# FYTalon/pienerf

Hardware: AMD Instinct MI355X
Metric: sim+render steps/s @800x800 chair (higher is better)
Workload: dtype f32 render / f64 sim

## Files before the change

### include/pienerf_hip.h

```cpp
#ifndef PIENERF_HIP_H
#define PIENERF_HIP_H
#include <stdint.h>
#ifdef __cplusplus
extern "C" {
#endif

#define PN_OK 0
#define PN_ERR_ARG 1
#define PN_ERR_HIP 2
#define PN_ERR_CAPACITY 3

const char* pn_version(void);

int pn_stream_create_cu_mask(uint32_t total_cu, uint32_t first_cu, uint32_t n_cu, int invert, void** stream_out);
int pn_stream_destroy(void* stream);
int pn_march_set_tail_rounds(int rounds);
int pn_march_set_skip_dda(int on);
int pn_device_cu_count(void);
const char* pn_last_error(void);


int pn_sph_from_ray(const float* rays_o, const float* rays_d, float radius, uint32_t N, float* coords, void* stream);
int pn_near_far_from_aabb(const float* rays_o, const float* rays_d, const float* aabb, uint32_t N, float min_near, float* nears, float* fars,
                          void* stream);

int pn_march_rays_quadratic_bending(const int* pig_cnt, const int* pig_bgn, const int* pig_idx, int n_vtx, int n_grid, const float* p_def,
                                    const float* p_ori, const float* F_IP, const float* dF_IP, int max_iter_num, const float* bbmin,
                                    const float* bbmax, float hgs, const int* resolution, int num_seek_IP, float IP_dx, int cut,
                                    const float* cut_bounds, uint32_t n_alive, uint32_t n_step, const int* rays_alive, const float* rays_t,
                                    const float* rays_o, const float* rays_d, float bound, float dt_gamma, uint32_t max_steps, uint32_t C,
                                    uint32_t H, const uint8_t* grid, const float* nears, const float* fars, float* xyzs, float* dirs,
                                    float* deltas, const float* noises, int* err_flag, void* stream);

int pn_composite_rays(uint32_t n_alive, uint32_t n_step, float T_thresh, int* rays_alive, float* rays_t, const float* sigmas, const float* rgbs,
                      const float* deltas, float* weights_sum, float* depth, float* image, void* stream);

int pn_compact_rays(const int* rays_alive, uint32_t n, int* out, int* n_out, int* scratch, void* stream);
uint32_t pn_compact_scratch_ints(uint32_t n);

int pn_pnts_in_grids(int n_vtx, int n_grid, const float* pnts, const float* bbmin, float hgs, const int* resolution, int* pig_cnt, int* pig_bgn,
                     int* pig_idx, int* err_flag, void* stream);

int pn_get_rays(const float* pose, float fx, float fy, float cx, float cy, int H, int W, float* rays_o, float* rays_d, void* stream);


int pn_grid_encode_forward(const float* inputs, const float* embeddings, const int* offsets_host, float* outputs, uint32_t B, uint32_t D,
                           uint32_t C, uint32_t L, float S, uint32_t H, float* dy_dx, uint32_t gridtype, int align_corners,
                           uint32_t interp, int out_bl_major, void* stream);

int pn_grid_encode_forward_half(const float* inputs, const uint16_t* embeddings, const int* offsets_host, uint16_t* outputs, uint32_t B, uint32_t D,
                                uint32_t C, uint32_t L, float S, uint32_t H, uint32_t gridtype, int align_corners, uint32_t interp,
                                int out_bl_major, void* stream);


int pn_sh_encode_forward(const float* inputs, float* outputs, uint32_t B, uint32_t D, uint32_t C, float* dy_dx, void* stream);


int pn_march_rays(uint32_t n_alive, uint32_t n_step, const int* rays_alive, const float* rays_t, const float* rays_o, const float* rays_d,
                  float bound, float dt_gamma, uint32_t max_steps, uint32_t C, uint32_t H, const uint8_t* grid, const float* nears,
                  const float* fars, float* xyzs, float* dirs, float* deltas, const float* noises, void* stream);
int pn_packbits(const float* grid, uint32_t N, float density_thresh, uint8_t* bitfield, void* stream);
int pn_morton3D(const int* coords, uint32_t N, int* indices, void* stream);
int pn_morton3D_invert(const int* indices, uint32_t N, int* coords, void* stream);


int pn_march_rays_train(const float* rays_o, const float* rays_d, const uint8_t* grid, float bound, float dt_gamma, uint32_t max_steps, uint32_t N,
                        uint32_t C, uint32_t H, uint32_t M, const float* nears, const float* fars, float* xyzs, float* dirs, float* deltas, int* rays,
                        int* counter, const float* noises, void* stream);
int pn_composite_rays_train_forward(const float* sigmas, const float* rgbs, const float* deltas, const int* rays, uint32_t M, uint32_t N, float T_thresh,
                                    float* weights_sum, float* depth, float* image, void* stream);
int pn_composite_rays_train_backward(const float* grad_weights_sum, const float* grad_image, const float* sigmas, const float* rgbs,
                                     const float* deltas, const int* rays, const float* weights_sum, const float* image, uint32_t M, uint32_t N,
                                     float T_thresh, float* grad_sigmas, float* grad_rgbs, void* stream);
int pn_grid_encode_backward(const float* grad, const float* inputs, const float* embeddings, const int* offsets_host, float* grad_embeddings,
                            uint32_t B, uint32_t D, uint32_t C, uint32_t L, float S, uint32_t H, const float* dy_dx, float* grad_inputs,
                            uint32_t gridtype, int align_corners, uint32_t interp, void* stream);
int pn_grid_encode_backward_half(const uint16_t* grad, const float* inputs, const int* offsets_host, uint16_t* grad_embeddings, uint32_t B, uint32_t D,
                                 uint32_t C, uint32_t L, float S, uint32_t H, uint32_t gridtype, int align_corners, uint32_t interp, void* stream);
int pn_grad_total_variation(const float* inputs, const float* embeddings, float* grad, const int* offsets_host, float weight, uint32_t B, uint32_t D,
                            uint32_t C, uint32_t L, float S, uint32_t H, uint32_t gridtype, int align_corners, void* stream);
int pn_sh_encode_backward(const float* grad, const float* inputs, uint32_t B, uint32_t D, uint32_t C, const float* dy_dx, float* grad_inputs,
                          void* stream);


typedef struct pn_net pn_net;
int pn_net_create(pn_net** out, const float* embeddings , const int* offsets_host , uint32_t L, uint32_t C,
                  float per_level_scale_log2, uint32_t base_resolution, float bound, const float* W0_host, const float* W1_host,
                  const float* W2_host, const float* W3_host, const float* W4_host, void* stream);
void pn_net_destroy(pn_net* net);
int pn_net_update(pn_net* net, const float* embeddings, const float* W0_host, const float* W1_host, const float* W2_host, const float* W3_host,
                  const float* W4_host, void* stream);
int pn_net_form(const pn_net* net);
int pn_net_form_epoch(const pn_net* net);
int pn_net_enable_half(pn_net* net, void* stream);
int pn_nerf_forward(const pn_net* net, const float* xyzs, const float* dirs, uint32_t M, float density_scale, float* sigmas, float* rgbs,
                    void* stream);
int pn_nerf_forward_half(const pn_net* net, const float* xyzs, const float* dirs, uint32_t M, float density_scale, float* sigmas, float* rgbs,
                         void* stream);
int pn_nerf_density(const pn_net* net, const float* xyzs, uint32_t M, float* sigmas, float* geo_feat, void* stream);
int pn_nerf_density_half(const pn_net* net, const float* xyzs, uint32_t M, float* sigmas, float* geo_feat, void* stream);
int pn_nerf_sigma(const pn_net* net, const float* xyzs, uint32_t M, float density_scale, float* sigmas, int half, void* stream);
int pn_host_float_to_half(const float* in_host, uint16_t* out_host, uint32_t n);


typedef struct pn_bg_net pn_bg_net;
int pn_bg_net_create(pn_bg_net** out, const float* embeddings, const int* offsets_host , uint32_t L, uint32_t C, float per_level_scale_log2,
                     uint32_t base_resolution, const float* W0_host, const float* W1_host, void* stream);
int pn_bg_net_update(pn_bg_net* net, const float* embeddings, const float* W0_host, const float* W1_host, void* stream);
void pn_bg_net_destroy(pn_bg_net* net);
int pn_background_forward(const pn_bg_net* net, const float* rays_o, const float* rays_d, uint32_t N, float radius, float* rgb_out,
                          const float* weights_sum, float* image, float* coords_out, void* stream);
int pn_background_forward_half(const pn_bg_net* net, const float* rays_o, const float* rays_d, uint32_t N, float radius, float* rgb_out,
                               const float* weights_sum, float* image, float* coords_out, void* stream);

int pn_background_coords(const pn_bg_net* net, const float* coords, const float* dirs, uint32_t N, float* rgb_out, int half, void* stream);

int pn_nerf_color(const pn_net* net, const float* dirs, const float* geo_feat, const uint8_t* mask, uint32_t M, float* rgbs, void* stream);
int pn_nerf_color_half(const pn_net* net, const float* dirs, const float* geo_feat, const uint8_t* mask, uint32_t M, float* rgbs, void* stream);

int pn_render_hier(const pn_net* net, const float* rays_o, const float* rays_d, uint32_t N, const float* aabb_host, float min_near, int num_steps,
                   int upsample_steps, float density_scale, float bg_scalar, const float* bg_rays, float* image, float* depth, float* weights_sum, int half,
                   void* stream);
int pn_hier_max_samples(void);


typedef struct pn_frame pn_frame;
typedef struct {
    int max_iter_num;
    float hash_grid_size;
    int num_seek_IP;
    float IP_dx;
    int cut;
    float cut_bounds[6];
    float bound;
    float min_near;
    float dt_gamma;
    uint32_t max_steps;
    float T_thresh;
    uint32_t cascade;
    uint32_t grid_size;
    float density_scale;
    float bg_color;
    int fp16;
    int reuse_tables;
    int ray_batch;
    int throughput;
    int throughput_trips;
    int ray_tile_w;
    int fused_from;
    int fused_whole;
    int fused_fold;
    int fused_grid;
} pn_render_opts;
int pn_frame_create(pn_frame** out, uint32_t max_rays, uint32_t max_vtx, uint32_t max_grid_cells);
void pn_frame_destroy(pn_frame* f);
int pn_render_deformed(pn_frame* f, const pn_net* net, const pn_render_opts* opts, const float* rays_o, const float* rays_d, uint32_t N,
                       const float* p_def, const float* p_ori, const float* F_IP, const float* dF_IP, int n_vtx, const uint8_t* bitfield,
                       float* image, float* depth, float* depth_0, float* weights_sum, int64_t* stats_host, void* stream);

int pn_render_deformed_async(pn_frame* f, const pn_net* net, const pn_render_opts* opts, const float* rays_o, const float* rays_d, uint32_t N,
                             const float* p_def, const float* p_ori, const float* F_IP, const float* dF_IP, int n_vtx, const uint8_t* bitfield,
                             float* image, float* depth, float* depth_0, float* weights_sum, int n_trips, void* stream);
int pn_render_status(pn_frame* f, int64_t* stats_host, int synchronize, void* stream);
int pn_frame_reset_unfinished(pn_frame* f, void* stream);

int pn_render_continue(pn_frame* f, const pn_net* net, const pn_render_opts* opts, const float* rays_o, const float* rays_d, uint32_t N,
                       const uint8_t* bitfield, float* image, float* depth, float* depth_0, float* weights_sum, int64_t* stats_host, int n_trips,
                       int is_static, void* stream);

int pn_render_static(pn_frame* f, const pn_net* net, const pn_render_opts* opts, const float* rays_o, const float* rays_d, uint32_t N,
                     const float* aabb_host, const uint8_t* bitfield, float* image, float* depth, float* depth_0, float* weights_sum,
                     int64_t* stats_host, int n_trips, void* stream);


typedef struct pn_copier pn_copier;
int pn_copier_create(pn_copier** out);
void pn_copier_destroy(pn_copier* c);
int pn_copier_submit(pn_copier* c, void* dst_host, const void* src_dev, uint64_t bytes, void* after_event, uint64_t* ticket);
int pn_copier_wait(pn_copier* c, uint64_t ticket);


int pn_mark_untrained_grid(const float* poses, uint32_t B, float fx, float fy, float cx, float cy, uint32_t cascade, uint32_t H, float bound,
                           float* density_grid, int* n_unseen, void* stream);
int pn_density_cells_full(uint32_t cascade, uint32_t H, float bound, const float* noise, float* xyzs, void* stream);
int pn_density_cells_partial(uint32_t cas, uint32_t H, float bound, uint32_t N, const int* rand_coords, const float* rand_pick, const float* noise,
                             const float* density_grid_cas, float* tmp_grid_cas, int* scratch, int* indices, float* xyzs, void* stream);
uint64_t pn_density_partial_scratch_ints(uint32_t H);
int pn_density_scatter(uint32_t n, const int* indices, const float* sigmas, float* tmp_grid_cas, void* stream);
int pn_density_grid_update(uint32_t n, float* density_grid, const float* tmp_grid, float decay, float density_thresh, uint8_t* bitfield,
                           double* partial, float* mean_thresh, void* stream);

int pn_frame_march_counters(pn_frame* f, int enable, uint64_t* counters_host, void* stream);
int pn_frame_fused_clocks(pn_frame* f, uint64_t* clocks_host, int* first_trip_out, int reset, void* stream);
int pn_frame_trip_records(pn_frame* f, int* records_host, int* tail_counts_host, int max_trips, void* stream);
int pn_frame_trip_times(pn_frame* f, float* march_ms_host, float* network_ms_host, int max_trips, int* n_trips_out, void* stream);


int pn_sim_update_F(int n_IP, const int* topo, const double* dof, const double* Nx, const double* dNx, const double* ddNx, float* pos, float* F,
                    float* dF, void* stream);

int pn_sim_calc_elastic(int n_IP, const int* topo, const double* dNx, const double* dof, double* RF, double* VF, double* FF, int mcadams_sweeps,
                        void* stream);

int pn_sim_collect_rhs(int n_k, double dx, const int* csr_bg, const int* csr_cnt, const int* csr_buf, const double* mu, const double* lam,
                       const double* dNx, const double* RF, const double* VF, double* rhs, void* stream);

int pn_sim_matvec3(int n, const double* A, const double* X, double* Y, void* stream);

int pn_sim_stepforward(int n_k, int n_IP, int iters, double dt, double dx, const int* topo, const int* csr_bg, const int* csr_cnt,
                       const int* csr_buf, const double* mu, const double* lam, const double* dNx, const double* dNx_csr, const int* csr_pos,
                       const double* Ainv,
                       const double* Mmat, const double* dof_rest, const double* rhs_rest, const double* rhs_gravity, const double* dof_f,
                       double* dof, double* dof_vel, double* work, int prepared, int mcadams_sweeps, void* stream);
uint64_t pn_sim_work_doubles(int n_k, int n_IP);
int pn_sim_cells_chunk_ips(void);
uint64_t pn_sim_cells_work_doubles(int n_k, int n_chunks);
int pn_sim_cells_prepare(int n_k, int n_chunks, double* work, void* stream);
int pn_sim_stepforward_cells(int n_k, int n_chunks, int iters, double dt, double dx, const int* chunk_tab, const double* dNx_cell, const double* mu_cell,
                             const double* lam_cell, const int* kp_bg, const int* kp_pos, const double* Ainv, const double* Mmat, const double* dof_rest,
                             const double* rhs_rest, const double* rhs_gravity, const double* dof_f, double* dof, double* dof_vel, double* work,
                             int mcadams_sweeps, void* stream);
uint64_t pn_sim_coop_bytes(int n_k, int n_IP, int n_wg);
int pn_sim_coop_prepare(int n_k, int n_IP, int n_wg, const int* csr_bg, const int* csr_cnt, void* coop, int* plan_out, void* stream);
int pn_sim_coop_status(const void* coop, int* timed_out);
int pn_sim_coop_clocks(const void* coop, uint64_t* ticks9);
int pn_sim_stepforward_coop(int n_k, int n_IP, int iters, double dt, double dx, const int* topo, const double* mu, const double* lam, const double* dNx,
                            const double* dNx_csr, const int* csr_pos, const double* Ainv, const double* Mmat, const double* dof_rest,
                            const double* rhs_rest, const double* rhs_gravity, const double* dof_f, double* dof, double* dof_vel, double* work,
                            void* coop, int n_wg, const int* plan, void* stream);
int pn_sim_prepare(int n_k, int n_IP, const int* csr_bg, const int* csr_cnt, double* work, void* stream);

int pn_sim_update_force(int n_k, int vid, const double* f3_host, double dx, const int* topo, const double* rho, const double* Nx, double* dof_f,
                        void* stream);

typedef struct pn_drag_state {
    int vid;
    int active;
    double target[3];
    double scale;
} pn_drag_state;
uint64_t pn_sim_drag_bytes(void);
uint64_t pn_sim_drag_work_doubles(void);
int pn_sim_drag_force(int n_k, int n_IP, const void* drag, const double* dof, double dx, const int* topo, const double* rho, const double* Nx,
                      double* dof_f, void* stream);
int pn_sim_drag_set(void* drag, int n_IP, int vid, int active, double scale, const double* target3_host, void* stream);
int pn_sim_drag_unproject(const float* depth0, int W, int H, double x, double y, const double* intr4, const double* pose16, const float* ip_pos,
                          int n_IP, void* drag, double* work, void* stream);


uint64_t pn_mc_work_bytes(int nx, int ny, int nz);
int pn_mc_count(const float* field, int nx, int ny, int nz, double threshold, void* work, int64_t* totals, void* stream);
int pn_mc_emit(const float* field, int nx, int ny, int nz, double threshold, const void* work, double* vertices, int* triangles, void* stream);
int pn_mc_case_table(uint8_t* tri_count, int8_t* tri_edges);

int pn_ccl_label(const uint8_t* occ, int nx, int ny, int nz, int connectivity, int* labels, void* stream);



int pn_sample_cells(const float* weights, const float* expo, int n_cells, int N, int64_t* cells_out, int* status, void* stream);
int pn_train_batch(const float* pose, float fx, float fy, float cx, float cy, int H, int W, int N, int mode, const int64_t* a, const int64_t* b,
                   const float* u, int patch, const float* image, int C, int64_t* inds_out, float* rays_o, float* rays_d, float* pixels_out,
                   void* stream);
int pn_error_map_update(float* map_row, const int64_t* cells, const float* err, int N, void* stream);

#ifdef __cplusplus
}
#endif
#endif
```

### pienerf_amd/_lib.py

```python
import ctypes as C
import os

_HERE = os.path.dirname(os.path.abspath(__file__))
LIB_PATH = os.environ.get("PN_LIB_PATH") or os.path.join(_HERE, "lib", "libpienerf_hip.so")

P = C.c_void_p
u32, i32, f32, f64, u64 = C.c_uint32, C.c_int, C.c_float, C.c_double, C.c_uint64


class RenderOpts(C.Structure):
    _fields_ = [("max_iter_num", i32), ("hash_grid_size", f32), ("num_seek_IP", i32), ("IP_dx", f32), ("cut", i32), ("cut_bounds", f32 * 6),
                ("bound", f32), ("min_near", f32), ("dt_gamma", f32), ("max_steps", u32), ("T_thresh", f32), ("cascade", u32), ("grid_size", u32),
                ("density_scale", f32), ("bg_color", f32), ("fp16", i32), ("reuse_tables", i32), ("ray_batch", i32), ("throughput", i32), ("throughput_trips", i32), ("ray_tile_w", i32),
                ("fused_from", i32), ("fused_whole", i32), ("fused_fold", i32), ("fused_grid", i32)]


SIGNATURES = {
    "pn_version": (C.c_char_p, []),
    "pn_last_error": (C.c_char_p, []),
    "pn_stream_create_cu_mask": (i32, [u32, u32, u32, i32, C.POINTER(C.c_void_p)]),
    "pn_stream_destroy": (i32, [P]),
    "pn_device_cu_count": (i32, []),
    "pn_march_set_tail_rounds": (i32, [i32]),
    "pn_march_set_skip_dda": (i32, [i32]),
    "pn_copier_create": (i32, [C.POINTER(P)]),
    "pn_copier_destroy": (None, [P]),
    "pn_copier_submit": (i32, [P, P, P, C.c_uint64, P, C.POINTER(C.c_uint64)]),
    "pn_copier_wait": (i32, [P, C.c_uint64]),
    "pn_near_far_from_aabb": (i32, [P, P, P, u32, f32, P, P, P]),
    "pn_sph_from_ray": (i32, [P, P, f32, u32, P, P]),
    "pn_march_rays_quadratic_bending": (i32, [P, P, P, i32, i32, P, P, P, P, i32, P, P, f32, P, i32, f32, i32, P, u32, u32, P, P, P, P, f32, f32, u32,
                                              u32, u32, P, P, P, P, P, P, P, P, P]),
    "pn_composite_rays": (i32, [u32, u32, f32, P, P, P, P, P, P, P, P, P]),
    "pn_compact_rays": (i32, [P, u32, P, P, P, P]),
    "pn_compact_scratch_ints": (u32, [u32]),
    "pn_pnts_in_grids": (i32, [i32, i32, P, P, f32, P, P, P, P, P, P]),
    "pn_get_rays": (i32, [P, f32, f32, f32, f32, i32, i32, P, P, P]),
    "pn_grid_encode_forward": (i32, [P, P, P, P, u32, u32, u32, u32, f32, u32, P, u32, i32, u32, i32, P]),
    "pn_sh_encode_forward": (i32, [P, P, u32, u32, u32, P, P]),
    "pn_net_create": (i32, [C.POINTER(P), P, P, u32, u32, f32, u32, f32, P, P, P, P, P, P]),
    "pn_net_destroy": (None, [P]),
    "pn_net_update": (i32, [P, P, P, P, P, P, P, P]),
    "pn_net_enable_half": (i32, [P, P]),
    "pn_nerf_forward_half": (i32, [P, P, P, u32, f32, P, P, P]),
    "pn_nerf_density_half": (i32, [P, P, u32, P, P, P]),
    "pn_nerf_sigma": (i32, [P, P, u32, f32, P, i32, P]),
    "pn_host_float_to_half": (i32, [P, P, u32]),
    "pn_grid_encode_forward_half": (i32, [P, P, P, P, u32, u32, u32, u32, f32, u32, u32, i32, u32, i32, P]),
    "pn_march_rays_train": (i32, [P, P, P, f32, f32, u32, u32, u32, u32, u32, P, P, P, P, P, P, P, P, P]),
    "pn_composite_rays_train_forward": (i32, [P, P, P, P, u32, u32, f32, P, P, P, P]),
    "pn_composite_rays_train_backward": (i32, [P, P, P, P, P, P, P, P, u32, u32, f32, P, P, P]),
    "pn_grid_encode_backward": (i32, [P, P, P, P, P, u32, u32, u32, u32, f32, u32, P, P, u32, i32, u32, P]),
    "pn_grid_encode_backward_half": (i32, [P, P, P, P, u32, u32, u32, u32, f32, u32, u32, i32, u32, P]),
    "pn_grad_total_variation": (i32, [P, P, P, P, f32, u32, u32, u32, u32, f32, u32, u32, i32, P]),
    "pn_sh_encode_backward": (i32, [P, P, u32, u32, u32, P, P, P]),
    "pn_march_rays": (i32, [u32, u32, P, P, P, P, f32, f32, u32, u32, u32, P, P, P, P, P, P, P, P]),
    "pn_packbits": (i32, [P, u32, f32, P, P]),
    "pn_morton3D": (i32, [P, u32, P, P]),
    "pn_morton3D_invert": (i32, [P, u32, P, P]),
    "pn_nerf_forward": (i32, [P, P, P, u32, f32, P, P, P]),
    "pn_nerf_density": (i32, [P, P, u32, P, P, P]),
    "pn_bg_net_create": (i32, [C.POINTER(P), P, P, u32, u32, f32, u32, P, P, P]),
    "pn_bg_net_update": (i32, [P, P, P, P, P]),
    "pn_bg_net_destroy": (None, [P]),
    "pn_background_forward": (i32, [P, P, P, u32, f32, P, P, P, P, P]),
    "pn_background_forward_half": (i32, [P, P, P, u32, f32, P, P, P, P, P]),
    "pn_background_coords": (i32, [P, P, P, u32, P, i32, P]),
    "pn_nerf_color": (i32, [P, P, P, P, u32, P, P]),
    "pn_nerf_color_half": (i32, [P, P, P, P, u32, P, P]),
    "pn_render_hier": (i32, [P, P, P, u32, C.POINTER(f32), f32, i32, i32, f32, f32, P, P, P, P, i32, P]),
    "pn_hier_max_samples": (i32, []),
    "pn_frame_create": (i32, [C.POINTER(P), u32, u32, u32]),
    "pn_frame_destroy": (None, [P]),
    "pn_render_deformed": (i32, [P, P, C.POINTER(RenderOpts), P, P, u32, P, P, P, P, i32, P, P, P, P, P, P, P]),
    "pn_render_deformed_async": (i32, [P, P, C.POINTER(RenderOpts), P, P, u32, P, P, P, P, i32, P, P, P, P, P, i32, P]),
    "pn_render_status": (i32, [P, P, i32, P]),
    "pn_frame_reset_unfinished": (i32, [P, P]),
    "pn_render_continue": (i32, [P, P, C.POINTER(RenderOpts), P, P, u32, P, P, P, P, P, P, i32, i32, P]),
    "pn_render_static": (i32, [P, P, C.POINTER(RenderOpts), P, P, u32, P, P, P, P, P, P, P, i32, P]),
    "pn_mark_untrained_grid": (i32, [P, u32, f32, f32, f32, f32, u32, u32, f32, P, P, P]),
    "pn_density_cells_full": (i32, [u32, u32, f32, P, P, P]),
    "pn_density_cells_partial": (i32, [u32, u32, f32, u32, P, P, P, P, P, P, P, P, P]),
    "pn_density_partial_scratch_ints": (u64, [u32]),
    "pn_density_scatter": (i32, [u32, P, P, P, P]),
    "pn_density_grid_update": (i32, [u32, P, P, f32, f32, P, P, P, P]),
    "pn_frame_march_counters": (i32, [P, i32, P, P]),
    "pn_frame_trip_times": (i32, [P, P, P, i32, P, P]),
    "pn_frame_fused_clocks": (i32, [P, P, P, i32, P]),
    "pn_net_form": (i32, [P]),
    "pn_net_form_epoch": (i32, [P]),
    "pn_frame_trip_records": (i32, [P, P, P, i32, P]),
    "pn_sim_update_F": (i32, [i32, P, P, P, P, P, P, P, P, P]),
    "pn_sim_calc_elastic": (i32, [i32, P, P, P, P, P, P, i32, P]),
    "pn_sim_collect_rhs": (i32, [i32, f64, P, P, P, P, P, P, P, P, P, P]),
    "pn_sim_matvec3": (i32, [i32, P, P, P, P]),
    "pn_sim_stepforward": (i32, [i32, i32, i32, f64, f64, P, P, P, P, P, P, P, P, P, P, P, P, P, P, P, P, P, P, i32, i32, P]),
    "pn_sim_prepare": (i32, [i32, i32, P, P, P, P]),
    "pn_sim_cells_chunk_ips": (i32, []),
    "pn_sim_cells_work_doubles": (u64, [i32, i32]),
    "pn_sim_cells_prepare": (i32, [i32, i32, P, P]),
    "pn_sim_stepforward_cells": (i32, [i32, i32, i32, f64, f64, P, P, P, P, P, P, P, P, P, P, P, P, P, P, P, i32, P]),
    "pn_sim_work_doubles": (u64, [i32, i32]),
    "pn_sim_coop_bytes": (u64, [i32, i32, i32]),
    "pn_sim_coop_prepare": (i32, [i32, i32, i32, P, P, P, C.POINTER(i32), P]),
    "pn_sim_coop_status": (i32, [P, C.POINTER(i32)]),
    "pn_sim_coop_clocks": (i32, [P, C.POINTER(u64)]),
    "pn_sim_stepforward_coop": (i32, [i32, i32, i32, f64, f64, P, P, P, P, P, P, P, P, P, P, P, P, P, P, P, P, i32, C.POINTER(i32), P]),
    "pn_sim_update_force": (i32, [i32, i32, P, f64, P, P, P, P, P]),
    "pn_sim_drag_bytes": (u64, []),
    "pn_sim_drag_work_doubles": (u64, []),
    "pn_sim_drag_force": (i32, [i32, i32, P, P, f64, P, P, P, P, P]),
    "pn_sim_drag_set": (i32, [P, i32, i32, i32, f64, P, P]),
    "pn_sim_drag_unproject": (i32, [P, i32, i32, f64, f64, P, P, P, i32, P, P, P]),
    "pn_mc_work_bytes": (u64, [i32, i32, i32]),
    "pn_mc_count": (i32, [P, i32, i32, i32, f64, P, P, P]),
    "pn_mc_emit": (i32, [P, i32, i32, i32, f64, P, P, P, P]),
    "pn_mc_case_table": (i32, [P, P]),
    "pn_ccl_label": (i32, [P, i32, i32, i32, i32, P, P]),
    "pn_sample_cells": (i32, [P, P, i32, i32, P, P, P]),
    "pn_train_batch": (i32, [P, f32, f32, f32, f32, i32, i32, i32, i32, P, P, P, i32, P, i32, P, P, P, P, P]),
    "pn_error_map_update": (i32, [P, P, P, i32, P]),
}

_lib = None


def lib():
    global _lib
    if _lib is None:
        if not os.path.exists(LIB_PATH):
            raise RuntimeError(f"{LIB_PATH} is missing: build it with `python -m pienerf_amd.build` (hipcc, gfx950). There is no CPU fallback.")
        import torch
        h = C.CDLL(LIB_PATH)
        for name, (res, args) in SIGNATURES.items():
            fn = getattr(h, name)
            fn.restype = res
            fn.argtypes = args
        _lib = h
    return _lib


def check(rc, what=""):
    if rc != 0:
        msg = lib().pn_last_error().decode(errors="replace")
        raise RuntimeError(f"libpienerf_hip: {what} failed with code {rc}: {msg}")


def require_gpu(*tensors):
    for t in tensors:
        if t is not None and not t.is_cuda:
            raise RuntimeError("pienerf_amd ops run on the GPU only (HIP kernels); got a CPU tensor and there is no CPU fallback")


def ptr(t):
    if t is None:
        return None
    assert t.is_contiguous(), "tensor must be contiguous"
    return C.c_void_p(t.data_ptr())


def stream_ptr():
    import torch
    return C.c_void_p(torch.cuda.current_stream().cuda_stream)
```

### pienerf_amd/csrc/pn_frame_kernels.h

```cpp
#pragma once
#include <float.h>

#include "pn_cell_hash.h"
#include "pn_compact.h"
#include "pn_march_kernels.h"
#include "pn_near_far.h"
#include "pn_side_tables.h"

#define PN_MAX_TRIPS 1100
#define PN_MIN_RAY_BATCH 64
#define PN_TRIP_BATCH 8
#define PN_TRIP_MARGIN 2
#define PN_TIMED_TRIPS 64

#include "pn_trips_fused.h"

struct pn_frame {
    uint32_t max_rays, max_vtx, max_cells;
    float *nears, *fars, *rays_t, *xyzs, *dirs, *deltas, *sigmas, *rgbs;
    float* acc_image;
    int *alive_a, *alive_b, *list, *chunk_counts;
    TailEntry* tail;
    int* list_seg;
    int* active_seg;
    uint32_t seg_cap;
    uint32_t* cell_bits;
    uint32_t* grid_regions;
    float* fars_eff;
    int* seg_counters;
    int* tail_counts;
    int *pig_cnt, *pig_bgn, *pig_idx, *pig_cursor;
    MarchSide side;
    PnTrip* trips;
    PnGroup* groups;
    int* group_cnt;
    uint32_t max_groups;
    PnFrameDev* dev;
    float* cut_bounds;
    PnTrip* trips_pinned;
    PnFrameDev* dev_pinned;
    float cut_bounds_host[6];
    int cut_bounds_valid;
    int last_trips;
    uint32_t last_N;
    uint32_t last_group_rays;
    int tables_n_vtx;
    unsigned long long* march_counters;
    int march_counters_on;
    hipEvent_t ev[PN_TIMED_TRIPS][3];
    int timed_trips;
    unsigned long long* stamps;
    int stamped;
    int* fused_ctl;
    uint32_t fused_blocks;
    unsigned long long* fused_clocks;
    int fused_first;
    float* t_resume;
    int* blist;
    int4* strag;
    uint32_t blist_cap;
    int skip_done;
    int head_marched;
    int fused_mode;
};

__global__ void k_set_aabb(PnFrameDev* dev, float a0, float a1, float a2, float a3, float a4, float a5) {
    dev->aabb[0] = a0; dev->aabb[1] = a1; dev->aabb[2] = a2; dev->aabb[3] = a3; dev->aabb[4] = a4; dev->aabb[5] = a5;
    dev->resolution[0] = dev->resolution[1] = dev->resolution[2] = dev->resolution[3] = 0;
    dev->err = 0;
}

__global__ void k_reset_unfinished(PnFrameDev* dev) { dev->unfinished = 0; }

__global__ void __launch_bounds__(256) k_frame_finish(uint32_t N, float bg, const float* __restrict__ nears, const float* __restrict__ fars,
                                                      const float* __restrict__ weights_sum, const float* __restrict__ depth_0,
                                                      const float* __restrict__ acc, float* __restrict__ image, float* __restrict__ depth,
                                                      const PnTrip* __restrict__ trips, PnFrameDev* dev, int trips_run, int add_fused) {
    const uint32_t i = threadIdx.x + blockIdx.x * blockDim.x;
    if (i < 64) {
        const int lane = (int)i;
        const int t_final = min(trips_run + (add_fused ? dev->fused_trips : 0), PN_MAX_TRIPS);
        int n_trips = 0;
        long long n_samples = 0;
        for (int k = lane; k < t_final; k += 64) {
            const PnTrip* r = trips + k;
            if (r->n_alive > 0) n_trips++;
            n_samples += r->dense ? r->n_emitted : r->n_samples;
        }
#pragma unroll
        for (int o = 32; o > 0; o >>= 1) { n_trips += __shfl_xor(n_trips, o); n_samples += __shfl_xor(n_samples, o); }
        if (lane == 0) {
            const int left = trips[t_final].n_alive;
            dev->trips_run = t_final;
            dev->fused_trips = 0;
            dev->stat_trips = n_trips;
            dev->stat_samples = n_samples;
            dev->alive_at_exit = left;
            if (left > 0) atomicAdd(&dev->unfinished, left);
        }
    }
    if (i >= N) return;
    const float k = (1 - weights_sum[i]) * bg;
    image[i * 3] = acc[i * 3] + k;
    image[i * 3 + 1] = acc[i * 3 + 1] + k;
    image[i * 3 + 2] = acc[i * 3 + 2] + k;
    depth[i] = fmaxf(depth_0[i] - nears[i], 0.0f) / (fars[i] - nears[i]);
}

__global__ void k_stamp(unsigned long long* slot) { *slot = __builtin_amdgcn_s_memrealtime(); }

template <bool LARGE>
__global__ void __launch_bounds__(1024) k_frame_tables(const float* __restrict__ p_def, int n_vtx, int cut, float bound, float hgs, int max_cells,
                                                       PnFrameDev* dev, int* pig_cnt, int* pig_bgn, int* pig_idx, int* pig_cursor, uint32_t* cell_bits) {
    extern __shared__ unsigned cnt2[];
    for (int w = threadIdx.x; w < 2 * ((max_cells + 31) / 32); w += blockDim.x) cell_bits[w] = 0u;
    __shared__ float smin[3][16], smax[3][16];
    __shared__ float sh_min[3];
    __shared__ int sh_res[4];
    __shared__ int wsum[16];
    __shared__ int carry_s;
    float mn[3] = {FLT_MAX, FLT_MAX, FLT_MAX}, mx[3] = {-FLT_MAX, -FLT_MAX, -FLT_MAX};
    for (int i = threadIdx.x; i < n_vtx; i += blockDim.x)
#pragma unroll
        for (int c = 0; c < 3; c++) { const float v = p_def[i * 3 + c]; mn[c] = fminf(mn[c], v); mx[c] = fmaxf(mx[c], v); }
    const int lane = threadIdx.x & 63, wid = threadIdx.x >> 6;
#pragma unroll
    for (int c = 0; c < 3; c++) {
#pragma unroll
        for (int o = 32; o > 0; o >>= 1) { mn[c] = fminf(mn[c], __shfl_xor(mn[c], o)); mx[c] = fmaxf(mx[c], __shfl_xor(mx[c], o)); }
        if (lane == 0) { smin[c][wid] = mn[c]; smax[c][wid] = mx[c]; }
    }
    __syncthreads();
    if (threadIdx.x == 0) {
        int ncell = 1;
        for (int c = 0; c < 3; c++) {
            float a = smin[c][0], b = smax[c][0];
            for (int w = 1; w < 16; w++) { a = fminf(a, smin[c][w]); b = fmaxf(b, smax[c][w]); }
            if (cut) { a = -bound; b = bound; }
            const float lo = a - 1e-3f, hi = b + 1e-3f;
            dev->aabb[c] = lo;
            dev->aabb[3 + c] = hi;
            sh_min[c] = lo;
            const int r = (int)ceilf((hi - lo) / hgs);
            dev->resolution[c] = r;
            sh_res[c] = r;
            ncell *= r;

        }
        int err = 0;
        if (ncell > max_cells || ncell <= 0) { err = 4; ncell = 0; }
        dev->resolution[3] = ncell;
        dev->err = err;
        dev->nb_alloc = 0;
        sh_res[3] = ncell;
        carry_s = 0;
    }
    __syncthreads();
    const int n_grid_all = sh_res[3], r0 = sh_res[0], r1 = sh_res[1], r2 = sh_res[2];
    const float b0 = sh_min[0], b1 = sh_min[1], b2 = sh_min[2];
    if (n_grid_all == 0) return;
    __shared__ int s_lo[3], s_hi[3];
    if (threadIdx.x < 3) { s_lo[threadIdx.x] = 0x7fffffff; s_hi[threadIdx.x] = -1; }
    __syncthreads();
    for (int p = threadIdx.x; p < n_vtx; p += blockDim.x) {
        const int q0 = (int)floorf((p_def[p * 3] - b0) / hgs), q1 = (int)floorf((p_def[p * 3 + 1] - b1) / hgs), q2 = (int)floorf((p_def[p * 3 + 2] - b2) / hgs);
        const int gid = q2 * r1 * r0 + q1 * r0 + q0;
        if (gid < 0 || gid >= n_grid_all) continue;
        const int c0 = gid % r0, c1 = (gid / r0) % r1, c2 = gid / (r0 * r1);
        atomicMin(&s_lo[0], c0); atomicMax(&s_hi[0], c0);
        atomicMin(&s_lo[1], c1); atomicMax(&s_hi[1], c1);
        atomicMin(&s_lo[2], c2); atomicMax(&s_hi[2], c2);
    }
    __syncthreads();
    if (threadIdx.x < 3) {
        const bool any = s_hi[threadIdx.x] >= 0;
        dev->ip_lo[threadIdx.x] = any ? s_lo[threadIdx.x] : 0;
        dev->ip_hi[threadIdx.x] = any ? s_hi[threadIdx.x] : -1;
    }
    if (LARGE) return;
    const int n_grid = n_grid_all;
    for (int g = threadIdx.x; g < (n_grid + 1) / 2; g += blockDim.x) cnt2[g] = 0u;
    __syncthreads();
    auto cell_of = [&](int p) {
        const int g0 = (int)floorf((p_def[p * 3] - b0) / hgs);
        const int g1 = (int)floorf((p_def[p * 3 + 1] - b1) / hgs);
        const int g2 = (int)floorf((p_def[p * 3 + 2] - b2) / hgs);
        const int gid = g2 * r1 * r0 + g1 * r0 + g0;
        return (gid < 0 || gid >= n_grid) ? -1 : gid;
    };
    auto count_of = [&](int g) { return (int)((cnt2[g >> 1] >> (16 * (g & 1))) & 0xFFFFu); };
    for (int p = threadIdx.x; p < n_vtx; p += blockDim.x) {
        const int gid = cell_of(p);
        if (gid >= 0) atomicAdd(&cnt2[gid >> 1], 1u << (16 * (gid & 1)));
        else atomicOr(&dev->err, 2);
    }
    __syncthreads();
    {
        int* out_cnt = pig_cnt;
        int* out_bgn = pig_bgn;
        int* out_cur = pig_cursor;
        for (int base = 0; base < n_grid; base += 4096) {
            const int i0 = base + threadIdx.x * 4;
            int v[4];
#pragma unroll
            for (int k = 0; k < 4; k++) {
                const int c = i0 + k;
                int val = 0;
                if (c < n_grid) {
                    val = count_of(c);
                    out_cnt[c] = val;
                }
                v[k] = val;
            }
            const int tsum = v[0] + v[1] + v[2] + v[3];
            int inc = tsum;
#pragma unroll
            for (int o = 1; o < 64; o <<= 1) {
                const int u = __shfl_up(inc, o);
                if (lane >= o) inc += u;
            }
            if (lane == 63) wsum[wid] = inc;
            __syncthreads();
            int woff = 0;
            for (int w = 0; w < wid; w++) woff += wsum[w];
            int total = 0;
            for (int w = 0; w < 16; w++) total += wsum[w];
            int run = carry_s + woff + inc - tsum;
#pragma unroll
            for (int k = 0; k < 4; k++) {
                if (i0 + k < n_grid) { out_bgn[i0 + k] = run; out_cur[i0 + k] = run; }
                run += v[k];
            }
            __syncthreads();
            if (threadIdx.x == 0) carry_s += total;
            __syncthreads();
        }
        if (threadIdx.x == 0) carry_s = 0;
        __syncthreads();
    }
    int* lidx = reinterpret_cast<int*>(cnt2 + (max_cells + 1) / 2);
    for (int p = threadIdx.x; p < n_vtx; p += blockDim.x) {
        const int gid = cell_of(p);
        if (gid >= 0) lidx[atomicAdd(pig_cursor + gid, 1)] = p;
    }
    __syncthreads();
    for (int g = threadIdx.x; g < n_grid; g += blockDim.x) {
        const int c = count_of(g);
        if (c < 2) continue;
        int* a = lidx + __hip_atomic_load(pig_bgn + g, __ATOMIC_RELAXED, __HIP_MEMORY_SCOPE_AGENT);
        for (int i = 1; i < c; i++) {
            const int v = a[i];
            int j = i - 1;
            while (j >= 0 && a[j] > v) { a[j + 1] = a[j]; j--; }
            a[j + 1] = v;
        }
    }
    __syncthreads();
    for (int p = threadIdx.x; p < n_vtx; p += blockDim.x) pig_idx[p] = lidx[p];
}

struct FramePrologue {
    int n_grid_max; const int* n_grid_dev; const int* res; const int* pig_cnt; const int* pig_bgn; const int* pig_idx; const float* p_def; int swap;
    int2* nb_rng; float4* nb; int nb_capacity; int list_blocks; uint32_t* cell_bits; int lds_words;
    int pack_blocks; int n_vtx; const float* p_ori; const float* F_IP; const float* dF_IP; float* rec;
    const float* rays_o; const float* rays_d; PnFrameDev* dev; uint32_t N; float min_near; float* nears; float* fars; float* rays_t; PnTrip* trips;
    int* tail_counts; int* seg_counters; int n_trip_records; int* alive; float* weights_sum; float* depth_0; float* image; PnGroup* groups;
    int* group_cnt; uint32_t group_rays; uint32_t n_groups; int* chunk_words;
    uint32_t tile_w, tile_lw;
    int early_finish; float bg; float* image_out; float* depth_out;
    const uint8_t* grid; uint32_t* grid_regions; int gr_blocks; int gr_R; int gr_C; uint32_t gr_H; float gr_bound; const float* cut_bounds;
};
#define PN_GRID_REGION_WORDS 1024

__device__ __forceinline__ void frame_lists_block(const FramePrologue& a) {
    extern __shared__ uint32_t lds_bits[];
    __shared__ int wtot[4];
    __shared__ int blk_base;
    const int n_grid = min(*a.n_grid_dev, a.n_grid_max);
    const int r0 = a.res[0], r1 = a.res[1], r2 = a.res[2];
    const int lane = threadIdx.x & 63, wid = threadIdx.x >> 6, sub = threadIdx.x & 7;
    const int words = (a.n_grid_max + 31) / 32;
    const int per_round = a.list_blocks * 32;
    const int ilo0 = a.dev->ip_lo[0], ilo1 = a.dev->ip_lo[1], ilo2 = a.dev->ip_lo[2], ihi0 = a.dev->ip_hi[0], ihi1 = a.dev->ip_hi[1], ihi2 = a.dev->ip_hi[2];
    const bool in_lds = a.lds_words > 0;
    if (in_lds) {
        for (int w = threadIdx.x; w < 2 * a.lds_words; w += blockDim.x) lds_bits[w] = 0u;
        __syncthreads();
    }
    for (int c0 = 0; c0 < n_grid; c0 += per_round) {
        const int c = c0 + (int)blockIdx.x * 32 + ((int)threadIdx.x >> 3);
        const bool valid = c < n_grid;
        int g0 = 0, g1 = 0, g2 = 0;
        if (valid) nb_cell_coords(c, r0, r1, g0, g1, g2);
        const bool near_ips = valid && g0 >= ilo0 - 1 && g0 <= ihi0 + 1 && g1 >= ilo1 - 1 && g1 <= ihi1 + 1 && g2 >= ilo2 - 1 && g2 <= ihi2 + 1;
        int cell[4], cnt[4], before[4];
        int total = 0;
#pragma unroll
        for (int k = 0; k < 4; k++) {
            const int q = sub + 8 * k;
            cell[k] = (near_ips && q < 27) ? ((q == 0) ? c : nb_neighbour(q - 1, a.swap, g0, g1, g2, r0, r1, r2)) : -1;
            cnt[k] = cell[k] >= 0 ? a.pig_cnt[cell[k]] : 0;
            int inc = cnt[k];
#pragma unroll
            for (int o = 1; o < 8; o <<= 1) {
                const int u = __shfl_up(inc, o, 8);
                if (sub >= o) inc += u;
            }
            before[k] = total + inc - cnt[k];
            total += __shfl(inc, 7, 8);
        }
        const int mine = (sub == 0) ? total : 0;
        int inc = mine;
#pragma unroll
        for (int o = 1; o < 64; o <<= 1) {
            const int u = __shfl_up(inc, o);
            if (lane >= o) inc += u;
        }
        if (lane == 63) wtot[wid] = inc;
        const int in_wave = __shfl(inc - mine, lane & ~7);
        __syncthreads();
        if (threadIdx.x == 0) {
            const int sum = wtot[0] + wtot[1] + wtot[2] + wtot[3];
            blk_base = sum ? atomicAdd(&a.dev->nb_alloc, sum) : 0;
        }
        __syncthreads();
        int w0 = blk_base + in_wave;
        for (int w = 0; w < wid; w++) w0 += wtot[w];
        __syncthreads();
        if (!valid) continue;
        const bool fits = w0 + total <= a.nb_capacity;
        if (sub == 0) {
            a.nb_rng[c] = (total > 0 && fits) ? make_int2(w0, w0 + total) : make_int2(0, 0);
            if (total > 0 && !fits) atomicOr(&a.dev->err, 8);
        }
        if (total == 0 || !fits) continue;
        if (sub == 0) atomicOr((in_lds ? lds_bits : a.cell_bits) + (c >> 5), 1u << (c & 31));
#pragma unroll
        for (int k = 0; k < 4; k++) {
            if (cell[k] < 0) continue;
            atomicOr((in_lds ? lds_bits + a.lds_words : a.cell_bits + words) + (cell[k] >> 5), 1u << (cell[k] & 31));
            const int n = cnt[k], b = a.pig_bgn[cell[k]];
            for (int i = 0; i < n; i++) {
                const int ip = a.pig_idx[b + i];
                a.nb[w0 + before[k] + i] = make_float4(a.p_def[ip * 3], a.p_def[ip * 3 + 1], a.p_def[ip * 3 + 2], __int_as_float(ip));
            }
        }
    }
    if (in_lds) {
        __syncthreads();
        for (int w = threadIdx.x; w < 2 * a.lds_words; w += blockDim.x) {
            const uint32_t v = lds_bits[w];
            if (v) atomicOr(a.cell_bits + (w < a.lds_words ? w : words + (w - a.lds_words)), v);
        }
    }
}

__device__ __forceinline__ void frame_rays_block(const FramePrologue& a, uint32_t block) {
    const uint32_t n = threadIdx.x + block * blockDim.x;
    if (block == 0 && a.groups) {
        for (uint32_t b = threadIdx.x; b < a.n_groups; b += blockDim.x) {
            a.groups[b] = PnGroup{(int)(b * a.group_rays), 1, (int)(b * a.group_rays), 0};
            a.group_cnt[b] = 0;
        }
    }
    {
        const int t = (int)block * 4 + (int)(threadIdx.x >> 6), w = threadIdx.x & 63;
        if (t < a.n_trip_records) {
            int v = 0;
            if (t == 0 && w == 0) v = (a.dev->err & 7) ? 0 : (int)a.N;
            if (t == 0 && w == 1) v = 1;
            reinterpret_cast<int*>(a.trips + t)[w] = v;
            if (w == 0) a.tail_counts[t] = 0;
        }
        if (block + 1 == gridDim.x - (uint32_t)(a.list_blocks + a.pack_blocks)) {
            for (int t2 = ((int)block + 1) * 4 + (int)(threadIdx.x >> 6); t2 < a.n_trip_records; t2 += 4) {
                reinterpret_cast<int*>(a.trips + t2)[w] = 0;
                if (w == 0) a.tail_counts[t2] = 0;
            }
        }
    }
    if (block == 0)
        for (int t = threadIdx.x; t < 6 * PN_SEGS; t += blockDim.x) a.seg_counters[t * PN_SEG_STRIDE] = 0;
    if (block == 0 && threadIdx.x == 0) {
        a.dev->fused_trips = 0;
        if (a.early_finish) {
            a.dev->trips_run = 0; a.dev->stat_trips = 0; a.dev->stat_samples = 0; a.dev->alive_at_exit = (int)a.N;
        }
    }
    if (threadIdx.x == 0) a.chunk_words[block] = 0;
    if (threadIdx.x < 2 && block + 1 == gridDim.x - (uint32_t)(a.list_blocks + a.pack_blocks)) a.chunk_words[block + 1 + threadIdx.x] = 0;
    if (n >= a.N) return;
    const float* aabb = a.dev->aabb;
    const float ox = a.rays_o[n * 3], oy = a.rays_o[n * 3 + 1], oz = a.rays_o[n * 3 + 2];
    const float dx = a.rays_d[n * 3], dy = a.rays_d[n * 3 + 1], dz = a.rays_d[n * 3 + 2];
    float near, far;
    pn_near_far(aabb, ox, oy, oz, dx, dy, dz, a.min_near, near, far);
    a.nears[n] = near;
    a.fars[n] = far;
    a.rays_t[n] = near;
    uint32_t ray = n;
    if (a.tile_w) {
        const uint32_t lw = a.tile_lw, tile = n >> 6, in = n & 63u, tiles_x = a.tile_w >> lw;
        ray = ((tile / tiles_x) * (64u >> lw) + (in >> lw)) * a.tile_w + ((tile % tiles_x) << lw) + (in & ((1u << lw) - 1u));
    }
    a.alive[n] = (int)ray;
    a.weights_sum[n] = 0.f;
    a.depth_0[n] = 0.f;
    a.image[n * 3] = 0.f; a.image[n * 3 + 1] = 0.f; a.image[n * 3 + 2] = 0.f;
    if (a.early_finish) {
        const float k = (1 - 0.f) * a.bg;
        a.image_out[n * 3] = 0.f + k; a.image_out[n * 3 + 1] = 0.f + k; a.image_out[n * 3 + 2] = 0.f + k;
        a.depth_out[n] = fmaxf(0.f - near, 0.0f) / (far - near);
    }
}

__global__ void __launch_bounds__(256) k_frame_prologue(FramePrologue a) {
    const int b = (int)blockIdx.x;
    if (b < a.list_blocks) { frame_lists_block(a); return; }
    if (b < a.list_blocks + a.pack_blocks) {
        const int t = threadIdx.x + (b - a.list_blocks) * 256;
        const int ip = t / PN_REC_FLOATS, j = t % PN_REC_FLOATS;
        if (ip < a.n_vtx) a.rec[t] = pnm2::pack_ip_float(j, ip, a.p_ori, a.p_def, a.F_IP, a.dF_IP);
        return;
    }
    if (b < a.list_blocks + a.pack_blocks + a.gr_blocks) {
        const int R = a.gr_R, n_reg = R * R * R;
        const int r = threadIdx.x + (b - a.list_blocks - a.pack_blocks) * 256;
        if (r < n_reg) {
            bool any = false;
            const int b0 = r % R, b1 = (r / R) % R, b2 = r / (R * R);
            const uint32_t vox_side = a.gr_H / (uint32_t)R, words_per_region = (vox_side * vox_side * vox_side) >> 6;
            const uint32_t words_per_level = (a.gr_H * a.gr_H * a.gr_H) >> 6;
            const uint2* g2 = reinterpret_cast<const uint2*>(a.grid);
            uint32_t acc_l[3] = {0u, 0u, 0u};
            for (int l = 0; l < a.gr_C; l++) {
                const int j = a.gr_C - 1 - l, side = 1 << j;
                const int c0 = R / 2 + (b0 - R / 2) * side, c1 = R / 2 + (b1 - R / 2) * side, c2 = R / 2 + (b2 - R / 2) * side;
                if (c0 < 0 || c1 < 0 || c2 < 0 || c0 + side > R || c1 + side > R || c2 + side > R) continue;
                const uint32_t first = (uint32_t)l * words_per_level + pnm2::morton3D((uint32_t)c0, (uint32_t)c1, (uint32_t)c2) * words_per_region;
                const uint32_t n_words = words_per_region << (3 * j);
                for (uint32_t q = 0; q < n_words; q++) {
                    const uint2 v = g2[(size_t)first + q];
                    acc_l[l] |= v.x | v.y;
                }
            }
            for (int L = a.gr_C - 2; L >= 0; L--) acc_l[L] |= acc_l[L + 1];
            const float w = 2.0f * a.gr_bound / (float)R, eps = 0.01f * w;
            const float x0 = -a.gr_bound + (float)b0 * w, y0 = -a.gr_bound + (float)b1 * w, z0 = -a.gr_bound + (float)b2 * w;
            const float* cb = a.cut_bounds;
            if (x0 + w > cb[0] - eps && x0 < cb[1] + eps && y0 + w > cb[2] - eps && z0 + w > cb[4] - eps && z0 < cb[5] + eps) any = true;
            for (int L = 0; L < a.gr_C; L++) {
                const unsigned long long m = __ballot(any || acc_l[L] != 0u);
                if ((threadIdx.x & 63) == 0) {
                    a.grid_regions[(size_t)L * (n_reg >> 5) + (r >> 5)] = (uint32_t)m;
                    a.grid_regions[(size_t)L * (n_reg >> 5) + (r >> 5) + 1] = (uint32_t)(m >> 32);
                }
            }
        }
        return;
    }
    frame_rays_block(a, (uint32_t)(b - a.list_blocks - a.pack_blocks - a.gr_blocks));
}
```

### pienerf_amd/csrc/pn_render_ops.hip

```cpp
#include <float.h>

#include "pn_render_records.h"
#include "pn_cell_hash.h"
#include "pn_side_tables.h"
#include "pn_march_kernels.h"
#include "pn_composite.h"
#include "pn_compact.h"
#include "pn_frame_kernels.h"

thread_local char pn_err_buf[512] = {0};

extern "C" int pn_pnts_in_grids(int n_vtx, int n_grid, const float* pnts, const float* bbmin, float hgs, const int* resolution, int* pig_cnt,
                                int* pig_bgn, int* pig_idx, int* err_flag, void* stream) {
    PN_REQUIRE(n_vtx > 0 && n_grid > 0 && pnts && bbmin && resolution && pig_cnt && pig_bgn && pig_idx);
    int* cursor = nullptr;
    hipStream_t st = (hipStream_t)stream;
    PN_HIP_CHECK(hipMallocAsync((void**)&cursor, sizeof(int) * (size_t)n_grid, st));
    int rc = pig_build(n_vtx, n_grid, nullptr, pnts, bbmin, hgs, resolution, pig_cnt, pig_bgn, pig_idx, cursor, err_flag, st);
    PN_HIP_CHECK(hipFreeAsync(cursor, st));
    return rc;
}

extern "C" int pn_march_set_skip_dda(int on) {
    PN_REQUIRE(on >= -1 && on <= 1);
    g_skip_dda_override = on;
    return PN_OK;
}
extern "C" int pn_march_set_tail_rounds(int rounds) {
    PN_REQUIRE(rounds >= 0);
    g_tail_rounds_override = rounds;
    return PN_OK;
}

extern "C" int pn_march_rays_quadratic_bending(const int* pig_cnt, const int* pig_bgn, const int* pig_idx, int n_vtx, int n_grid,
                                               const float* p_def, const float* p_ori, const float* F_IP, const float* dF_IP, int max_iter_num,
                                               const float* bbmin, const float* bbmax, float hgs, const int* resolution, int num_seek_IP,
                                               float IP_dx, int cut, const float* cut_bounds, uint32_t n_alive, uint32_t n_step,
                                               const int* rays_alive, const float* rays_t, const float* rays_o, const float* rays_d, float bound,
                                               float dt_gamma, uint32_t max_steps, uint32_t C, uint32_t H, const uint8_t* grid, const float* nears,
                                               const float* fars, float* xyzs, float* dirs, float* deltas, const float* noises, int* err_flag,
                                               void* stream) {
    (void)nears;
    PN_REQUIRE(pig_cnt && pig_bgn && pig_idx && p_def && p_ori && F_IP && dF_IP && bbmin && bbmax && resolution);
    PN_REQUIRE(rays_alive && rays_t && rays_o && rays_d && grid && fars && xyzs && dirs && deltas);
    PN_REQUIRE(num_seek_IP >= 1 && num_seek_IP <= 3);
    PN_REQUIRE(!cut || cut_bounds);
    PN_REQUIRE(C >= 1 && C <= 8 && H > 0 && n_step >= 1 && n_vtx > 0 && n_grid > 0);
    if (n_alive == 0) return PN_OK;
    hipStream_t st = (hipStream_t)stream;
    MarchSide s;
    s.nb_capacity = 27 * n_vtx;
    char* pool = nullptr;
    const size_t ints = ((size_t)n_grid + 1) * 5 * sizeof(int), nbb = (size_t)s.nb_capacity * sizeof(float4), recb = (size_t)n_vtx * PN_REC_FLOATS * sizeof(float);
    const size_t off_nb = (ints + 255) & ~(size_t)255, off_rec = (off_nb + nbb + 255) & ~(size_t)255;
    const size_t off_res = (off_rec + recb + 255) & ~(size_t)255;
    const uint32_t tail_cap = seg_cap_for(n_alive);
    const size_t tail_ctr = (size_t)3 * PN_SEGS * PN_SEG_STRIDE * sizeof(int);
    const size_t off_tail = (off_res + (size_t)n_alive * sizeof(float) + 255) & ~(size_t)255;
    PN_HIP_CHECK(hipMallocAsync((void**)&pool, off_tail + tail_ctr + (size_t)PN_SEGS * tail_cap * sizeof(TailEntry), st));
    PN_HIP_CHECK(hipMemsetAsync(pool + off_tail, 0, tail_ctr, st));
    s.nb_cnt = (int*)pool; s.nb_bgn = s.nb_cnt + n_grid + 1; s.nb_cursor = s.nb_bgn + n_grid + 1; s.nb_rng = (int2*)(s.nb_cursor + n_grid + 1);
    s.nb = (float4*)(pool + off_nb); s.rec = (float*)(pool + off_rec);
    int rc = march_side_build(s, n_vtx, n_grid, nullptr, resolution, pig_cnt, pig_bgn, pig_idx, p_def, p_ori, F_IP, dF_IP, num_seek_IP, err_flag, st);
    if (rc == PN_OK) {
        pnm::MarchParams a = make_march_params(pig_cnt, pig_bgn, pig_idx, n_vtx, n_grid, p_def, p_ori, F_IP, dF_IP, max_iter_num, bbmin, bbmax, hgs,
                                               resolution, num_seek_IP, IP_dx, cut, cut_bounds, rays_t, rays_o, rays_d, bound, dt_gamma, max_steps,
                                               C, H, grid, fars, err_flag);
        pnm2::March2Tables tb{s.nb_rng, s.nb, (const float4*)s.rec};
        int* const tail_ctrs = (int*)(pool + off_tail);
        MarchIO io{};
        io.n_alive = n_alive; io.n_step = n_step; io.rays_alive = rays_alive;
        io.xyzs = xyzs; io.dirs = dirs; io.deltas = deltas; io.noises = noises;
        io.t_resume = (float*)(pool + off_res);
        io.tail = (TailEntry*)(pool + off_tail + tail_ctr);
        io.tail_counts = tail_ctrs; io.tail_back = tail_ctrs + PN_SEGS * PN_SEG_STRIDE; io.tail_cursors = tail_ctrs + 2 * PN_SEGS * PN_SEG_STRIDE;
        io.tail_seg_cap = (int)tail_cap;
        io.max_rounds = (int)march_tail_rounds();
        if (io.t_resume) k_march_skip<<<pn_div_up(n_alive, 256), 256, 0, st>>>(a, tb, io);
        launch_march(num_seek_IP, pn_div_up(n_alive, 32), std::max(std::min(pn_div_up(n_alive, 4), 2048u), (uint32_t)PN_SEGS / 4), st, a, tb, io);
    }
    PN_HIP_CHECK(hipFreeAsync(pool, st));
    if (rc) return rc;
    PN_LAUNCH_CHECK();
    return PN_OK;
}

extern "C" int pn_composite_rays(uint32_t n_alive, uint32_t n_step, float T_thresh, int* rays_alive, float* rays_t, const float* sigmas,
                                 const float* rgbs, const float* deltas, float* weights_sum, float* depth, float* image, void* stream) {
    if (n_alive == 0) return PN_OK;
    PN_REQUIRE(rays_alive && rays_t && sigmas && rgbs && deltas && weights_sum && depth && image && n_step >= 1);
    k_composite<<<pn_div_up(n_alive, 256), 256, 0, (hipStream_t)stream>>>(n_alive, n_step, T_thresh, rays_alive, rays_t, sigmas, rgbs, deltas,
                                                                         weights_sum, depth, image, nullptr, nullptr, nullptr, 0, nullptr);
    PN_LAUNCH_CHECK();
    return PN_OK;
}

extern "C" uint32_t pn_compact_scratch_ints(uint32_t n) { return pn_div_up(n, 256) + 1; }

extern "C" int pn_compact_rays(const int* rays_alive, uint32_t n, int* out, int* n_out, int* scratch, void* stream) {
    PN_REQUIRE(n_out);
    hipStream_t st = (hipStream_t)stream;
    if (n == 0) { PN_HIP_CHECK(hipMemsetAsync(n_out, 0, sizeof(int), st)); return PN_OK; }
    PN_REQUIRE(rays_alive && out && scratch);
    const uint32_t chunks = pn_div_up(n, 256);
    k_chunk_count<<<chunks, 256, 0, st>>>(rays_alive, n, scratch);
    k_compact<<<chunks, 256, 0, st>>>(rays_alive, n, scratch, out, n_out, nullptr, nullptr, 0, 0, 0, nullptr, nullptr, nullptr, nullptr, nullptr, 0, 0);
    PN_LAUNCH_CHECK();
    return PN_OK;
}


extern "C" int pn_frame_create(pn_frame** out, uint32_t max_rays, uint32_t max_vtx, uint32_t max_grid_cells) {
    PN_REQUIRE(out && max_rays > 0 && max_vtx > 0 && max_grid_cells > 0);
    pn_frame* f = new pn_frame();
    memset(f, 0, sizeof(*f));
    f->max_rays = max_rays; f->max_vtx = max_vtx; f->max_cells = max_grid_cells;
    const size_t N = max_rays;
#define PN_ALLOC(ptr, bytes) PN_HIP_CHECK(hipMalloc((void**)&(ptr), (bytes)))
    PN_ALLOC(f->nears, N * 4); PN_ALLOC(f->fars, N * 4); PN_ALLOC(f->rays_t, N * 4);
    {
        int dev_id = 0, cus = 0;
        PN_HIP_CHECK(hipGetDevice(&dev_id));
        PN_HIP_CHECK(hipDeviceGetAttribute(&cus, hipDeviceAttributeMultiprocessorCount, dev_id));
        f->fused_blocks = (uint32_t)std::min(std::max(cus, 1), 1024);
    }
    f->blist_cap = (uint32_t)(N / 8 + 64 + (size_t)(f->fused_blocks + 1) * 64);
    const size_t NS = N + (size_t)f->fused_blocks * PN_FUSED_WAVES * 64 + f->blist_cap;
    PN_ALLOC(f->xyzs, NS * 12); PN_ALLOC(f->dirs, NS * 12); PN_ALLOC(f->deltas, NS * 8); PN_ALLOC(f->sigmas, NS * 4); PN_ALLOC(f->rgbs, NS * 12);
    PN_ALLOC(f->fused_ctl, (size_t)PN_FUSED_CTL_INTS * 4);
    PN_HIP_CHECK(hipMemset(f->fused_ctl, 0, (size_t)PN_FUSED_CTL_INTS * 4));
    PN_ALLOC(f->fused_clocks, 16 * sizeof(unsigned long long));
    PN_HIP_CHECK(hipMemset(f->fused_clocks, 0, 16 * sizeof(unsigned long long)));
    f->fused_first = -1;
    PN_ALLOC(f->t_resume, N * 4);
    PN_ALLOC(f->blist, (size_t)f->blist_cap * 8);
    PN_ALLOC(f->strag, (size_t)f->blist_cap * 16);
    PN_ALLOC(f->acc_image, N * 12);
    PN_ALLOC(f->alive_a, N * 4); PN_ALLOC(f->alive_b, N * 4); PN_ALLOC(f->list, N * 4); PN_ALLOC(f->chunk_counts, (N / 256 + 4) * 4);
    PN_ALLOC(f->pig_cnt, (size_t)max_grid_cells * 4); PN_ALLOC(f->pig_bgn, (size_t)max_grid_cells * 4);
    PN_ALLOC(f->pig_cursor, (size_t)max_grid_cells * 4); PN_ALLOC(f->pig_idx, (size_t)max_vtx * 4);
    PN_ALLOC(f->side.nb_rng, ((size_t)max_grid_cells + 1) * sizeof(int2));
    f->side.nb_capacity = 27 * (int)max_vtx;
    PN_ALLOC(f->side.nb, (size_t)f->side.nb_capacity * sizeof(float4)); PN_ALLOC(f->side.rec, (size_t)max_vtx * PN_REC_FLOATS * 4);
    f->seg_cap = seg_cap_for(max_rays);
    PN_ALLOC(f->tail, (size_t)PN_SEGS * f->seg_cap * sizeof(TailEntry)); PN_ALLOC(f->tail_counts, sizeof(int) * (PN_MAX_TRIPS + 2));
    PN_ALLOC(f->list_seg, (size_t)PN_SEGS * f->seg_cap * 4); PN_ALLOC(f->active_seg, (size_t)PN_SEGS * f->seg_cap * 4);
    PN_ALLOC(f->seg_counters, (size_t)6 * PN_SEGS * PN_SEG_STRIDE * 4);
    PN_ALLOC(f->cell_bits, 2 * (((size_t)max_grid_cells + 31) / 32) * 4);
    PN_ALLOC(f->fars_eff, N * 4);
    PN_ALLOC(f->grid_regions, (size_t)PN_GRID_REGION_WORDS * 4);
    PN_ALLOC(f->trips, sizeof(PnTrip) * (PN_MAX_TRIPS + 2)); PN_ALLOC(f->dev, sizeof(PnFrameDev)); PN_ALLOC(f->cut_bounds, 6 * 4);
    f->max_groups = pn_div_up(max_rays, PN_MIN_RAY_BATCH) + 1;
    PN_ALLOC(f->groups, sizeof(PnGroup) * 2 * f->max_groups); PN_ALLOC(f->group_cnt, sizeof(int) * f->max_groups);
#undef PN_ALLOC
    PN_HIP_CHECK(hipMalloc((void**)&f->march_counters, 16 * sizeof(unsigned long long)));
    PN_HIP_CHECK(hipMalloc((void**)&f->stamps, sizeof(unsigned long long) * PN_TIMED_TRIPS * 3));
    PN_HIP_CHECK(hipHostMalloc((void**)&f->trips_pinned, sizeof(PnTrip) * (PN_MAX_TRIPS + 2)));
    PN_HIP_CHECK(hipHostMalloc((void**)&f->dev_pinned, sizeof(PnFrameDev)));
    PN_HIP_CHECK(hipMemset(f->dev, 0, sizeof(PnFrameDev)));
    memset(f->dev_pinned, 0, sizeof(PnFrameDev));
    *out = f;
    return PN_OK;
}

extern "C" void pn_frame_destroy(pn_frame* f) {
    if (!f) return;
    void* ptrs[] = {f->acc_image, f->nears, f->fars, f->rays_t, f->xyzs, f->dirs, f->deltas, f->sigmas, f->rgbs, f->alive_a, f->alive_b, f->list,
                    f->chunk_counts, f->pig_cnt, f->pig_bgn, f->pig_cursor, f->pig_idx, f->trips, f->dev, f->cut_bounds,
                    f->side.nb_rng, f->side.nb, f->side.rec, f->march_counters, f->tail, f->tail_counts, f->stamps,
                    f->list_seg, f->active_seg, f->seg_counters, f->cell_bits, f->fars_eff, f->grid_regions, f->groups, f->group_cnt, f->fused_ctl, f->fused_clocks, f->t_resume, f->blist, f->strag};
    for (void* p : ptrs) if (p) (void)hipFree(p);
    for (int t = 0; t < PN_TIMED_TRIPS; t++)
        for (int e = 0; e < 3; e++) if (f->ev[t][e]) (void)hipEventDestroy(f->ev[t][e]);
    if (f->trips_pinned) (void)hipHostFree(f->trips_pinned);
    if (f->dev_pinned) (void)hipHostFree(f->dev_pinned);
    delete f;
}

static void frame_stats(pn_frame* f, int64_t* stats_host) {
    stats_host[0] = f->dev_pinned->stat_trips;
    stats_host[1] = f->dev_pinned->stat_samples;
    stats_host[2] = f->dev_pinned->err;
    stats_host[3] = f->dev_pinned->alive_at_exit;
    stats_host[4] = f->dev_pinned->unfinished;
}


struct FramePlan {
    bool is_static;
    uint32_t nblk;
    uint32_t march_grid, march_grid_first, march_grid_later, trip_grid, tail_grid;
    int dda_start;
    uint32_t skip_hop_budget;
    size_t bit_words;
    bool short_rays;
    int skip_bits_words;
    uint32_t reg_R;
    int grid_region_words_1, grid_region_words;
    size_t skip_lds;
    uint32_t lpr_rounds, lpr_trips;
    uint32_t group_rays, n_groups;
    bool fused_ok, want_whole, want_fold, early_finish;
    int fuse_from;
};

static FramePlan make_frame_plan(const pn_frame* f, const pn_render_opts* o, uint32_t N, bool is_static, bool resume, int async_trips, const uint8_t* bitfield) {
    FramePlan p{};
    p.is_static = is_static;
    p.nblk = pn_div_up(N, 256);
    p.march_grid = 8192;
    p.trip_grid = std::min(p.nblk, 1024u);
    p.march_grid_first = std::max(std::min(pn_div_up(N, 32), p.march_grid), (uint32_t)PN_SEGS);
    p.march_grid_later = std::max(std::min(pn_div_up(N, 256), p.march_grid), (uint32_t)PN_SEGS);
    p.tail_grid = std::max(std::min(pn_div_up(N, 4), 1024u), (uint32_t)PN_SEGS / 4);
    p.dda_start = g_skip_dda_override >= 0 ? g_skip_dda_override : 1;
    p.skip_hop_budget = 8;
    p.lpr_rounds = o->throughput > 0 ? (uint32_t)o->throughput : 0u;
    p.lpr_trips = (uint32_t)std::max(o->throughput_trips, 1);
    p.bit_words = (f->max_cells + 31) / 32;
    p.short_rays = !is_static && !o->cut && p.bit_words * 8 <= 48 * 1024;
    p.skip_bits_words = (p.short_rays || p.bit_words * 4 <= 48 * 1024) ? (int)p.bit_words : 0;
    p.reg_R = o->grid_size / 8;
    const bool reg_ok = !is_static && o->cut && p.dda_start && bitfield && o->grid_size % 32 == 0 && o->cascade >= 1 && o->cascade <= 3 &&
                        o->bound == (float)(1u << (o->cascade - 1)) && (p.reg_R / 2) % (1u << (o->cascade - 1)) == 0 &&
                        (uint64_t)p.reg_R * p.reg_R * p.reg_R / 32 * o->cascade <= PN_GRID_REGION_WORDS && ((uintptr_t)bitfield & 15) == 0;
    p.grid_region_words_1 = reg_ok ? (int)((uint64_t)p.reg_R * p.reg_R * p.reg_R / 32) : 0;
    p.grid_region_words = p.grid_region_words_1 * (int)o->cascade;
    p.skip_lds = (size_t)p.skip_bits_words * 4 * (p.short_rays ? 2 : 1) + (size_t)p.grid_region_words * 4;
    p.group_rays = o->ray_batch > 0 ? (uint32_t)o->ray_batch : 0u;
    p.n_groups = p.group_rays ? pn_div_up(N, p.group_rays) : 0u;
    p.fused_ok = !is_static && !p.group_rays && o->fused_from >= 0 && o->max_steps <= 8u * PN_FUSED_MAX_TRIPS;
    p.fuse_from = p.fused_ok ? std::max(o->fused_from, 1) : PN_MAX_TRIPS + 1;
    p.want_whole = p.fused_ok && o->fused_whole != 0 && o->fused_from == 0 && !resume;
    p.want_fold = p.fused_ok && !p.want_whole && o->fused_fold != 0 && o->fused_from <= 1 && !resume;
    p.early_finish = p.want_whole;
    return p;
}

struct RenderCall {
    pn_frame* f;
    const pn_net* net;
    const pn_render_opts* o;
    const float *rays_o, *rays_d;
    uint32_t N;
    const float *p_def, *p_ori, *F_IP, *dF_IP;
    int n_vtx;
    const uint8_t* bitfield;
    float *image, *depth, *depth_0, *weights_sum;
    const float* aabb_static;
    hipStream_t st;
    pnm::MarchParams mp, mq;
    pnm2::March2Tables tb;
};

static int* alive_list(const pn_frame* f, int t) { return (t & 1) ? f->alive_b : f->alive_a; }
static PnGroup* group_records(const pn_frame* f, const FramePlan& pl, int t) { return pl.group_rays ? f->groups + (size_t)(t & 1) * f->max_groups : nullptr; }
enum { SEG_TAIL, SEG_SAMP, SEG_EMIT, SEG_CURS, SEG_BACK, SEG_ACTIVE };
static int* seg_counter(const pn_frame* f, int which) { return f->seg_counters + which * PN_SEGS * PN_SEG_STRIDE; }

static MarchIO make_march_io(const RenderCall& c, const FramePlan& pl, int tt) {
    const pn_frame* f = c.f;
    const bool lpr = (uint32_t)tt < pl.lpr_trips && pl.lpr_rounds > 0;
    MarchIO io{};
    io.rays_alive = alive_list(f, tt);
    io.xyzs = f->xyzs; io.dirs = f->dirs; io.deltas = f->deltas;
    io.trip = f->trips + tt;
    io.list = f->list;
    io.t_resume = (tt == 0) ? f->t_resume : nullptr;
    io.tail = f->tail;
    io.tail_counts = seg_counter(f, SEG_TAIL); io.tail_back = seg_counter(f, SEG_BACK); io.tail_cursors = seg_counter(f, SEG_CURS);
    io.tail_seg_cap = (int)f->seg_cap;
    io.max_rounds = lpr ? (int)pl.lpr_rounds : (int)march_tail_rounds(tt);
    io.active = (tt == 0) ? f->active_seg : nullptr;
    io.active_counts = (tt == 0) ? seg_counter(f, SEG_ACTIVE) : nullptr;
    io.active_seg_cap = (int)f->seg_cap;
    io.list_seg = f->list_seg; io.samp_counts = seg_counter(f, SEG_SAMP); io.list_seg_cap = (int)f->seg_cap;
    io.emit_parts = seg_counter(f, SEG_EMIT);
    io.cell_bits = f->cell_bits; io.cell_bits_words = pl.skip_bits_words;
    io.cell_bits2 = pl.short_rays ? f->cell_bits + pl.bit_words : nullptr;
    io.fars_eff = pl.short_rays ? f->fars_eff : nullptr;
    io.groups = group_records(f, pl, tt); io.group_rays = pl.group_rays;
    io.lane_per_ray = lpr ? 1 : 0;
    io.dda_start = pl.dda_start; io.hop_budget = (int)pl.skip_hop_budget;
    io.grid_regions = pl.grid_region_words > 0 ? f->grid_regions : nullptr;
    io.grid_regions_words = pl.grid_region_words; io.grid_regions_R = (int)pl.reg_R;
    return io;
}

static int time_mark(pn_frame* f, hipStream_t st, int trip, int e, bool fused_group) {
    if (!(f->march_counters_on & 2) || trip >= PN_TIMED_TRIPS) return PN_OK;
    hipStreamCaptureStatus cs = hipStreamCaptureStatusNone;
    PN_HIP_CHECK(hipStreamIsCapturing(st, &cs));
    const bool stamp = cs != hipStreamCaptureStatusNone;
    f->stamped = stamp ? 1 : 0;
    if (stamp) {
        k_stamp<<<1, 1, 0, st>>>(f->stamps + trip * 3 + e);
    } else {
        if (!f->ev[trip][e]) PN_HIP_CHECK(hipEventCreate(&f->ev[trip][e]));
        PN_HIP_CHECK(hipEventRecord(f->ev[trip][e], st));
    }
    if (e == 2) f->timed_trips = fused_group ? std::max(f->timed_trips, trip + 1) : trip + 1;
    return PN_OK;
}

static int enqueue_tables(const RenderCall& c, bool is_static, bool keep_tables) {
    pn_frame* f = c.f;
    const pn_render_opts* o = c.o;
    const size_t tables_lds = ((size_t)f->max_cells + 1) / 2 * sizeof(unsigned) + (size_t)f->max_vtx * sizeof(int);
    const bool large = tables_lds > 150 * 1024;
    if (is_static) {
        const float* b = c.aabb_static;
        k_set_aabb<<<1, 1, 0, c.st>>>(f->dev, b[0], b[1], b[2], b[3], b[4], b[5]);
    } else if (keep_tables) {
    } else if (!large) {
        static size_t tables_lds_set[PN_MAX_DEVICES] = {0};
        int dev_id = 0;
        PN_HIP_CHECK(hipGetDevice(&dev_id));
        if (dev_id < 0 || dev_id >= PN_MAX_DEVICES || tables_lds > tables_lds_set[dev_id]) {
            PN_HIP_CHECK(hipFuncSetAttribute((const void*)k_frame_tables<false>, hipFuncAttributeMaxDynamicSharedMemorySize, (int)tables_lds));
            if (dev_id >= 0 && dev_id < PN_MAX_DEVICES) tables_lds_set[dev_id] = tables_lds;
        }
        k_frame_tables<false><<<1, 1024, tables_lds, c.st>>>(c.p_def, c.n_vtx, o->cut, o->bound, o->hash_grid_size, (int)f->max_cells, f->dev, f->pig_cnt,
                                                         f->pig_bgn, f->pig_idx, f->pig_cursor, f->cell_bits);
    } else {
        k_frame_tables<true><<<1, 1024, 0, c.st>>>(c.p_def, c.n_vtx, o->cut, o->bound, o->hash_grid_size, (int)f->max_cells, f->dev, f->pig_cnt, f->pig_bgn,
                                                   f->pig_idx, f->pig_cursor, f->cell_bits);
        return pig_build(c.n_vtx, (int)f->max_cells, f->dev->resolution + 3, c.p_def, f->dev->aabb, o->hash_grid_size, f->dev->resolution, f->pig_cnt, f->pig_bgn,
                         f->pig_idx, f->pig_cursor, &f->dev->err, c.st);
    }
    return PN_OK;
}

static int enqueue_prologue(const RenderCall& c, const FramePlan& pl) {
    pn_frame* f = c.f;
    const pn_render_opts* o = c.o;
    const bool keep_tables = !pl.is_static && o->reuse_tables && f->tables_n_vtx == c.n_vtx;
    int rc = enqueue_tables(c, pl.is_static, keep_tables);
    if (rc) return rc;
    FramePrologue fp;
    memset(&fp, 0, sizeof(fp));
    if (!pl.is_static && !keep_tables) {
        f->tables_n_vtx = c.n_vtx;
        fp.n_grid_max = (int)f->max_cells; fp.n_grid_dev = f->dev->resolution + 3; fp.res = f->dev->resolution; fp.pig_cnt = f->pig_cnt; fp.pig_bgn = f->pig_bgn;
        fp.pig_idx = f->pig_idx; fp.p_def = c.p_def; fp.swap = (o->num_seek_IP == 1) ? 1 : 0; fp.nb_rng = f->side.nb_rng; fp.nb = f->side.nb;
        fp.nb_capacity = f->side.nb_capacity; fp.cell_bits = f->cell_bits;
        fp.list_blocks = (int)std::min(pn_div_up((uint64_t)f->max_cells, 32), 2048u);
        fp.pack_blocks = (int)pn_div_up((uint64_t)c.n_vtx * PN_REC_FLOATS, 256);
        fp.n_vtx = c.n_vtx; fp.p_ori = c.p_ori; fp.F_IP = c.F_IP; fp.dF_IP = c.dF_IP; fp.rec = f->side.rec;
    }
    fp.rays_o = c.rays_o; fp.rays_d = c.rays_d; fp.dev = f->dev; fp.N = c.N; fp.min_near = o->min_near; fp.nears = f->nears; fp.fars = f->fars; fp.rays_t = f->rays_t;
    fp.trips = f->trips; fp.tail_counts = f->tail_counts; fp.seg_counters = f->seg_counters; fp.n_trip_records = PN_MAX_TRIPS + 2; fp.alive = f->alive_a;
    fp.weights_sum = c.weights_sum; fp.depth_0 = c.depth_0; fp.image = f->acc_image; fp.groups = pl.group_rays ? f->groups : nullptr; fp.group_cnt = f->group_cnt;
    fp.group_rays = pl.group_rays; fp.n_groups = pl.n_groups; fp.chunk_words = f->chunk_counts;
    fp.early_finish = pl.early_finish ? 1 : 0; fp.bg = o->bg_color; fp.image_out = c.image; fp.depth_out = c.depth;
    {
        const uint32_t lw = 4;
        const uint32_t tw = o->ray_tile_w > 0 ? (uint32_t)o->ray_tile_w : 0u;
        fp.tile_lw = lw;
        fp.tile_w = (!pl.is_static && !pl.group_rays && tw && tw % (1u << lw) == 0 && c.N % ((64u >> lw) * tw) == 0) ? tw : 0u;
    }
    fp.lds_words = (fp.list_blocks > 0 && pl.bit_words * 8 <= 64 * 1024) ? (int)pl.bit_words : 0;
    if (pl.grid_region_words > 0) {
        fp.grid = c.bitfield; fp.grid_regions = f->grid_regions; fp.gr_R = (int)pl.reg_R; fp.gr_C = (int)o->cascade; fp.gr_H = o->grid_size;
        fp.gr_bound = o->bound; fp.cut_bounds = f->cut_bounds; fp.gr_blocks = (int)pn_div_up((uint64_t)pl.grid_region_words_1 * 32, 256);
    }
    k_frame_prologue<<<(uint32_t)(fp.list_blocks + fp.pack_blocks + fp.gr_blocks) + pl.nblk, 256, (size_t)fp.lds_words * 8, c.st>>>(fp);
    PN_LAUNCH_CHECK();
    return PN_OK;
}

static void enqueue_skip(const RenderCall& c, const FramePlan& pl, const MarchIO& io0) {
    if (c.f->skip_done) return;
    k_march_skip<<<pl.nblk, 256, pl.skip_lds, c.st>>>(c.mp, c.tb, io0);
    c.f->skip_done = 1;
}
static void enqueue_march(const RenderCall& c, const FramePlan& pl, int t, bool margin) {
    const MarchIO io = make_march_io(c, pl, t);
    if (io.t_resume) enqueue_skip(c, pl, io);
    launch_march(c.o->num_seek_IP, t == 0 ? pl.march_grid_first : (margin ? 2u * PN_SEGS : pl.march_grid_later), margin ? (uint32_t)PN_SEGS : pl.tail_grid, c.st,
                 c.mq, c.tb, io);
}

static void enqueue_composite(const RenderCall& c, const FramePlan& pl, int t, bool margin) {
    pn_frame* f = c.f;
    const pn_render_opts* o = c.o;
    int *cur = alive_list(f, t), *nxt = alive_list(f, t + 1);
    PnGroup *g_cur = group_records(f, pl, t), *g_nxt = group_records(f, pl, t + 1);
    static const bool cc_trip0 = pn_env_u32("PN_CC_TRIP0", 0) != 0;
    if (!pl.is_static && !margin && (t > 0 || cc_trip0)) {
        static const uint32_t cc_grid = pn_env_u32("PN_CC_GRID", 512);
        const uint32_t cc_poll_cap = 1u << 20;
        k_composite_compact<<<std::min(cc_grid, pn_div_up(c.N, 256)), 256, 0, c.st>>>(o->T_thresh, cur, nxt, f->rays_t, f->sigmas, f->rgbs, f->deltas, c.weights_sum,
                                                                                   c.depth_0, f->acc_image, f->trips + t, f->trips + t + 1, (unsigned*)f->chunk_counts,
                                                                                   (uint32_t)t + 1, c.N, o->max_steps, 1, f->seg_counters, f->tail_counts + t, g_cur,
                                                                                   g_nxt, f->group_cnt, pl.group_rays, pl.n_groups, &f->dev->err, cc_poll_cap);
        return;
    }
    const uint32_t pair_grid = margin ? std::min(pl.trip_grid, 64u) : pl.trip_grid;
    k_composite<<<pair_grid, 256, 0, c.st>>>(0, 0, o->T_thresh, cur, f->rays_t, f->sigmas, f->rgbs, f->deltas, c.weights_sum, c.depth_0, f->acc_image, f->trips + t,
                                             f->chunk_counts, g_cur, pl.group_rays, pl.n_groups > 1 ? f->group_cnt : nullptr);
    k_compact<<<pair_grid, 256, 0, c.st>>>(cur, 0, f->chunk_counts, nxt, nullptr, f->trips + t, f->trips + t + 1, c.N, o->max_steps, pl.is_static ? 0 : 1,
                                           pl.is_static ? nullptr : f->seg_counters, f->tail_counts + t, g_cur, g_nxt, f->group_cnt, pl.group_rays, pl.n_groups);
}

static int enqueue_trip(const RenderCall& c, const FramePlan& pl, int t, bool margin) {
    pn_frame* f = c.f;
    const pn_render_opts* o = c.o;
    int rc;
    if ((rc = time_mark(f, c.st, t, 0, false))) return rc;
    if (pl.is_static) {
        k_march_static_trip<<<pl.trip_grid, 256, 0, c.st>>>(f->trips + t, alive_list(f, t), f->rays_t, c.rays_o, c.rays_d, o->bound, o->dt_gamma, o->max_steps,
                                                            o->cascade, o->grid_size, c.bitfield, f->fars, f->xyzs, f->dirs, f->deltas, f->list);
    } else {
        if (!(t == 0 && f->head_marched)) enqueue_march(c, pl, t, margin);
        if (t == 0) k_list_pack<<<PN_SEGS, 256, 0, c.st>>>(f->trips + t, seg_counter(f, SEG_SAMP), f->list_seg, (int)f->seg_cap, f->list);
    }
    if ((rc = time_mark(f, c.st, t, 1, false))) return rc;
    rc = pn_nerf_forward_launch(c.net, f->xyzs, f->dirs, f->list, &f->trips[t].n_samples, c.N, o->density_scale, f->sigmas, f->rgbs, o->fp16, c.st, margin ? 64u : 0u);
    if (rc) return rc;
    if ((rc = time_mark(f, c.st, t, 2, false))) return rc;
    enqueue_composite(c, pl, t, margin);
    return PN_OK;
}

static int enqueue_fused(const RenderCall& c, const FramePlan& pl, int t, int form, bool finalize) {
    pn_frame* f = c.f;
    const pn_net* net = c.net;
    const pn_render_opts* o = c.o;
    const bool whole = form == 1, fold = form == 2;
    int rc;
    if (fold) {
        if ((rc = time_mark(f, c.st, 0, 0, true))) return rc;
        enqueue_march(c, pl, 0, false);
        f->head_marched = 1;
        if ((rc = time_mark(f, c.st, 0, 1, true)) || (rc = time_mark(f, c.st, 0, 2, true))) return rc;
    }
    FusedArgs fa;
    memset(&fa, 0, sizeof(fa));
    fa.lv = (const PnFusedLevel*)(o->fp16 ? net->fused_levels : net->byte_levels); fa.emb = net->embeddings; fa.emb_h = (const uint32_t*)net->emb_half; fa.emb_bytes = net->n_entries * 4u;
    fa.wimg_g = (const uint4*)(o->fp16 ? net->whalf : (net->x_ok ? net->wx : net->wsplit)); fa.net_bound = net->bound; fa.net_inv2b = 1.0f / (2 * net->bound); fa.density_scale = o->density_scale;
    fa.x_scales = net->x_scales;
    fa.trips = f->trips + t; fa.N_rays = c.N; fa.max_steps = o->max_steps; fa.T_thresh = o->T_thresh;
    fa.alive = alive_list(f, t);
    fa.rays_t = f->rays_t; fa.weights_sum = c.weights_sum; fa.depth = c.depth_0; fa.image = f->acc_image;
    fa.xyzs = f->xyzs; fa.dirs = f->dirs; fa.deltas = f->deltas; fa.sigmas = f->sigmas; fa.rgbs = f->rgbs;
    fa.ctl = f->fused_ctl; fa.dev = f->dev; fa.tail_diag = f->tail_counts + t;
    fa.clocks = (f->march_counters_on & 4) ? f->fused_clocks : nullptr;
    if (whole) {
        fa.active = f->active_seg; fa.active_counts = seg_counter(f, SEG_ACTIVE); fa.active_seg_cap = (int)f->seg_cap; fa.t_resume = f->t_resume;
        fa.blist = f->blist; fa.strag = f->strag; fa.blist_cap = f->blist_cap;
        fa.a_rounds = 24;
    }
    if (fold) {
        fa.list_seg = f->list_seg; fa.samp_counts = seg_counter(f, SEG_SAMP); fa.list_seg_cap = (int)f->seg_cap;
        fa.seg_tail = seg_counter(f, SEG_TAIL); fa.seg_back = seg_counter(f, SEG_BACK);
        fa.blist = f->blist; fa.strag = f->strag; fa.blist_cap = f->blist_cap;
    }
    if (finalize) {
        fa.finalize = 1; fa.bg = o->bg_color; fa.nears = f->nears; fa.fars_full = f->fars; fa.image_out = c.image; fa.depth_out = c.depth;
    }
    const int tb_idx = fold ? 1 : t;
    if ((rc = time_mark(f, c.st, tb_idx, 0, true))) return rc;
    if (whole) enqueue_skip(c, pl, make_march_io(c, pl, 0));
    const uint32_t blocks = o->fused_grid > 0 ? std::min((uint32_t)o->fused_grid, f->fused_blocks) : f->fused_blocks;
    rc = launch_trips_fused(o->num_seek_IP, o->max_iter_num > 1, o->fp16 ? 1 : (net->x_ok ? 2 : 0), form, blocks, c.st, c.mq, c.tb, fa);
    if (rc) return rc;
    if ((rc = time_mark(f, c.st, tb_idx, 1, true)) || (rc = time_mark(f, c.st, tb_idx, 2, true))) return rc;
    f->fused_first = tb_idx;
    f->fused_mode = form;
    return PN_OK;
}

static int check_render_call(const RenderCall& c, bool is_static, bool resume, int async_trips) {
    const pn_frame* f = c.f;
    const pn_render_opts* o = c.o;
    PN_REQUIRE(f && c.net && o && c.rays_o && c.rays_d && c.bitfield && c.image && c.depth && c.depth_0 && c.weights_sum);
    PN_REQUIRE(is_static || resume || (c.p_def && c.p_ori && c.F_IP && c.dF_IP && c.n_vtx > 0 && (uint32_t)c.n_vtx <= f->max_vtx));
    PN_REQUIRE(!resume || c.N == f->last_N);
    PN_REQUIRE(c.N > 0 && c.N <= f->max_rays);
    PN_REQUIRE(o->num_seek_IP >= 1 && o->num_seek_IP <= 3 && o->cascade >= 1 && o->cascade <= 8 && o->max_steps <= PN_MAX_TRIPS - PN_TRIP_BATCH);
    PN_REQUIRE(async_trips >= 0 && async_trips <= PN_MAX_TRIPS);
    PN_REQUIRE(!o->fp16 || c.net->emb_half);
    PN_REQUIRE(o->ray_batch == 0 || (o->ray_batch >= PN_MIN_RAY_BATCH && !is_static));
    PN_REQUIRE((o->ray_batch > 0 ? pn_div_up(c.N, (uint32_t)o->ray_batch) : 0u) <= f->max_groups);
    PN_REQUIRE(!resume || (o->ray_batch > 0 ? (uint32_t)o->ray_batch : 0u) == f->last_group_rays);
    return PN_OK;
}

static int enqueue_trips(const RenderCall& c, const FramePlan& pl, int async_trips, bool resume, int& t, int& add_fused, bool& finished_in_launch) {
    pn_frame* f = c.f;
    int rc;
    bool done = false;
    bool whole_try = pl.want_whole && t == 0, fold_try = pl.want_fold && t == 0;
    while (!done && t < PN_MAX_TRIPS) {
        const bool whole = whole_try;
        whole_try = false;
        const bool fold = !whole && fold_try && t == 0 && !f->head_marched;
        if (fold) fold_try = false;
        if (whole || fold || t >= pl.fuse_from) {
            const bool finalize = (whole || fold) && pl.early_finish;
            if ((rc = enqueue_fused(c, pl, t, whole ? 1 : (fold ? 2 : 0), finalize))) return rc;
            if (async_trips > 0) {
                add_fused = 1;
                finished_in_launch = finalize;
                break;
            }
            PN_HIP_CHECK(hipMemcpyAsync(f->dev_pinned, f->dev, sizeof(PnFrameDev), hipMemcpyDeviceToHost, c.st));
            PN_HIP_CHECK(hipMemcpyAsync(f->trips_pinned + t, f->trips + t, sizeof(PnTrip), hipMemcpyDeviceToHost, c.st));
            PN_HIP_CHECK(hipStreamSynchronize(c.st));
            if (f->dev_pinned->fused_trips > 0) {
                t += f->dev_pinned->fused_trips;
                finished_in_launch = finalize;
                break;
            }
            if (f->trips_pinned[t].n_alive <= 0) break;
            f->fused_first = -1;
            f->fused_mode = 0;
        }
        const int batch = async_trips > 0 ? (pl.fused_ok ? pl.fuse_from - t : async_trips) : (pl.fused_ok ? std::max(pl.fuse_from - t, 1) : PN_TRIP_BATCH);
        for (int k = 0; k < batch; k++, t++) {
            const bool margin = !pl.fused_ok && async_trips > PN_TRIP_MARGIN && k >= async_trips - PN_TRIP_MARGIN && !resume;
            if ((rc = enqueue_trip(c, pl, t, margin))) return rc;
        }
        PN_LAUNCH_CHECK();
        if (async_trips > 0) {
            if (pl.fused_ok) continue;
            break;
        }
        if (pl.fused_ok && t >= pl.fuse_from) continue;
        PN_HIP_CHECK(hipMemcpyAsync(f->trips_pinned + t, f->trips + t, sizeof(PnTrip), hipMemcpyDeviceToHost, c.st));
        PN_HIP_CHECK(hipStreamSynchronize(c.st));
        done = f->trips_pinned[t].n_alive <= 0;
    }
    return PN_OK;
}

static int render_impl(pn_frame* f, const pn_net* net, const pn_render_opts* o, const float* rays_o, const float* rays_d, uint32_t N,
                       const float* p_def, const float* p_ori, const float* F_IP, const float* dF_IP, int n_vtx, const uint8_t* bitfield, float* image,
                       float* depth, float* depth_0, float* weights_sum, int64_t* stats_host, int async_trips, void* stream,
                       const float* aabb_static = nullptr, int mode = 0 ) {
    const bool is_static = aabb_static != nullptr || mode == 2;
    const bool resume = mode != 0;
    RenderCall c{};
    c.f = f; c.net = net; c.o = o; c.rays_o = rays_o; c.rays_d = rays_d; c.N = N;
    c.p_def = p_def; c.p_ori = p_ori; c.F_IP = F_IP; c.dF_IP = dF_IP; c.n_vtx = n_vtx; c.bitfield = bitfield;
    c.image = image; c.depth = depth; c.depth_0 = depth_0; c.weights_sum = weights_sum; c.aabb_static = aabb_static; c.st = (hipStream_t)stream;
    int rc = check_render_call(c, is_static, resume, async_trips);
    if (rc) return rc;
    const FramePlan pl = make_frame_plan(f, o, N, is_static, resume, async_trips, bitfield);
    c.mp = make_march_params(f->pig_cnt, f->pig_bgn, f->pig_idx, n_vtx, 0, p_def, p_ori, F_IP, dF_IP, o->max_iter_num, f->dev->aabb, f->dev->aabb + 3,
                             o->hash_grid_size, f->dev->resolution, o->num_seek_IP, o->IP_dx, o->cut, f->cut_bounds, f->rays_t, rays_o, rays_d, o->bound,
                             o->dt_gamma, o->max_steps, o->cascade, o->grid_size, bitfield, f->fars, &f->dev->err);
    c.mp.stats = (f->march_counters_on & 1) ? f->march_counters : nullptr;
    c.mq = c.mp;
    if (pl.short_rays) c.mq.fars = f->fars_eff;
    c.tb = pnm2::March2Tables{f->side.nb_rng, f->side.nb, (const float4*)f->side.rec};

    if (!f->cut_bounds_valid || memcmp(f->cut_bounds_host, o->cut_bounds, sizeof(f->cut_bounds_host)) != 0) {
        memcpy(f->cut_bounds_host, o->cut_bounds, sizeof(f->cut_bounds_host));
        PN_HIP_CHECK(hipMemcpyAsync(f->cut_bounds, f->cut_bounds_host, 6 * sizeof(float), hipMemcpyHostToDevice, c.st));
        f->cut_bounds_valid = 1;
    }
    if (!resume) {
        if ((rc = enqueue_prologue(c, pl))) return rc;
        f->skip_done = 0;
        f->head_marched = 0;
    }
    int t = resume ? f->dev_pinned->trips_run : 0;
    PN_REQUIRE(t >= 0 && t <= PN_MAX_TRIPS);
    f->fused_first = -1;
    int add_fused = 0;
    bool finished_in_launch = false;
    if ((rc = enqueue_trips(c, pl, async_trips, resume, t, add_fused, finished_in_launch))) return rc;
    if (!finished_in_launch)
        k_frame_finish<<<pl.nblk, 256, 0, c.st>>>(N, o->bg_color, f->nears, f->fars, weights_sum, depth_0, f->acc_image, image, depth, f->trips, f->dev, t, add_fused);
    PN_LAUNCH_CHECK();
    f->last_trips = t;
    f->last_N = N;
    f->last_group_rays = pl.group_rays;
    PN_HIP_CHECK(hipMemcpyAsync(f->dev_pinned, f->dev, sizeof(PnFrameDev), hipMemcpyDeviceToHost, c.st));
    if (async_trips == 0 && stats_host) {
        PN_HIP_CHECK(hipStreamSynchronize(c.st));
        frame_stats(f, stats_host);
    }
    return PN_OK;
}

extern "C" int pn_render_deformed(pn_frame* f, const pn_net* net, const pn_render_opts* o, const float* rays_o, const float* rays_d, uint32_t N,
                                  const float* p_def, const float* p_ori, const float* F_IP, const float* dF_IP, int n_vtx,
                                  const uint8_t* bitfield, float* image, float* depth, float* depth_0, float* weights_sum, int64_t* stats_host,
                                  void* stream) {
    return render_impl(f, net, o, rays_o, rays_d, N, p_def, p_ori, F_IP, dF_IP, n_vtx, bitfield, image, depth, depth_0, weights_sum, stats_host, 0, stream);
}

extern "C" int pn_render_deformed_async(pn_frame* f, const pn_net* net, const pn_render_opts* o, const float* rays_o, const float* rays_d,
                                        uint32_t N, const float* p_def, const float* p_ori, const float* F_IP, const float* dF_IP, int n_vtx,
                                        const uint8_t* bitfield, float* image, float* depth, float* depth_0, float* weights_sum, int n_trips,
                                        void* stream) {
    PN_REQUIRE(n_trips > 0);
    return render_impl(f, net, o, rays_o, rays_d, N, p_def, p_ori, F_IP, dF_IP, n_vtx, bitfield, image, depth, depth_0, weights_sum, nullptr, n_trips,
                       stream);
}

extern "C" int pn_render_static(pn_frame* f, const pn_net* net, const pn_render_opts* o, const float* rays_o, const float* rays_d, uint32_t N,
                                const float* aabb_host, const uint8_t* bitfield, float* image, float* depth, float* depth_0, float* weights_sum,
                                int64_t* stats_host, int n_trips, void* stream) {
    PN_REQUIRE(aabb_host && n_trips >= 0);
    return render_impl(f, net, o, rays_o, rays_d, N, nullptr, nullptr, nullptr, nullptr, 0, bitfield, image, depth, depth_0, weights_sum, stats_host, n_trips,
                       stream, aabb_host);
}

extern "C" int pn_render_continue(pn_frame* f, const pn_net* net, const pn_render_opts* o, const float* rays_o, const float* rays_d, uint32_t N,
                                  const uint8_t* bitfield, float* image, float* depth, float* depth_0, float* weights_sum, int64_t* stats_host, int n_trips,
                                  int is_static, void* stream) {
    PN_REQUIRE(n_trips >= 0);
    return render_impl(f, net, o, rays_o, rays_d, N, nullptr, nullptr, nullptr, nullptr, 0, bitfield, image, depth, depth_0, weights_sum, stats_host, n_trips,
                       stream, nullptr, is_static ? 2 : 1);
}

extern "C" int pn_frame_march_counters(pn_frame* f, int enable, uint64_t* counters_host, void* stream) {
    PN_REQUIRE(f);
    hipStream_t st = (hipStream_t)stream;
    if (counters_host) {
        PN_HIP_CHECK(hipMemcpyAsync(counters_host, f->march_counters, 4 * sizeof(unsigned long long), hipMemcpyDeviceToHost, st));
#if PN_DBG_PHASES || PN_DBG_STATS
        {
            unsigned long long ph[16];
            PN_HIP_CHECK(hipMemcpy(ph, f->march_counters, sizeof(ph), hipMemcpyDeviceToHost));
            fprintf(stderr, "phases:");
            for (int i = 4; i < 16; i++) fprintf(stderr, " %llu", ph[i]);
            fprintf(stderr, "\n");
        }
#endif
        PN_HIP_CHECK(hipStreamSynchronize(st));
    }
    if ((enable & 1) && !(f->march_counters_on & 1)) PN_HIP_CHECK(hipMemsetAsync(f->march_counters, 0, 16 * sizeof(unsigned long long), st));
    f->march_counters_on = enable & 7;
    return PN_OK;
}

extern "C" int pn_frame_fused_clocks(pn_frame* f, uint64_t* clocks_host, int* first_trip_out, int reset, void* stream) {
    PN_REQUIRE(f);
    hipStream_t st = (hipStream_t)stream;
    if (clocks_host) {
        PN_HIP_CHECK(hipMemcpyAsync(clocks_host, f->fused_clocks, 16 * sizeof(unsigned long long), hipMemcpyDeviceToHost, st));
        PN_HIP_CHECK(hipStreamSynchronize(st));
        clocks_host[15] = f->fused_first >= 0 ? (uint64_t)f->fused_mode : 0u;
    }
    if (first_trip_out) *first_trip_out = f->fused_first;
    if (reset) PN_HIP_CHECK(hipMemsetAsync(f->fused_clocks, 0, 16 * sizeof(unsigned long long), st));
    return PN_OK;
}

extern "C" int pn_frame_trip_times(pn_frame* f, float* march_ms_host, float* network_ms_host, int max_trips, int* n_trips_out, void* stream) {
    PN_REQUIRE(f && march_ms_host && network_ms_host && n_trips_out && max_trips >= 0);
    PN_HIP_CHECK(hipStreamSynchronize((hipStream_t)stream));
    const int n = f->timed_trips < max_trips ? f->timed_trips : max_trips;
    if (f->stamped) {
        static unsigned long long host[PN_TIMED_TRIPS * 3];
        PN_HIP_CHECK(hipMemcpy(host, f->stamps, sizeof(unsigned long long) * (size_t)n * 3, hipMemcpyDeviceToHost));
        for (int t = 0; t < n; t++) {
            march_ms_host[t] = (float)((double)(host[t * 3 + 1] - host[t * 3]) * 1e-5);
            network_ms_host[t] = (float)((double)(host[t * 3 + 2] - host[t * 3 + 1]) * 1e-5);
        }
    } else {
        for (int t = 0; t < n; t++) {
            PN_HIP_CHECK(hipEventElapsedTime(march_ms_host + t, f->ev[t][0], f->ev[t][1]));
            PN_HIP_CHECK(hipEventElapsedTime(network_ms_host + t, f->ev[t][1], f->ev[t][2]));
        }
    }
    *n_trips_out = n;
    return PN_OK;
}

extern "C" int pn_frame_trip_records(pn_frame* f, int* records_host, int* tail_counts_host, int max_trips, void* stream) {
    PN_REQUIRE(f && records_host && tail_counts_host && max_trips >= 0);
    PN_HIP_CHECK(hipStreamSynchronize((hipStream_t)stream));
    const int n = max_trips < PN_MAX_TRIPS ? max_trips : PN_MAX_TRIPS;
    std::vector<PnTrip> rec((size_t)n);
    PN_HIP_CHECK(hipMemcpy(rec.data(), f->trips, sizeof(PnTrip) * (size_t)n, hipMemcpyDeviceToHost));
    for (int i = 0; i < n; i++) {
        int* r = records_host + 5 * i;
        r[0] = rec[i].n_alive; r[1] = rec[i].n_step; r[2] = rec[i].step_base; r[3] = rec[i].n_samples; r[4] = rec[i].dense ? rec[i].n_emitted : -1;
    }
    PN_HIP_CHECK(hipMemcpy(tail_counts_host, f->tail_counts, sizeof(int) * (size_t)n, hipMemcpyDeviceToHost));
    return PN_OK;
}


extern "C" int pn_frame_reset_unfinished(pn_frame* f, void* stream) {
    PN_REQUIRE(f);
    k_reset_unfinished<<<1, 1, 0, (hipStream_t)stream>>>(f->dev);
    PN_LAUNCH_CHECK();
    return PN_OK;
}

extern "C" int pn_render_status(pn_frame* f, int64_t* stats_host, int synchronize, void* stream) {
    PN_REQUIRE(f && stats_host);
    if (synchronize) PN_HIP_CHECK(hipStreamSynchronize((hipStream_t)stream));
    frame_stats(f, stats_host);
    return PN_OK;
}
```

### pienerf_amd/frames.py

```python
import random

import torch
import torch.distributed as dist


def agree_on_launch_form(kw, src=0, group=None, device=None):
    import torch
    import torch.distributed as dist
    on_gpu = dist.get_backend(group) == "nccl"
    pick = torch.tensor([int(kw["fused_from"]), int(bool(kw["fused_whole"])), int(bool(kw["fused_fold"]))], dtype=torch.int64,
                        device=device if on_gpu else "cpu")
    dist.broadcast(pick, src=src, group=group)
    kw["fused_from"], kw["fused_whole"], kw["fused_fold"] = int(pick[0]), bool(pick[1]), bool(pick[2])
    return kw


def dedicated_sim_default(world_size):
    return world_size >= 3


def frame_owner(frame, world_size, sim_owner=0, dedicated_sim=False):
    if not dedicated_sim or world_size == 1:
        return frame % world_size
    k = frame % (world_size - 1)
    return k if k < sim_owner else k + 1


def broadcast_tensors(tensors, src=0, group=None):
    if not dist.is_initialized() or dist.get_world_size(group) == 1:
        return
    for t in tensors:
        dist.broadcast(t, src=src, group=group)


def checkpoint_tensors(model):
    ts = [model.encoder.embeddings.data, model.density_bitfield] + [l.weight.data for l in list(model.sigma_net) + list(model.color_net)]
    if getattr(model, "bg_net", None) is not None:
        ts += [model.encoder_bg.embeddings.data] + [l.weight.data for l in model.bg_net]
    return ts


def broadcast_checkpoint(model, src=0, group=None):
    broadcast_tensors(checkpoint_tensors(model), src=src, group=group)
    for stamp in ("_net_sig", "_bg_sig"):
        if hasattr(model, stamp):
            setattr(model, stamp, None)


def tile_partition(W, H, world, tile=8):
    ys, xs = torch.meshgrid(torch.arange(H), torch.arange(W), indexing="ij")
    block = (ys // tile) * ((W + tile - 1) // tile) + (xs // tile)
    owner = (block % world).reshape(-1)
    parts = [torch.nonzero(owner == r).reshape(-1) for r in range(world)]
    n = max(p.numel() for p in parts)
    return [torch.cat([p, torch.full((n - p.numel(),), -1, dtype=torch.int64)]) for p in parts]


class TileParallel:

    def __init__(self, W, H, render_subset, get_dof, set_dof, sim_step, sim_owner=0, group=None, tile=8, device="cpu", force_collectives=False):
        on = dist.is_available() and dist.is_initialized()
        self.collectives = on and (dist.get_world_size(group) > 1 or bool(force_collectives))
        self.world = dist.get_world_size(group) if on else 1
        self.rank = dist.get_rank(group) if on else 0
        self.W, self.H, self.group, self.owner = W, H, group, sim_owner
        self.src = dist.get_global_rank(group, sim_owner) if (on and group is not None) else sim_owner
        self.parts = [p.to(device) for p in tile_partition(W, H, self.world, tile)]
        self.render_subset, self.get_dof, self.set_dof, self.sim_step = render_subset, get_dof, set_dof, sim_step
        self._recv = None
        self._gather = None

    def step(self):
        if self.collectives:
            buf = self.get_dof() if self.rank == self.owner else (self._recv if self._recv is not None else torch.empty_like(self.get_dof()))
            self._recv = None if self.rank == self.owner else buf
            dist.broadcast(buf, src=self.src, group=self.group)
            if self.rank != self.owner:
                self.set_dof(buf)
        mine = self.render_subset(self.parts[self.rank]).contiguous()
        if self.collectives:
            if self._gather is None or self._gather.shape[1:] != mine.shape or self._gather.dtype != mine.dtype:
                self._gather = torch.empty((self.world,) + tuple(mine.shape), dtype=mine.dtype, device=mine.device)
            dist.all_gather_into_tensor(self._gather.view(-1, mine.shape[1]), mine, group=self.group)
            gathered = list(self._gather.unbind(0))
        else:
            gathered = [mine]
        full = torch.empty(self.W * self.H, mine.shape[1], dtype=mine.dtype, device=mine.device)
        for part, data in zip(self.parts, gathered):
            ok = part >= 0
            full[part[ok]] = data[ok]
        if self.rank == self.owner:
            self.sim_step()
        return full


class FramePipeline:

    def __init__(self, backend, world=1, rank=0, lanes=2, depth=2, ahead=None, sim_owner=0, dedicated_sim=None, copy_out=True, on_retire=None, force_collectives=False,
                 sim_on_lanes=False):
        self.b, self.world, self.rank, self.lanes, self.depth, self.owner = backend, int(world), int(rank), int(lanes), int(depth), int(sim_owner)
        self.dedicated = dedicated_sim_default(self.world) if dedicated_sim is None else bool(dedicated_sim and self.world > 1)
        self.ahead = self.world * self.lanes * self.depth if ahead is None else int(ahead)
        self.slots = self.ahead + self.world * self.lanes * self.depth + 1
        self.copy_out = copy_out
        self.collectives = self.world > 1 or bool(force_collectives)
        self.on_retire = on_retire
        b = backend
        self.s_sim, self.s_comm, self.s_copy = b.stream("sim"), b.stream("comm"), b.stream("copy")
        self.s_lane = [b.stream(f"lane{i}") for i in range(self.lanes)]
        S = self.slots
        self.snap_ready = [b.event() for _ in range(S)]
        self.bc_done = [b.event() for _ in range(S)]
        self.ip_done = [b.event() for _ in range(S)]
        self.bc_used, self.ip_used = [False] * S, [False] * S
        n_ws = self.lanes * self.depth
        self.render_done = [b.event() for _ in range(n_ws)]
        self.out_ready = [b.event() for _ in range(n_ws)]
        self.pending = [None] * n_ws
        self.frame = 0
        self.my_frames = 0
        self.sim_next = 0
        self.bc_next = 0
        self.retired = []
        self.last_ws, self.last_frame = None, None
        self.sim_on_lanes = bool(sim_on_lanes) and self.world == 1
        self.sub_done = [b.event() for _ in range(self.lanes + 2)] if self.sim_on_lanes else []
        self.force_done, self.force_pending = (b.event() if self.sim_on_lanes else None), False

    def before_force(self):
        if self.sim_on_lanes and self.sim_next > 0:
            self.s_sim.wait(self.sub_done[(self.sim_next - 1) % len(self.sub_done)])

    def after_force(self):
        if self.sim_on_lanes:
            self.force_done.record(self.s_sim)
            self.force_pending = True

    def _ws(self, k):
        lane = k % self.lanes
        return lane, lane * self.depth + (k // self.lanes) % self.depth

    def _advance_simulator(self, upto):
        b, S = self.b, self.slots
        while self.sim_next <= upto:
            g = self.sim_next
            slot = g % S
            s = self.s_lane[g % self.lanes] if self.sim_on_lanes else self.s_sim
            if self.sim_on_lanes:
                if g > 0:
                    s.wait(self.sub_done[(g - 1) % len(self.sub_done)])
                if self.force_pending:
                    s.wait(self.force_done)
                    self.force_pending = False
            if self.bc_used[slot]:
                s.wait(self.bc_done[slot])
            if self.ip_used[slot]:
                s.wait(self.ip_done[slot])
            b.snapshot(s, slot)
            self.snap_ready[slot].record(s)
            b.substep(s)
            if self.sim_on_lanes:
                self.sub_done[g % len(self.sub_done)].record(s)
            self.sim_next += 1

    def _broadcasts(self, upto):
        b, S = self.b, self.slots
        while self.bc_next <= upto:
            slot = self.bc_next % S
            if self.rank == self.owner:
                self.s_comm.wait(self.snap_ready[slot])
            elif self.ip_used[slot]:
                self.s_comm.wait(self.ip_done[slot])
            b.broadcast(self.s_comm, slot, self.owner)
            self.bc_done[slot].record(self.s_comm)
            self.bc_used[slot] = True
            self.bc_next += 1

    def retire(self, ws):
        f = self.pending[ws]
        if f is None:
            return None
        b = self.b
        (self.out_ready if self.copy_out else self.render_done)[ws].host_wait()
        if not b.complete(ws):
            b.finish(ws)
        self.pending[ws] = None
        res = b.result(ws)
        if self.on_retire is not None:
            self.on_retire(f, res)
            fence = getattr(b, "consumer_fence", None)
            if fence is not None:
                fence(ws)
        return f, res

    def step(self, pose=None):
        b, f, S = self.b, self.frame, self.slots
        self.retired = []
        if self.rank == self.owner:
            self._advance_simulator(f + self.ahead)
        if self.collectives:
            self._broadcasts(f + self.ahead)
        mine = frame_owner(f, self.world, self.owner, self.dedicated) == self.rank
        if mine:
            lane, ws = self._ws(self.my_frames)
            done = self.retire(ws)
            if done is not None:
                self.retired.append(done)
            slot = f % S
            s = self.s_lane[lane]
            s.wait(self.bc_done[slot] if self.collectives else self.snap_ready[slot])
            b.render(s, f, ws, slot, pose)
            self.ip_done[slot].record(s)
            self.ip_used[slot] = True
            self.render_done[ws].record(s)
            if self.copy_out:
                where = getattr(b, "copy_on", "copy")
                sc = s if where == "lane" else (self.s_sim if where == "sim" else self.s_copy)
                if sc is not s:
                    sc.wait(self.render_done[ws])
                b.copy_out(sc, ws)
                self.out_ready[ws].record(sc)
            self.pending[ws] = f
            self.last_ws, self.last_frame = ws, f
            self.my_frames += 1
        elif self.dedicated and self.rank == self.owner and self.world > 1:
            self.bc_done[f % S].host_wait()
        self.frame += 1
        return self.retired

    def drain(self):
        out = [self.retire(ws) for ws in range(self.lanes * self.depth)]
        out = sorted(r for r in out if r is not None)
        self.retired = out
        return out

    @property
    def substeps_enqueued(self):
        return self.sim_next


class _SimEvent:
    def __init__(self, be):
        self.be, self.stream, self.pos = be, None, -1

    def record(self, stream):
        self.stream, self.pos = stream, len(stream.ops) + stream.base
        stream.ops.append(("record", self, None))

    def host_wait(self):
        self.be.run_until(self)


class _SimStream:
    def __init__(self, name):
        self.name, self.ops, self.base, self.executed = name, [], 0, 0

    def wait(self, event):
        self.ops.append(("wait", (event.stream, event.pos), None))


class SimulatedBackend:

    def __init__(self, world, rank, n_dof=64, owner=0, seed=0, needs_more_trips=lambda frame: False, group=None):
        self.world, self.rank, self.owner, self.group = world, rank, owner, group
        self.rng = random.Random(seed * 1000 + rank)
        self.streams = {}
        self.dof = torch.arange(n_dof, dtype=torch.float64) * (1.0 if rank == owner else -7.0)
        self.steps = 0
        self.snap, self.snap_tag = {}, {}
        self.readers_left = {}
        self.ws_out, self.ws_host, self.ws_trips_short = {}, {}, {}
        self.needs_more_trips = needs_more_trips
        self.log = []

    def stream(self, name):
        return self.streams.setdefault(name, _SimStream(name))

    def event(self):
        return _SimEvent(self)

    def _enqueue(self, s, what, fn):
        s.ops.append(("op", what, fn))

    def _ready(self, s):
        if not s.ops:
            return False
        kind, a, _ = s.ops[0]
        return kind != "wait" or a[0] is None or a[0].executed > a[1]

    def _run_one(self, s):
        kind, a, fn = s.ops.pop(0)
        s.base += 1
        if kind == "op":
            fn()
        s.executed += 1

    def run_until(self, event):
        guard = 0
        while not (event.stream is None or event.stream.executed > event.pos):
            ready = [s for s in self.streams.values() if self._ready(s)]
            assert ready, f"deadlock: nothing can run while waiting for a point of stream {event.stream.name}"
            pick = event.stream if (event.stream in ready and self.rng.random() < 0.5) else self.rng.choice(ready)
            self._run_one(pick)
            guard += 1
            assert guard < 10_000_000

    def flush(self):
        while True:
            ready = [s for s in self.streams.values() if self._ready(s)]
            if not ready:
                break
            self._run_one(self.rng.choice(ready))
        assert all(not s.ops for s in self.streams.values()), "operations left that can never run"

    def snapshot(self, s, slot):
        g = self._sim_enq = getattr(self, "_sim_enq", 0)
        self._sim_enq += 1

        def run():
            prev = self.snap_tag.get(slot)
            assert self.steps == g, f"snapshot of frame {g} taken after {self.steps} substeps"
            assert self.readers_left.get((slot, prev), 0) == 0, f"snapshot slot {slot} overwritten with frame {g} while frame {prev} still has readers"
            self.snap[slot] = self.dof.clone()
            self.snap_tag[slot] = g
        self._enqueue(s, f"snapshot {g}", run)

    def substep(self, s):
        def run():
            self.dof = self.dof * 1.01 + 0.5
            self.steps += 1
        self._enqueue(s, "substep", run)

    def broadcast(self, s, slot, src):
        g = self._bc_enq = getattr(self, "_bc_enq", 0)
        self._bc_enq += 1

        def run():
            if self.rank == src:
                assert self.snap_tag.get(slot) == g, f"broadcast of frame {g} finds frame {self.snap_tag.get(slot)} in slot {slot}"
                buf = self.snap[slot]
            else:
                prev = self.snap_tag.get(slot)
                assert self.readers_left.get((slot, prev), 0) == 0, f"slot {slot} received frame {g} while frame {prev} still has readers"
                buf = self.snap.setdefault(slot, torch.empty_like(self.dof))
            dist.broadcast(buf, src=src, group=self.group)
            self.snap_tag[slot] = g
        self._enqueue(s, f"broadcast {g}", run)

    def render(self, s, frame, ws, slot, pose):
        key = (slot, frame)
        self.readers_left[key] = self.readers_left.get(key, 0) + 1

        def run():
            assert self.snap_tag.get(slot) == frame, f"frame {frame} rendered from slot {slot} holding frame {self.snap_tag.get(slot)}"
            self.readers_left[key] -= 1
            short = bool(self.needs_more_trips(frame))
            self.ws_out[ws] = (frame, float(self.snap[slot].sum()), None if pose is None else float(pose), "partial" if short else "full")
            self.ws_trips_short[ws] = short
            self.log.append(frame)
        self._enqueue(s, f"render {frame}", run)

    def copy_out(self, s, ws):
        def run():
            self.ws_host[ws] = self.ws_out[ws]
        self._enqueue(s, f"copy_out {ws}", run)

    def complete(self, ws):
        return not self.ws_trips_short[ws]

    def finish(self, ws):
        f, v, p, _ = self.ws_out[ws]
        self.ws_out[ws] = self.ws_host[ws] = (f, v, p, "full")
        self.ws_trips_short[ws] = False

    def result(self, ws):
        return self.ws_host.get(ws, self.ws_out.get(ws))
```

### pienerf_amd/harness.py

```python
import contextlib
import gc
import os

import numpy as np
import torch

from . import scene
from .nerf.network import NeRFNetwork
from .nerf.utils import get_rays
from .simulator.solver import Simulator


@contextlib.contextmanager
def _capture(graph, **kw):
    gc.collect()
    was = gc.isenabled()
    gc.disable()
    try:
        with torch.cuda.graph(graph, capture_error_mode="thread_local", **kw):
            yield
    finally:
        if was:
            gc.enable()


THROUGHPUT_FORM_MIN_RAYS = 131072

class SimRenderHarness:
    def __init__(self, opt=None, cloud=None, ckpt=None, device="cuda", overlap_sim=True):
        self.opt = dict(opt or scene.default_opt())
        o = self.opt
        self.device = torch.device(device)
        self.cloud = cloud if cloud is not None else scene.make_chair_points(hgs=o["hash_grid_size"], bound=o["bound"])
        self.ckpt = ckpt if ckpt is not None else scene.make_checkpoint(bound=o["bound"], bg_radius=o["bg_radius"])
        self.model = NeRFNetwork(encoding="hashgrid", bound=o["bound"], cuda_ray=True, density_scale=1, min_near=o["min_near"],
                                 density_thresh=o["density_thresh"], bg_radius=o["bg_radius"]).to(self.device)
        self.model.load_checkpoint_dict(self.ckpt)
        self.model.eval()
        self.sim = Simulator(dt=o["sim_dt"], iters=o["sim_iters"], bbox=torch.tensor([2.0 * o["bound"]] * 3), dx=o["sim_dx"], stiff=o["sim_stiff"],
                             base=torch.tensor([-o["bound"]] * 3), device=self.device)
        c = self.cloud
        self.sim.InitializeFromArrays(c["pos"], c["mass"], c["mu"], c["lam"], c["pin"])
        IP_pos, IP_F, IP_dF = self.sim.get_IP_info()
        m = self.model
        m.p_ori, m.p_def, m.IP_F, m.IP_dF = IP_pos, IP_pos, IP_F, IP_dF
        m.IP_dx = self.sim.dx * 1.05
        self.frame = 0
        self.pose = scene.orbit_pose(o["radius"])
        self.intrinsics = scene.orbit_intrinsics(o["W"], o["H"], o["fovy"])
        self._pose_dev = None
        self.overlap_sim = overlap_sim
        if overlap_sim:
            self._sim_stream = torch.cuda.Stream(self.device)
            self._ip_ready = torch.cuda.Event()
            self._sim_done = torch.cuda.Event()
            self._sim_done.record(torch.cuda.current_stream(self.device))
            self.sim.force_stream = self._sim_stream

    def synchronize(self):
        torch.cuda.synchronize(self.device)
        self._check_persistent_substep()

    def _amp(self):
        return torch.autocast("cuda", dtype=torch.float16, enabled=bool(self.opt.get("fp16", False)))

    def render_kwargs(self):
        return dict(self.opt)

    @torch.no_grad()
    def step(self, pose=None, intrinsics=None, W=None, H=None, simulate=True, collect_stats=False, fused=True, render_kw=None):
        o = self.opt
        W, H = W or o["W"], H or o["H"]
        pose = self.pose if pose is None else pose
        intrinsics = self.intrinsics if intrinsics is None else intrinsics
        key = np.asarray(pose, np.float32).tobytes()
        if self._pose_dev is None or self._pose_dev[0] != key:
            self._pose_dev = (key, torch.from_numpy(np.asarray(pose, np.float32)).unsqueeze(0).to(self.device))
        rays = get_rays(self._pose_dev[1], intrinsics, H, W, -1)
        m = self.model
        if simulate:
            main = torch.cuda.current_stream(self.device)
            if self.overlap_sim:
                main.wait_event(self._sim_done)
            IP_pos, IP_F, IP_dF = self.sim.get_IP_info()
            m.p_def, m.IP_F, m.IP_dF = IP_pos, IP_F, IP_dF
            if self.overlap_sim:
                self._ip_ready.record(main)
                self._sim_stream.wait_event(self._ip_ready)
                with torch.cuda.stream(self._sim_stream):
                    self.sim.stepforward()
                    self._sim_done.record(self._sim_stream)
            else:
                self.sim.stepforward()
            self.frame += 1
        kw = self.render_kwargs()
        kw.update(render_kw or {})
        kw["collect_stats"] = collect_stats
        with self._amp():
            if fused:
                out = m.render_deformed(rays["rays_o"], rays["rays_d"], staged=True, bg_color=None, perturb=False, **kw)
            else:
                out = m.rund_cuda_ops(rays["rays_o"], rays["rays_d"], bg_color=None, perturb=False, **kw)
        if self.sim.drag_enabled:
            self._drag_frame = ("eager", out["depth_0"].reshape(H, W), m.p_def, pose, intrinsics)
        return {"image": out["image"].reshape(-1, H, W, 3), "depth": out["depth"].reshape(-1, H, W), "depth_0": out["depth_0"].reshape(-1, H, W),
                "rays_o": rays["rays_o"], "rays_d": rays["rays_d"]}

    def _step_body(self, n_trips, W, H):
        m = self.model
        main = torch.cuda.current_stream(self.device)
        rays = get_rays(self._graph_pose, self.intrinsics, H, W, -1)
        IP_pos, IP_F, IP_dF = self.sim.get_IP_info()
        m.p_def, m.IP_F, m.IP_dF = IP_pos, IP_F, IP_dF
        self._sim_stream.wait_stream(main)
        with torch.cuda.stream(self._sim_stream):
            self.sim.stepforward()
        kw = self.render_kwargs()
        kw["async_trips"] = n_trips
        with self._amp():
            out = m.render_deformed(rays["rays_o"], rays["rays_d"], staged=True, bg_color=None, perturb=False, **kw)
        main.wait_stream(self._sim_stream)
        return {"image": out["image"].reshape(-1, H, W, 3), "depth": out["depth"].reshape(-1, H, W), "depth_0": out["depth_0"].reshape(-1, H, W),
                "weights_sum": out["weights_sum"], "rays_o": rays["rays_o"], "rays_d": rays["rays_d"], "_ip": (IP_pos, IP_F, IP_dF)}

    @torch.no_grad()
    def capture(self, n_trips=8, W=None, H=None):
        o = self.opt
        W, H = W or o["W"], H or o["H"]
        if not hasattr(self, "_sim_stream"):
            self._sim_stream = torch.cuda.Stream(self.device)
        self._graph_pose = torch.from_numpy(np.asarray(self.pose, np.float32)).unsqueeze(0).to(self.device)
        self._graph_pose_host = self.pose
        keep = (self.sim.dof.clone(), self.sim.dof_vel.clone())
        warm = torch.cuda.Stream(self.device)
        warm.wait_stream(torch.cuda.current_stream(self.device))
        with torch.cuda.stream(warm):
            for _ in range(2):
                self._step_body(n_trips, W, H)
        torch.cuda.current_stream(self.device).wait_stream(warm)
        torch.cuda.synchronize(self.device)
        self._graph = torch.cuda.CUDAGraph()
        with _capture(self._graph):
            self._graph_out = self._step_body(n_trips, W, H)
        self.sim.dof.copy_(keep[0])
        self.sim.dof_vel.copy_(keep[1])
        self.sim.reset_warm_start()
        self._graph_trips = n_trips
        self._graph_done = None
        self._graph_drag = self.sim.drag_enabled
        self._graph_form_epoch = self._net_form_epoch()
        return self

    def _net_form_epoch(self):
        from ._lib import lib
        net = getattr(self.model, "_net", None)
        return int(lib().pn_net_form_epoch(net)) if net is not None else 0

    def _check_net_form(self, captured, what):
        if self._net_form_epoch() != captured:
            raise RuntimeError(f"the network's weights were refreshed into another arithmetic form (pn_net_form) since {what} was captured: its graphs "
                               f"hold the old form's kernels — capture again")

    @torch.no_grad()
    def step_graph(self, pose=None):
        if getattr(self, "_graph", None) is None:
            self.capture()
        self._check_net_form(self._graph_form_epoch, "the step")
        self._check_previous_graph_frame()
        if pose is not None:
            self._graph_pose.copy_(torch.from_numpy(np.asarray(pose, np.float32)).unsqueeze(0))
        self._graph.replay()
        self._graph_done = torch.cuda.Event()
        self._graph_done.record(torch.cuda.current_stream(self.device))
        self.frame += 1
        if pose is not None:
            self._graph_pose_host = pose
        if self._graph_drag:
            g = self._graph_out
            self._drag_frame = ("graph", g["depth_0"][0], g["_ip"][0], self._graph_pose_host, self.intrinsics)
        else:
            self._drag_frame = ("graph",)
        return self._graph_out

    def finish_graph_frame(self):
        self._check_previous_graph_frame()
        return self._graph_out

    def _check_previous_graph_frame(self):
        if getattr(self, "_graph_done", None) is not None:
            self._graph_done.synchronize()
            st = self.model.render_status(synchronize=False)
            self._graph_done = None
            if st["alive_at_exit"] > 0:
                g = self._graph_out
                with self._amp():
                    self.model.render_continue(0, g["rays_o"], g["rays_d"], g, bg_color=None, **self.render_kwargs())
                self.graph_continued = getattr(self, "graph_continued", 0) + 1

    def _cu_masked_stream(self, first_cu, n_cu, invert):
        import ctypes

        from ._lib import check, lib
        total = lib().pn_device_cu_count()
        h = ctypes.c_void_p()
        with torch.cuda.device(self.device):
            check(lib().pn_stream_create_cu_mask(total, first_cu, n_cu, int(invert), ctypes.byref(h)), "stream_create_cu_mask")
        self._raw_streams = getattr(self, "_raw_streams", []) + [h.value]
        return torch.cuda.ExternalStream(h.value, device=self.device)

    @torch.no_grad()
    def capture_pipelined(self, lanes=2, n_trips=8, W=None, H=None, sim_ahead=None, depth=2, sim_priority=0, sim_cus=0, copy_out=True, group=None,
                          frame_parallel=False, sim_owner=0, dedicated_sim=None, on_retire=None, copy_on="host", _probe_no_substep=False, _time_trips=False,
                          render_kw=None, _force_collectives=False, sim_on_lanes=False):
        import torch.distributed as dist

        from .frames import FramePipeline
        o = self.opt
        W, H = W or o["W"], H or o["H"]
        on = bool(frame_parallel) and dist.is_available() and dist.is_initialized()
        world = dist.get_world_size(group) if on else 1
        rank = dist.get_rank(group) if on else 0
        if n_trips is None:
            self.step(simulate=False, collect_stats=True, W=W, H=H)
            n_trips = int(self.model.last_stats["trips"]) + 2
        from .frames import dedicated_sim_default
        if (world > 1 and (dedicated_sim_default(world) if dedicated_sim is None else bool(dedicated_sim)) and rank == sim_owner
                and dist.get_backend(group) == "nccl" and os.environ.get("PN_SIM_COOP", "") == "1"):
            self.sim.enable_persistent()
        be = _HipBackend(self, lanes, depth, int(n_trips), W, H, sim_priority, sim_cus, copy_out, group if on else None,
                         (dist.get_global_rank(group, sim_owner) if (on and group is not None) else sim_owner), _probe_no_substep, _time_trips, copy_on,
                         render_kw=render_kw, distributed=on)
        self._pipe = FramePipeline(be, world=world, rank=rank, lanes=lanes, depth=depth, ahead=(lanes if sim_ahead is None and world == 1 else sim_ahead),
                                   sim_owner=sim_owner, dedicated_sim=dedicated_sim, copy_out=copy_out, on_retire=on_retire,
                                   force_collectives=bool(_force_collectives) and on, sim_on_lanes=sim_on_lanes)
        self.sim.force_hooks = (self._pipe.before_force, self._pipe.after_force) if self._pipe.sim_on_lanes else None
        self._pipe_drag = self.sim.drag_enabled
        self._drag_frame = ("pipelined",)
        self._pipe_backend = be
        self._pipe_form_epoch = self._net_form_epoch()
        self.model._in_flight = lambda pipe=self._pipe: sum(f is not None for f in pipe.pending)
        return self

    def capture_frame_parallel(self, lanes=2, n_trips=8, group=None, sim_owner=0, dedicated_sim=None, **kw):
        return self.capture_pipelined(lanes=lanes, n_trips=n_trips, group=group, frame_parallel=True, sim_owner=sim_owner, dedicated_sim=dedicated_sim, **kw)

    @torch.no_grad()
    def step_pipelined(self, pose=None):
        self._check_net_form(self._pipe_form_epoch, "the pipeline")
        out = self._pipe.step(pose)
        self.frame = self._pipe.frame
        return out

    step_frame_parallel = step_pipelined

    @property
    def substeps_enqueued(self):
        return self._pipe.substeps_enqueued

    @torch.no_grad()
    def drain_pipeline(self):
        out = self._pipe.drain()
        torch.cuda.synchronize(self.device)
        self._check_persistent_substep()
        return out

    def wait_frame_copies(self):
        torch.cuda.synchronize(self.device)
        be = getattr(self, "_pipe_backend", None)
        if be is not None and hasattr(be, "wait_copies"):
            be.wait_copies()

    @torch.no_grad()
    def verify_last_frame(self):
        pipe, be, m = self._pipe, self._pipe_backend, self.model
        ws = pipe.last_ws
        if ws is None:
            return {"ok": False, "frame": None, "why": "no frame was enqueued"}
        torch.cuda.synchronize(self.device)
        res = be.result(ws)
        keep = (m.p_def, m.IP_F, m.IP_dF)
        try:
            m.p_def, m.IP_F, m.IP_dF = be.ip[ws]
            rays = get_rays(be.pose_dev[ws], self.intrinsics, be.H, be.W, -1)
            kw = dict(self.render_kwargs())
            kw.pop("ray_batch", None)
            if be.kw.get("ray_batch"):
                kw["ray_batch"] = be.kw["ray_batch"]
            with self._amp():
                out = m.render_deformed(rays["rays_o"], rays["rays_d"], staged=True, bg_color=None, perturb=False, **kw)
            torch.cuda.synchronize(self.device)
            worst, ok = 0.0, True
            for k in ("image", "depth_0"):
                want = out[k].reshape(-1).cpu().numpy()
                got = (res[k] if k in res else res["device"][k].cpu().numpy()).reshape(-1)
                ok = ok and bool(np.array_equal(want, got))
                worst = max(worst, float(np.abs(want - got).max()))
        finally:
            m.p_def, m.IP_F, m.IP_dF = keep
        return {"ok": ok, "frame": int(pipe.last_frame), "max_abs_diff": worst}

    def _check_persistent_substep(self):
        if self.sim.persistent and self.sim.persistent_timed_out():
            raise RuntimeError("the persistent substep (pn_sim_stepforward_coop) timed out at a device-wide barrier: the simulator state is invalid "
                               "(another kernel held CUs for seconds, or two persistent substeps ran at once); use Simulator(persistent=False)")

    @torch.no_grad()
    def capture_tile_parallel(self, group=None, sim_owner=0, tile=8, W=None, H=None, _force_collectives=False):
        from .frames import TileParallel
        o, m, dev = self.opt, self.model, self.device
        W, H = W or o["W"], H or o["H"]
        ip = tuple(torch.empty((self.sim.n_IP, c), dtype=torch.float32, device=dev) for c in (3, 9, 27))
        self._tile_pose = torch.from_numpy(np.asarray(self.pose, np.float32)).unsqueeze(0).to(dev)

        def render_subset(idx):
            rays = get_rays(self._tile_pose, self.intrinsics, H, W, -1)
            sel = idx.clamp(min=0)
            self.sim.get_IP_info(out=ip)
            m.p_def, m.IP_F, m.IP_dF = ip
            with self._amp():
                out = m.render_deformed(rays["rays_o"][:, sel].contiguous(), rays["rays_d"][:, sel].contiguous(), bg_color=None, perturb=False, frame_slot=800,
                                        **self.render_kwargs())
            return torch.cat([out["image"].view(-1, 3), out["depth"].view(-1, 1), out["depth_0"].view(-1, 1)], dim=1)

        def set_dof(t):
            self.sim.dof.copy_(t)
        self._tile = TileParallel(W, H, render_subset, lambda: self.sim.dof, set_dof, self.sim.stepforward, sim_owner=sim_owner, group=group, tile=tile, device=dev,
                                  force_collectives=_force_collectives)
        self._tile_WH = (W, H)
        return self

    @torch.no_grad()
    def step_tile_parallel(self, pose=None):
        if pose is not None:
            self._tile_pose.copy_(torch.from_numpy(np.asarray(pose, np.float32)).view(1, 4, 4).to(self.device))
        full = self._tile.step()
        W, H = self._tile_WH
        self.frame += 1
        return {"image": full[:, :3].reshape(1, H, W, 3), "depth": full[:, 3].reshape(1, H, W), "depth_0": full[:, 4].reshape(1, H, W)}

    def capture_staged(self, batch=None, **kw):
        rk = dict(kw.pop("render_kw", None) or {}, ray_batch=int(batch or self.opt.get("max_ray_batch", 4096)))
        return self.capture_pipelined(render_kw=rk, **kw)

    def step_staged(self, pose=None):
        return self.step_pipelined(pose)

    def finish_staged(self):
        return self.drain_pipeline()

    def enable_drag(self, scale=None):
        self.sim.enable_drag(scale)
        return self

    def _drag_check(self):
        if not self.sim.drag_enabled:
            raise RuntimeError("drag: call enable_drag() first (before capture() / capture_pipelined())")
        mode = getattr(self, "_drag_frame", None)
        if mode is None:
            raise RuntimeError("drag: no frame has been rendered yet (the cursor is unprojected against the last frame's depth_0)")
        if mode[0] == "graph" and not getattr(self, "_graph_drag", False):
            raise RuntimeError("drag: the step graph was captured before enable_drag(), its substep ignores the drag state: capture() again")
        if mode[0] == "pipelined" and not getattr(self, "_pipe_drag", False):
            raise RuntimeError("drag: the pipeline was captured before enable_drag(), its substep ignores the drag state: capture_pipelined() again")
        return mode

    def _drag_inputs(self, depth0, ip_pos, pick):
        mode = self._drag_check()
        if mode[0] == "pipelined":
            if depth0 is None:
                raise ValueError("drag in the pipelined form: pass depth0, the depth_0 of the last frame step_pipelined() returned")
            depth0 = torch.as_tensor(depth0).to(self.device, torch.float32).contiguous()
            if pick and ip_pos is None:
                with self.sim._on_force_stream():
                    ip_pos = self.sim.get_IP_info()[0]
            return depth0, ip_pos, self.pose, self.intrinsics
        if mode[0] == "graph":
            self._check_previous_graph_frame()
        return (mode[1] if depth0 is None else depth0), (mode[2] if ip_pos is None else ip_pos), mode[3], mode[4]

    def drag(self, x, y, depth0=None, ip_pos=None):
        d, ip, pose, intr = self._drag_inputs(depth0, ip_pos, True)
        return self.sim.drag_pick(d, x, y, pose, intr, ip)

    def move(self, x, y, depth0=None):
        d, _, pose, intr = self._drag_inputs(depth0, None, False)
        self.sim.drag_to(d, x, y, pose, intr)

    def release(self):
        self._drag_check()
        self.sim.release()

    def to_host(self, out):
        return {k: out[k][0].detach().cpu().numpy() for k in ("image", "depth", "depth_0")}


class _HipStream:
    def __init__(self, s):
        self.s = s

    def wait(self, ev):
        self.s.wait_event(ev.e)


class _HostCopyStream:

    def __init__(self, backend):
        self.backend, self.after, self.ticket = backend, None, None

    def wait(self, ev):
        self.after = ev


class _HipEvent:
    def __init__(self):
        self.e = torch.cuda.Event()
        self.copy = None

    def record(self, stream):
        if isinstance(stream, _HostCopyStream):
            self.copy = (stream.backend.copier, stream.ticket)
        else:
            self.copy = None
            self.e.record(stream.s)

    def host_wait(self):
        if self.copy is not None:
            from ._lib import check, lib
            check(lib().pn_copier_wait(self.copy[0], self.copy[1]), "copier_wait")
        else:
            self.e.synchronize()


class _HipBackend:

    def __init__(self, h, lanes, depth, n_trips, W, H, sim_priority, sim_cus, copy_out, group, src, probe_no_substep, time_trips=False, copy_on="host",
                 render_kw=None, distributed=False):
        self.copy_on = copy_on
        self.copier = None
        if copy_on == "host" and copy_out:
            import ctypes

            from ._lib import check, lib
            hc = ctypes.c_void_p()
            check(lib().pn_copier_create(ctypes.byref(hc)), "copier_create")
            self.copier = hc
        self.h, self.lanes, self.depth, self.trips, self.W, self.H, self.group, self.src = h, lanes, depth, n_trips, W, H, group, src
        dev, m, sim = h.device, h.model, h.sim
        self.continued = 0
        if sim_cus > 0:
            self._streams = {"sim": h._cu_masked_stream(0, sim_cus, invert=False)}
            lane_streams = [h._cu_masked_stream(0, sim_cus, invert=True) for _ in range(lanes)]
        elif sim_cus < 0:
            self._streams = {"sim": torch.cuda.Stream(dev, priority=sim_priority)}
            lane_streams = [h._cu_masked_stream(0, -sim_cus, invert=True) for _ in range(lanes)]
        else:
            self._streams = {"sim": torch.cuda.Stream(dev, priority=sim_priority)}
            lane_streams = [torch.cuda.Stream(dev) for _ in range(lanes)]
        for i, s in enumerate(lane_streams):
            self._streams[f"lane{i}"] = s
        self._streams["comm"], self._streams["copy"] = torch.cuda.Stream(dev), torch.cuda.Stream(dev)
        sim.force_stream = self._streams["sim"]
        self.snap = {}
        n_ws, n_IP = lanes * depth, sim.n_IP
        self.consumer_done = [None] * n_ws
        kw = dict(h.render_kwargs(), async_trips=n_trips)
        kw.update(render_kw or {})
        kw.setdefault("march_throughput", 64 if lanes > 1 else 0)
        if lanes > 1:
            cus = torch.cuda.get_device_properties(dev).multi_processor_count
            kw.setdefault("fused_grid", max(cus * 5 // 8 if lanes == 2 else cus // 2, 1))
        self.kw = kw
        if "fused_from" not in kw:
            h.step(simulate=False, collect_stats=True, W=W, H=H)
            recs = m.trip_records(slot=0, max_trips=64)
            kw["fused_from"] = next((i for i, r in enumerate(recs) if i >= 1 and r[1] == 8), -1) if not kw.get("ray_batch") else -1
        if "fused_whole" not in kw:
            whole = lanes == 2 and kw["fused_from"] == 1
            if whole:
                h.step(simulate=False, collect_stats=True, W=W, H=H, render_kw=dict(kw, fused_whole=True, fused_from=0, async_trips=0))
                whole = m.fused_clocks(slot=0)["first_trip"] == 0
            kw["fused_whole"] = bool(whole)
            if whole:
                kw["fused_from"] = 0
        if "fused_fold" not in kw:
            fold = lanes >= 3 and (not kw.get("fused_whole")) and kw["fused_from"] == 1
            if fold:
                h.step(simulate=False, collect_stats=True, W=W, H=H, render_kw=dict(kw, fused_fold=True, async_trips=0))
                fold = m.fused_clocks(slot=0)["mode"] == 2
            kw["fused_fold"] = bool(fold)
        if distributed:
            from .frames import agree_on_launch_form
            agree_on_launch_form(kw, src=src, group=group, device=dev)
        pose0 = torch.from_numpy(np.asarray(h.pose, np.float32)).unsqueeze(0)
        self.pose_dev = [pose0.to(dev) for _ in range(n_ws)]
        self.pose_pin = [pose0.clone().pin_memory() for _ in range(n_ws)]
        self.pose_key = [pose0.numpy().tobytes()] * n_ws
        self.ip = [tuple(torch.empty((n_IP, c), dtype=torch.float32, device=dev) for c in (3, 9, 27)) for _ in range(n_ws)]
        keep = (sim.dof.clone(), sim.dof_vel.clone())
        main = torch.cuda.current_stream(dev)
        for ws in range(n_ws):
            s = self._streams[f"lane{ws // depth}"]
            s.wait_stream(main)
            with torch.cuda.stream(s):
                for _ in range(2):
                    sim.get_IP_info(out=self.ip[ws])
                    sim.stepforward()
                    m.p_def, m.IP_F, m.IP_dF = self.ip[ws]
                    rays = get_rays(self.pose_dev[ws], h.intrinsics, H, W, -1)
                    with h._amp():
                        m.render_deformed(rays["rays_o"], rays["rays_d"], staged=True, bg_color=None, perturb=False, **dict(kw, frame_slot=ws))
            torch.cuda.synchronize(dev)
            if ws == 0 and kw.get("march_throughput") and "march_throughput_trips" not in kw:
                n_lpr = 1
                for rec in m.trip_records(slot=0)[1:]:
                    if rec[0] < THROUGHPUT_FORM_MIN_RAYS:
                        break
                    n_lpr += 1
                kw["march_throughput_trips"] = n_lpr
        self.sim_graph = torch.cuda.CUDAGraph()
        with _capture(self.sim_graph, stream=self._streams["sim"]):
            if not probe_no_substep:
                sim.stepforward()
            else:
                sim.dof_vel.mul_(1.0)
        self.graph, self.rays, self.out, self.host, self.packed = [], [], [], [], []
        N = W * H
        for ws in range(n_ws):
            s = self._streams[f"lane{ws // depth}"]
            m.p_def, m.IP_F, m.IP_dF = self.ip[ws]
            if time_trips:
                m.march_counters(2, slot=ws)
            pk = torch.empty(N * 5, dtype=torch.float32, device=dev)
            ob = {"image": pk[:3 * N].view(N, 3), "depth": pk[3 * N:4 * N], "depth_0": pk[4 * N:], "weights_sum": torch.empty(N, dtype=torch.float32, device=dev)}
            g = torch.cuda.CUDAGraph()
            with _capture(g, stream=s):
                rays = get_rays(self.pose_dev[ws], h.intrinsics, H, W, -1)
                with h._amp():
                    out = m.render_deformed(rays["rays_o"], rays["rays_d"], staged=True, bg_color=None, perturb=False, out_buffers=ob, **dict(kw, frame_slot=ws))
            self.graph.append(g)
            self.rays.append(rays)
            self.out.append(out)
            self.packed.append(pk)
            self.host.append([torch.empty(N * 5, dtype=torch.float32).pin_memory() for _ in range(2)] if copy_out else None)
        self.host_gen = [0] * n_ws
        torch.cuda.synchronize(dev)
        if self.copier is not None:
            import ctypes

            from ._lib import check, lib
            for ws in range(n_ws):
                for hb in self.host[ws]:
                    t = ctypes.c_uint64()
                    check(lib().pn_copier_submit(self.copier, ctypes.c_void_p(hb.data_ptr()), ctypes.c_void_p(self.packed[ws].data_ptr()),
                                                 hb.numel() * hb.element_size(), None, ctypes.byref(t)), "copier_submit")
                    check(lib().pn_copier_wait(self.copier, t.value), "copier_wait")
        sim.dof.copy_(keep[0])
        sim.dof_vel.copy_(keep[1])
        sim.reset_warm_start()
        torch.cuda.synchronize(dev)

    def stream(self, name):
        if name == "copy" and self.copier is not None:
            return _HostCopyStream(self)
        return _HipStream(self._streams[name])

    def __del__(self):
        if getattr(self, "copier", None) is not None:
            try:
                from ._lib import lib
                lib().pn_copier_destroy(self.copier)
            except Exception:
                pass
            self.copier = None

    def event(self):
        return _HipEvent()

    def _snap(self, slot):
        if slot not in self.snap:
            self.snap[slot] = torch.empty_like(self.h.sim.dof)
        return self.snap[slot]

    def snapshot(self, s, slot):
        with torch.cuda.stream(s.s):
            self._snap(slot).copy_(self.h.sim.dof)

    def substep(self, s):
        with torch.cuda.stream(s.s):
            self.sim_graph.replay()

    def broadcast(self, s, slot, src):
        import torch.distributed as dist
        with torch.cuda.stream(s.s):
            dist.broadcast(self._snap(slot), src=self.src, group=self.group)

    def consumer_fence(self, ws):
        ev = torch.cuda.Event()
        ev.record(torch.cuda.current_stream(self.h.device))
        self.consumer_done[ws] = ev

    def render(self, s, frame, ws, slot, pose):
        with torch.cuda.stream(s.s):
            if self.consumer_done[ws] is not None:
                s.s.wait_event(self.consumer_done[ws])
                self.consumer_done[ws] = None
            p = np.ascontiguousarray(self.h.pose if pose is None else pose, dtype=np.float32).reshape(1, 4, 4)
            key = p.tobytes()
            if self.pose_key[ws] != key:
                self.pose_key[ws] = key
                self.pose_pin[ws].copy_(torch.from_numpy(p))
                self.pose_dev[ws].copy_(self.pose_pin[ws], non_blocking=True)
            self.h.sim.get_IP_info(dof=self._snap(slot), out=self.ip[ws])
            self.graph[ws].replay()

    def copy_out(self, s, ws, same_buffer=False):
        if not same_buffer:
            self.host_gen[ws] ^= 1
        dst, src = self.host[ws][self.host_gen[ws]], self.packed[ws]
        if isinstance(s, _HostCopyStream):
            import ctypes

            from ._lib import check, lib
            t = ctypes.c_uint64()
            after = ctypes.c_void_p(s.after.e.cuda_event) if s.after is not None else None
            check(lib().pn_copier_submit(self.copier, ctypes.c_void_p(dst.data_ptr()), ctypes.c_void_p(src.data_ptr()), src.numel() * src.element_size(), after,
                                         ctypes.byref(t)), "copier_submit")
            s.ticket = t.value
            self.last_ticket = t.value
            return
        with torch.cuda.stream(s.s):
            dst.copy_(src, non_blocking=True)

    def wait_copies(self):
        if self.copier is not None and getattr(self, "last_ticket", None) is not None:
            from ._lib import check, lib
            check(lib().pn_copier_wait(self.copier, self.last_ticket), "copier_wait")

    def complete(self, ws):
        return self.h.model.render_status(synchronize=False, slot=ws)["alive_at_exit"] == 0

    def finish(self, ws):
        h, m = self.h, self.h.model
        s = self._streams[f"lane{ws // self.depth}"]
        with torch.cuda.stream(s):
            with h._amp():
                m.render_continue(ws, self.rays[ws]["rays_o"], self.rays[ws]["rays_d"], self.out[ws], bg_color=None, **self.kw)
            if self.host[ws] is not None:
                self.copy_out(_HipStream(s), ws, same_buffer=True)
        s.synchronize()
        self.continued += 1
        if self.continued == 8:
            import warnings
            warnings.warn("8 frames of this pipeline had rays alive behind their captured trips and were finished by blocking renders: the launch form picked "
                          "at capture no longer fits the scene / pose — capture_pipelined() again from the current state", RuntimeWarning, stacklevel=2)

    def result(self, ws):
        o = self.out[ws]
        H, W, N = self.H, self.W, self.H * self.W
        dev = {"image": o["image"].view(-1, H, W, 3), "depth": o["depth"].view(-1, H, W), "depth_0": o["depth_0"].view(-1, H, W)}
        if self.host[ws] is None:
            return {"device": dev}
        hb = self.host[ws][self.host_gen[ws]].numpy()
        return {"image": hb[:3 * N].reshape(H, W, 3), "depth": hb[3 * N:4 * N].reshape(H, W), "depth_0": hb[4 * N:].reshape(H, W), "device": dev}
```

### pienerf_amd/nerf/renderer.py

```python
import ctypes as C
import math

import torch
import torch.nn as nn

from .. import raymarching
from .._lib import RenderOpts, check, lib, ptr, require_gpu, stream_ptr
from .utils import get_pnts_in_grids


def _flat_rays(rays_o, rays_d):
    return rays_o.to(torch.float32).contiguous().view(-1, 3), rays_d.to(torch.float32).contiguous().view(-1, 3)


def sample_pdf(bins, weights, n_samples, det=False):
    if weights.shape[-1] < 1:
        raise RuntimeError("sample_pdf: no bin weights (the hierarchical sampler needs num_steps >= 3: weights[:, 1:-1] is empty)")
    weights = weights + 1e-5
    pdf = weights / torch.sum(weights, -1, keepdim=True)
    cdf = torch.cumsum(pdf, -1)
    cdf = torch.cat([torch.zeros_like(cdf[..., :1]), cdf], -1)
    if det:
        u = torch.linspace(0. + 0.5 / n_samples, 1. - 0.5 / n_samples, steps=n_samples).to(weights.device)
        u = u.expand(list(cdf.shape[:-1]) + [n_samples])
    else:
        u = torch.rand(list(cdf.shape[:-1]) + [n_samples]).to(weights.device)
    u = u.contiguous()
    inds = torch.searchsorted(cdf, u, right=True)
    below = torch.clamp(inds - 1, min=0)
    above = torch.clamp(inds, max=cdf.shape[-1] - 1)
    cdf_lo, cdf_hi = torch.gather(cdf, -1, below), torch.gather(cdf, -1, above)
    bins_lo, bins_hi = torch.gather(bins, -1, below), torch.gather(bins, -1, above)
    denom = cdf_hi - cdf_lo
    denom = torch.where(denom < 1e-5, torch.ones_like(denom), denom)
    t = (u - cdf_lo) / denom
    return bins_lo + t * (bins_hi - bins_lo)


class NeRFRenderer(nn.Module):
    def __init__(self, bound=1, cuda_ray=False, density_scale=1, min_near=0.2, density_thresh=0.01, bg_radius=-1):
        super().__init__()
        self.bound = bound
        self.cascade = 1 + math.ceil(math.log2(bound))
        self.grid_size = 128
        self.density_scale = density_scale
        self.min_near = min_near
        self.density_thresh = density_thresh
        self.bg_radius = bg_radius
        aabb = torch.FloatTensor([-bound, -bound, -bound, bound, bound, bound])
        self.register_buffer("aabb_train", aabb)
        self.register_buffer("aabb_infer", aabb.clone())
        self.cuda_ray = cuda_ray
        if cuda_ray:
            self.register_buffer("density_grid", torch.zeros([self.cascade, self.grid_size ** 3]))
            self.register_buffer("density_bitfield", torch.zeros(self.cascade * self.grid_size ** 3 // 8, dtype=torch.uint8))
            self.register_buffer("step_counter", torch.zeros(16, 2, dtype=torch.int32))
            self.mean_density = 0
            self.iter_density = 0
            self.mean_count = 0
            self.local_step = 0
        self._frame = None
        self._frames = {}
        self.last_stats = None

    def forward(self, x, d):
        raise NotImplementedError()

    def density(self, x):
        raise NotImplementedError()

    def color(self, x, d, mask=None, **kwargs):
        raise NotImplementedError()

    def _net_handle(self, half=False):
        raise NotImplementedError()

    def background(self, x, d):
        raise NotImplementedError()

    def blend_background(self, rays_o, rays_d, weights_sum, image):
        raise NotImplementedError()

    @staticmethod
    def _autocast_half():
        return False

    def render_deformed(self, rays_o, rays_d, staged=False, max_ray_batch=4096, **kwargs):
        if not self.cuda_ray:
            raise RuntimeError("render_deformed: only the cuda_ray path (main_gui.py / main_render.py with -O) is implemented")
        return self.rund_cuda(rays_o, rays_d, **kwargs)

    def _ip_state(self, device):
        return [t.to(device=device, dtype=torch.float32).contiguous() for t in (self.p_def, self.p_ori, self.IP_F, self.IP_dF)]

    def _frame_handle(self, N, n_vtx, hgs, slot=0, cells=None):
        side = int(math.ceil(2.2 * float(self.bound) / hgs)) + 2
        cells = side ** 3 if cells is None else int(cells)
        key = (N, n_vtx, cells)
        cur = self._frames.get(slot)
        if cur is None or cur[1] != key:
            if cur is not None:
                lib().pn_frame_destroy(cur[0])
            h = C.c_void_p()
            check(lib().pn_frame_create(C.byref(h), N, n_vtx, cells), "frame_create")
            self._frames[slot] = (h, key)
        if slot == 0:
            self._frame = self._frames[0][0]
        return self._frames[slot][0]

    def _deformed_opts(self, dt_gamma, bg_scalar, max_steps, T_thresh, kwargs, n_rays=0):
        o = RenderOpts()
        o.max_iter_num = int(kwargs.get("max_iter_num"))
        o.hash_grid_size = float(kwargs.get("hash_grid_size"))
        o.num_seek_IP = int(kwargs.get("num_seek_IP"))
        o.IP_dx = float(self.IP_dx)
        o.cut = int(bool(kwargs.get("cut")))
        cb = kwargs.get("cut_bounds") or [0.0] * 6
        for i in range(6):
            o.cut_bounds[i] = float(cb[i])
        o.bound = float(kwargs.get("bound", self.bound))
        o.min_near = float(self.min_near)
        o.dt_gamma = float(dt_gamma)
        o.max_steps = int(max_steps)
        o.T_thresh = float(T_thresh)
        o.cascade = int(self.cascade)
        o.grid_size = int(self.grid_size)
        o.density_scale = float(self.density_scale)
        o.bg_color = float(bg_scalar)
        o.fp16 = int(self._autocast_half())
        o.reuse_tables = int(bool(kwargs.get("reuse_tables")))
        o.ray_batch = int(kwargs.get("ray_batch") or 0)
        o.throughput = int(kwargs.get("march_throughput") or 0)
        o.throughput_trips = int(kwargs.get("march_throughput_trips") or 0)
        tw = kwargs.get("ray_tile_w")
        if tw is None and n_rays and kwargs.get("W") and kwargs.get("H") and int(kwargs["W"]) * int(kwargs["H"]) == n_rays:
            tw = kwargs["W"]
        o.ray_tile_w = int(tw or 0)
        o.fused_from = int(kwargs.get("fused_from") or 0)
        o.fused_grid = int(kwargs.get("fused_grid") or 0)
        o.fused_fold = int(bool(kwargs.get("fused_fold")))
        o.fused_whole = int(bool(kwargs.get("fused_whole")))
        return o

    def _static_opts(self, dt_gamma, bg_scalar, max_steps, T_thresh):
        o = RenderOpts()
        o.max_iter_num, o.hash_grid_size, o.num_seek_IP, o.IP_dx, o.cut = 1, 1.0, 1, 0.0, 0
        o.bound, o.min_near, o.dt_gamma, o.max_steps, o.T_thresh = float(self.bound), float(self.min_near), float(dt_gamma), int(max_steps), float(T_thresh)
        o.cascade, o.grid_size, o.density_scale, o.bg_color = int(self.cascade), int(self.grid_size), float(self.density_scale), float(bg_scalar)
        o.fp16 = int(self._autocast_half())
        return o

    def rund_cuda(self, rays_o, rays_d, dt_gamma=0, bg_color=None, perturb=False, max_steps=1024, T_thresh=1e-2, **kwargs):
        if perturb:
            return self.rund_cuda_ops(rays_o, rays_d, dt_gamma, bg_color, perturb, max_steps, T_thresh, **kwargs)
        prefix = rays_o.shape[:-1]
        rays_o, rays_d = _flat_rays(rays_o, rays_d)
        require_gpu(rays_o, rays_d)
        N, device = rays_o.shape[0], rays_o.device
        if self.bg_radius > 0:
            bg_color = 0
        if bg_color is None:
            bg_color = 1
        bg_tensor = bg_color.to(device=device, dtype=torch.float32) if torch.is_tensor(bg_color) else None
        p_def, p_ori, F_IP, dF_IP = self._ip_state(device)
        assert p_def.shape == p_ori.shape and p_ori.shape[0] > 0
        n_vtx = p_ori.shape[0]
        o = self._deformed_opts(dt_gamma, 0.0 if bg_tensor is not None else bg_color, max_steps, T_thresh, kwargs, n_rays=N)
        ob = kwargs.get("out_buffers")
        if ob is not None:
            image, depth, depth_0, weights_sum = ob["image"], ob["depth"], ob["depth_0"], ob["weights_sum"]
            assert image.shape == (N, 3) and depth.shape == (N,) and all(t.is_contiguous() and t.dtype == torch.float32 for t in (image, depth, depth_0, weights_sum))
        else:
            image = torch.empty(N, 3, dtype=torch.float32, device=device)
            depth = torch.empty(N, dtype=torch.float32, device=device)
            depth_0 = torch.empty(N, dtype=torch.float32, device=device)
            weights_sum = torch.empty(N, dtype=torch.float32, device=device)
        async_trips = int(kwargs.get("async_trips") or 0)
        frame, net = self._frame_handle(N, n_vtx, o.hash_grid_size, int(kwargs.get("frame_slot") or 0)), self._net_handle(half=bool(o.fp16))
        if async_trips > 0:
            check(lib().pn_render_deformed_async(frame, net, C.byref(o), ptr(rays_o), ptr(rays_d), N, ptr(p_def), ptr(p_ori), ptr(F_IP), ptr(dF_IP),
                                                 n_vtx, ptr(self.density_bitfield), ptr(image), ptr(depth), ptr(depth_0), ptr(weights_sum),
                                                 async_trips, stream_ptr()), "render_deformed_async")
        else:
            stats = (C.c_int64 * 5)() if kwargs.get("collect_stats") else None
            check(lib().pn_render_deformed(frame, net, C.byref(o), ptr(rays_o), ptr(rays_d), N, ptr(p_def), ptr(p_ori), ptr(F_IP), ptr(dF_IP), n_vtx,
                                           ptr(self.density_bitfield), ptr(image), ptr(depth), ptr(depth_0), ptr(weights_sum), stats, stream_ptr()),
                  "render_deformed")
            if stats is not None:
                self._set_stats(stats)
        if self.bg_radius > 0:
            self.blend_background(rays_o, rays_d, weights_sum, image)
        elif bg_tensor is not None:
            image = image + (1 - weights_sum).unsqueeze(-1) * bg_tensor
        return {"depth": depth.view(*prefix), "image": image.view(*prefix, 3), "depth_0": depth_0.view(*prefix), "weights_sum": weights_sum}

    def render_continue(self, slot, rays_o, rays_d, out, n_trips=0, dt_gamma=0, bg_color=None, max_steps=1024, T_thresh=1e-2, static=False, **kwargs):
        rays_o, rays_d = _flat_rays(rays_o, rays_d)
        N = rays_o.shape[0]
        if self.bg_radius > 0:
            bg_color = 0
        if static:
            o = self._static_opts(dt_gamma, 1 if bg_color is None else bg_color, max_steps, T_thresh)
        else:
            o = self._deformed_opts(dt_gamma, 1 if bg_color is None else bg_color, max_steps, T_thresh, kwargs, n_rays=N)
        image, depth, ws = out["image"].view(-1, 3), out["depth"].view(-1), out["weights_sum"].view(-1)
        depth_0 = out["depth_0"].view(-1) if "depth_0" in out else torch.empty_like(depth)
        assert image.is_contiguous() and image.shape[0] == N
        stats = (C.c_int64 * 5)() if int(n_trips) == 0 else None
        check(lib().pn_render_continue(self._frames[slot][0], self._net_handle(half=bool(o.fp16)), C.byref(o), ptr(rays_o), ptr(rays_d), N,
                                       ptr(self.density_bitfield), ptr(image), ptr(depth), ptr(depth_0), ptr(ws), stats, int(n_trips), int(bool(static)),
                                       stream_ptr()), "render_continue")
        if self.bg_radius > 0:
            self.blend_background(rays_o, rays_d, ws, image)
        if stats is not None:
            self._set_stats(stats)
        return out

    def _set_stats(self, stats):
        self.last_stats = dict(trips=int(stats[0]), samples=int(stats[1]), err=int(stats[2]), alive_at_exit=int(stats[3]), unfinished=int(stats[4]))
        if stats[2]:
            raise RuntimeError(f"render_deformed: device error flags {int(stats[2])} (1: sample cell outside the spatial hash, "
                               "2: IP outside it, 4: spatial-hash capacity exceeded, 8: candidate-list capacity exceeded, "
                               "16: the fused composite/compaction gave up waiting for an earlier chunk, 32: the fused launch found its kernarg segment laid "
                               "out otherwise than csrc/pn_trips_fused.h: fused_karg_fresh assumes)")

    def march_counters(self, enable, read=False, slot=0):
        out = (C.c_uint64 * 4)() if read else None
        check(lib().pn_frame_march_counters(self._frames[slot][0], int(enable), out, stream_ptr()), "march_counters")
        return None if out is None else dict(iterations=int(out[0]), candidates=int(out[1]), warps=int(out[2]), samples=int(out[3]))

    def fused_clocks(self, slot=0, reset=False):
        out, first = (C.c_uint64 * 16)(), C.c_int(-1)
        check(lib().pn_frame_fused_clocks(self._frames[slot][0], out, C.byref(first), int(bool(reset)), stream_ptr()), "fused_clocks")
        return dict(refill=int(out[0]), march=int(out[1]), windows=int(out[2]), network=int(out[3]), composite=int(out[4]), wave_rounds=int(out[5]),
                    waves=int(out[6]), lifetime_ticks=int(out[7]), max_rounds=int(out[8]), max_lifetime_ticks=int(out[9]), first_trip=int(first.value),
                    a_march=int(out[10]), a_windows=int(out[11]), a_network=int(out[12]), a_composite=int(out[13]), a_barrier=int(out[14]),
                    mode=int(out[15]))

    def trip_records(self, slot=0, max_trips=16):
        rec, tail = (C.c_int * (5 * max_trips))(), (C.c_int * max_trips)()
        check(lib().pn_frame_trip_records(self._frames[slot][0], rec, tail, max_trips, stream_ptr()), "trip_records")
        return [tuple(rec[5 * i:5 * i + 5]) + (tail[i],) for i in range(max_trips) if rec[5 * i] > 0]

    def trip_times(self, slot=0):
        a, b, n = (C.c_float * 64)(), (C.c_float * 64)(), C.c_int(0)
        check(lib().pn_frame_trip_times(self._frames[slot][0], a, b, 64, C.byref(n), stream_ptr()), "trip_times")
        return [float(a[i]) for i in range(n.value)], [float(b[i]) for i in range(n.value)]

    def render_status(self, synchronize=True, slot=0):
        stats = (C.c_int64 * 5)()
        check(lib().pn_render_status(self._frames[slot][0], stats, int(bool(synchronize)), stream_ptr()), "render_status")
        self._set_stats(stats)
        return self.last_stats

    def reset_extra_state(self):
        if not self.cuda_ray:
            return
        self.density_grid.zero_()
        self.mean_density = 0
        self.iter_density = 0
        self.step_counter.zero_()
        self.mean_count = 0
        self.local_step = 0

    def run_cuda(self, rays_o, rays_d, dt_gamma=0, bg_color=None, perturb=False, force_all_rays=False, max_steps=1024, T_thresh=1e-2, **kwargs):
        if not self.training and not perturb and (self.bg_radius > 0 or not torch.is_tensor(bg_color)):
            return self._run_static_fused(rays_o, rays_d, dt_gamma, 1 if bg_color is None else bg_color, max_steps, T_thresh, **kwargs)
        return self.run_cuda_ops(rays_o, rays_d, dt_gamma, bg_color, perturb, force_all_rays, max_steps, T_thresh, **kwargs)

    def _run_static_fused(self, rays_o, rays_d, dt_gamma, bg_color, max_steps, T_thresh, **kwargs):
        prefix = rays_o.shape[:-1]
        rays_o, rays_d = _flat_rays(rays_o, rays_d)
        require_gpu(rays_o, rays_d)
        if self.bg_radius > 0:
            bg_color = 0
        N, device = rays_o.shape[0], rays_o.device
        o = self._static_opts(dt_gamma, bg_color, max_steps, T_thresh)
        aabb = (C.c_float * 6)(*self._aabb_infer_host())
        image, depth, depth_0, ws = (torch.empty(N, 3, dtype=torch.float32, device=device), torch.empty(N, dtype=torch.float32, device=device),
                                     torch.empty(N, dtype=torch.float32, device=device), torch.empty(N, dtype=torch.float32, device=device))
        frame = self._frame_handle(N, 1, 1.0, int(kwargs.get("frame_slot") or 0), cells=1)
        async_trips = int(kwargs.get("async_trips") or 0)
        stats = (C.c_int64 * 5)() if not async_trips else None
        check(lib().pn_render_static(frame, self._net_handle(half=bool(o.fp16)), C.byref(o), ptr(rays_o), ptr(rays_d), N, aabb, ptr(self.density_bitfield),
                                     ptr(image), ptr(depth), ptr(depth_0), ptr(ws), stats, async_trips, stream_ptr()), "render_static")
        if self.bg_radius > 0:
            self.blend_background(rays_o, rays_d, ws, image)
        if stats is not None:
            self._set_stats(stats)
        return {"depth": depth.view(*prefix), "image": image.view(*prefix, 3), "weights_sum": ws}

    def _aabb_infer_host(self):
        key = (self.aabb_infer.data_ptr(), self.aabb_infer._version)
        if getattr(self, "_aabb_cache", (None, None))[0] != key:
            if torch.cuda.is_current_stream_capturing():
                raise RuntimeError("aabb_infer changed: render one frame outside stream capture first")
            self._aabb_cache = (key, [float(v) for v in self.aabb_infer.tolist()])
        return self._aabb_cache[1]

    def run_cuda_ops(self, rays_o, rays_d, dt_gamma=0, bg_color=None, perturb=False, force_all_rays=False, max_steps=1024, T_thresh=1e-2, **kwargs):
        shape = rays_o.shape[:-1]
        o3, d3 = rays_o.contiguous().view(-1, 3), rays_d.contiguous().view(-1, 3)
        nears, fars = raymarching.near_far_from_aabb(o3, d3, self.aabb_train if self.training else self.aabb_infer, self.min_near)
        if self.bg_radius > 0:
            bg_color = self.background(raymarching.sph_from_ray(o3, d3, self.bg_radius), d3)
        bg = 1 if bg_color is None else bg_color

        def shade(xyzs, dirs):
            sig, rgb = self(xyzs, dirs)
            return self.density_scale * sig, rgb

        if self.training:
            slot = self.step_counter[self.local_step % 16]
            slot.zero_()
            self.local_step += 1
            xyzs, dirs, deltas, rays = raymarching.march_rays_train(o3, d3, self.bound, self.density_bitfield, self.cascade, self.grid_size, nears, fars, slot,
                                                                    self.mean_count, perturb, 128, force_all_rays, dt_gamma, max_steps)
            ws, depth, image = raymarching.composite_rays_train(*shade(xyzs, dirs), deltas, rays, T_thresh)
            self.last_stats = dict(trips=1, samples=int(xyzs.shape[0]), err=0, alive_at_exit=0)
        else:
            with torch.no_grad():
                n_rays, dev = o3.shape[0], o3.device
                ws, depth, image = (torch.zeros(n_rays, device=dev), torch.zeros(n_rays, device=dev), torch.zeros(n_rays, 3, device=dev))
                alive, t_now = torch.arange(n_rays, dtype=torch.int32, device=dev), nears.clone()
                done_steps = trips = samples = 0
                while done_steps < max_steps and alive.shape[0] > 0:
                    k = alive.shape[0]
                    per_ray = max(min(n_rays // k, 8), 1)
                    xyzs, dirs, deltas = raymarching.march_rays(k, per_ray, alive, t_now, o3, d3, self.bound, self.density_bitfield, self.cascade,
                                                                self.grid_size, nears, fars, 128, perturb if done_steps == 0 else False, dt_gamma, max_steps)
                    raymarching.composite_rays(k, per_ray, alive, t_now, *shade(xyzs, dirs), deltas, ws, depth, image, T_thresh)
                    alive = raymarching.compact_rays(alive)
                    samples += int((deltas[:, 0] != 0).sum())
                    done_steps += per_ray
                    trips += 1
                self.last_stats = dict(trips=trips, samples=samples, err=0, alive_at_exit=int(alive.shape[0]))
        image = image + (1 - ws).unsqueeze(-1) * bg
        depth = torch.clamp(depth - nears, min=0) / (fars - nears)
        return {"depth": depth.view(*shape), "image": image.view(*shape, 3), "weights_sum": ws}

    def render(self, rays_o, rays_d, staged=False, max_ray_batch=4096, **kwargs):
        if self.cuda_ray:
            return self.run_cuda(rays_o, rays_d, **kwargs)
        if not staged:
            return self.run(rays_o, rays_d, **kwargs)
        if self._hier_fused_ok(rays_o, **kwargs):
            out = self.run(rays_o, rays_d, **kwargs)
            return {"depth": out["depth"], "image": out["image"]}
        B, N = rays_o.shape[:2]
        depth = torch.empty((B, N), device=rays_o.device)
        image = torch.empty((B, N, 3), device=rays_o.device)
        for b in range(B):
            for head in range(0, N, max_ray_batch):
                tail = min(head + max_ray_batch, N)
                part = self.run(rays_o[b:b + 1, head:tail], rays_d[b:b + 1, head:tail], **kwargs)
                depth[b:b + 1, head:tail] = part["depth"]
                image[b:b + 1, head:tail] = part["image"]
        return {"depth": depth, "image": image}

    @staticmethod
    def _check_hier_steps(num_steps, upsample_steps):
        if int(num_steps) < 1 or int(upsample_steps) < 0:
            raise RuntimeError(f"run: num_steps = {num_steps}, upsample_steps = {upsample_steps}")
        if int(upsample_steps) > 0 and int(num_steps) < 3:
            raise RuntimeError(f"run: upsample_steps = {upsample_steps} needs num_steps >= 3 (got {num_steps}): sample_pdf is handed weights[:, 1:-1], "
                               "which is empty, and the reference fails inside it")

    def _hier_fused_ok(self, rays_o, num_steps=128, upsample_steps=128, bg_color=None, perturb=False, **kwargs):
        if self.training or perturb or torch.is_grad_enabled() or self._autocast_half():
            return False
        if int(num_steps) + int(upsample_steps) > int(lib().pn_hier_max_samples()):
            return False
        if self.bg_radius > 0 or not torch.is_tensor(bg_color):
            return True
        n = rays_o.numel() // 3
        return tuple(bg_color.shape) in ((3,), (n, 3))

    def run(self, rays_o, rays_d, num_steps=128, upsample_steps=128, bg_color=None, perturb=False, **kwargs):
        self._check_hier_steps(num_steps, upsample_steps)
        if self._hier_fused_ok(rays_o, num_steps, upsample_steps, bg_color, perturb):
            return self._run_hier_fused(rays_o, rays_d, int(num_steps), int(upsample_steps), bg_color)
        return self.run_ops(rays_o, rays_d, num_steps, upsample_steps, bg_color, perturb, **kwargs)

    def _run_hier_fused(self, rays_o, rays_d, num_steps, upsample_steps, bg_color):
        prefix = rays_o.shape[:-1]
        rays_o, rays_d = _flat_rays(rays_o, rays_d)
        require_gpu(rays_o, rays_d)
        N, device = rays_o.shape[0], rays_o.device
        bg_rays, bg_scalar = None, 1.0
        if self.bg_radius > 0:
            bg_scalar = 0.0
        elif torch.is_tensor(bg_color):
            bg_rays = bg_color.to(device=device, dtype=torch.float32).expand(N, 3).contiguous()
        elif bg_color is not None:
            bg_scalar = float(bg_color)
        image = torch.empty(N, 3, dtype=torch.float32, device=device)
        depth = torch.empty(N, dtype=torch.float32, device=device)
        ws = torch.empty(N, dtype=torch.float32, device=device)
        aabb = (C.c_float * 6)(*self._aabb_infer_host())
        check(lib().pn_render_hier(self._net_handle(), ptr(rays_o), ptr(rays_d), N, aabb, float(self.min_near), num_steps, upsample_steps,
                                   float(self.density_scale), bg_scalar, ptr(bg_rays), ptr(image), ptr(depth), ptr(ws), 0, stream_ptr()), "render_hier")
        if self.bg_radius > 0 and N > 0:
            self.blend_background(rays_o, rays_d, ws, image)
        return {"depth": depth.view(*prefix), "image": image.view(*prefix, 3), "weights_sum": ws}

    def run_ops(self, rays_o, rays_d, num_steps=128, upsample_steps=128, bg_color=None, perturb=False, **kwargs):
        self._check_hier_steps(num_steps, upsample_steps)
        prefix = rays_o.shape[:-1]
        rays_o = rays_o.contiguous().view(-1, 3)
        rays_d = rays_d.contiguous().view(-1, 3)
        require_gpu(rays_o, rays_d)
        N, device = rays_o.shape[0], rays_o.device
        aabb = self.aabb_train if self.training else self.aabb_infer
        nears, fars = raymarching.near_far_from_aabb(rays_o, rays_d, aabb, self.min_near)
        nears, fars = nears.unsqueeze(-1), fars.unsqueeze(-1)
        z_vals = torch.linspace(0.0, 1.0, num_steps, device=device).unsqueeze(0).expand((N, num_steps))
        z_vals = nears + (fars - nears) * z_vals
        sample_dist = (fars - nears) / num_steps
        if perturb:
            z_vals = z_vals + (torch.rand(z_vals.shape, device=device) - 0.5) * sample_dist
        xyzs = rays_o.unsqueeze(-2) + rays_d.unsqueeze(-2) * z_vals.unsqueeze(-1)
        xyzs = torch.min(torch.max(xyzs, aabb[:3]), aabb[3:])

        def weights_of(z, sigma):
            deltas = z[..., 1:] - z[..., :-1]
            deltas = torch.cat([deltas, sample_dist * torch.ones_like(deltas[..., :1])], dim=-1)
            alphas = 1 - torch.exp(-deltas * self.density_scale * sigma)
            shifted = torch.cat([torch.ones_like(alphas[..., :1]), 1 - alphas + 1e-15], dim=-1)
            return deltas, alphas * torch.cumprod(shifted, dim=-1)[..., :-1]

        dens = {k: v.view(N, num_steps, -1) for k, v in self.density(xyzs.reshape(-1, 3)).items()}
        if upsample_steps > 0:
            with torch.no_grad():
                deltas, weights = weights_of(z_vals, dens["sigma"].squeeze(-1))
                z_mid = z_vals[..., :-1] + 0.5 * deltas[..., :-1]
                new_z = sample_pdf(z_mid, weights[:, 1:-1], upsample_steps, det=not self.training).detach()
                new_xyzs = rays_o.unsqueeze(-2) + rays_d.unsqueeze(-2) * new_z.unsqueeze(-1)
                new_xyzs = torch.min(torch.max(new_xyzs, aabb[:3]), aabb[3:])
            new_dens = {k: v.view(N, upsample_steps, -1) for k, v in self.density(new_xyzs.reshape(-1, 3)).items()}
            z_vals, z_index = torch.sort(torch.cat([z_vals, new_z], dim=1), dim=1)
            xyzs = torch.cat([xyzs, new_xyzs], dim=1)
            xyzs = torch.gather(xyzs, dim=1, index=z_index.unsqueeze(-1).expand_as(xyzs))
            for k in dens:
                both = torch.cat([dens[k], new_dens[k]], dim=1)
                dens[k] = torch.gather(both, dim=1, index=z_index.unsqueeze(-1).expand_as(both))
        _, weights = weights_of(z_vals, dens["sigma"].squeeze(-1))
        dirs = rays_d.view(-1, 1, 3).expand_as(xyzs)
        dens = {k: v.reshape(-1, v.shape[-1]) for k, v in dens.items()}
        mask = weights > 1e-4
        rgbs = self.color(xyzs.reshape(-1, 3), dirs.reshape(-1, 3), mask=mask.reshape(-1), **dens).view(N, -1, 3)
        weights_sum = weights.sum(dim=-1)
        ori_z_vals = ((z_vals - nears) / (fars - nears)).clamp(0, 1)
        depth = torch.sum(weights * ori_z_vals, dim=-1)
        image = torch.sum(weights.unsqueeze(-1) * rgbs, dim=-2)
        if self.bg_radius > 0:
            bg_color = self.background(raymarching.sph_from_ray(rays_o, rays_d, self.bg_radius), rays_d.reshape(-1, 3))
        elif bg_color is None:
            bg_color = 1
        image = image + (1 - weights_sum).unsqueeze(-1) * bg_color
        return {"depth": depth.view(*prefix), "image": image.view(*prefix, 3), "weights_sum": weights_sum}

    @torch.no_grad()
    def mark_untrained_grid(self, poses, intrinsic, S=64):
        if not self.cuda_ray:
            return
        cams = torch.as_tensor(poses).to(device=self.density_grid.device, dtype=torch.float32).contiguous().view(-1, 4, 4)
        require_gpu(cams, self.density_grid)
        fx, fy, cx, cy = (float(v) for v in intrinsic)
        n_unseen = torch.zeros(1, dtype=torch.int32, device=cams.device)
        check(lib().pn_mark_untrained_grid(ptr(cams), cams.shape[0], fx, fy, cx, cy, self.cascade, self.grid_size, float(self.bound),
                                           ptr(self.density_grid), ptr(n_unseen), stream_ptr()), "mark_untrained_grid")
        return int(n_unseen.item())

    @torch.no_grad()
    def update_extra_state(self, decay=0.95, S=128):
        if not self.cuda_ray:
            return
        grid = self.density_grid
        dev, H, n_cas = grid.device, self.grid_size, self.cascade
        require_gpu(grid)
        cells = H ** 3
        net, half = self._net_handle(half=self._autocast_half()), int(self._autocast_half())
        tmp = torch.empty_like(grid)
        if self.iter_density < 16:
            pts = torch.empty(n_cas * cells, 3, dtype=torch.float32, device=dev)
            check(lib().pn_density_cells_full(n_cas, H, float(self.bound), ptr(torch.rand(n_cas * cells, 3, device=dev)), ptr(pts), stream_ptr()), "density_cells_full")
            check(lib().pn_nerf_sigma(net, ptr(pts), n_cas * cells, float(self.density_scale), ptr(tmp), half, stream_ptr()), "nerf_sigma")
        else:
            n = cells // 4
            scratch = torch.empty(int(lib().pn_density_partial_scratch_ints(H)), dtype=torch.int32, device=dev)
            pts = torch.empty(2 * n, 3, dtype=torch.float32, device=dev)
            idx = torch.empty(2 * n, dtype=torch.int32, device=dev)
            sig = torch.empty(2 * n, dtype=torch.float32, device=dev)
            for cas in range(n_cas):
                draws = torch.randint(0, H, (n, 3), device=dev, dtype=torch.int32)
                check(lib().pn_density_cells_partial(cas, H, float(self.bound), n, ptr(draws), ptr(torch.rand(n, device=dev)), ptr(torch.rand(2 * n, 3, device=dev)),
                                                     ptr(grid[cas]), ptr(tmp[cas]), ptr(scratch), ptr(idx), ptr(pts), stream_ptr()), "density_cells_partial")
                check(lib().pn_nerf_sigma(net, ptr(pts), 2 * n, float(self.density_scale), ptr(sig), half, stream_ptr()), "nerf_sigma")
                check(lib().pn_density_scatter(2 * n, ptr(idx), ptr(sig), ptr(tmp[cas]), stream_ptr()), "density_scatter")
        partial = torch.empty((n_cas * cells + 255) // 256, dtype=torch.float64, device=dev)
        mean_thresh = torch.empty(2, dtype=torch.float32, device=dev)
        check(lib().pn_density_grid_update(n_cas * cells, ptr(grid), ptr(tmp), float(decay), float(self.density_thresh), ptr(self.density_bitfield),
                                           ptr(partial), ptr(mean_thresh), stream_ptr()), "density_grid_update")
        self.mean_density = float(mean_thresh[0].item())
        self.iter_density += 1
        counted = min(16, self.local_step)
        if counted > 0:
            self.mean_count = int(self.step_counter[:counted, 0].sum().item() / counted)
        self.local_step = 0

    def rund_cuda_ops(self, rays_o, rays_d, dt_gamma=0, bg_color=None, perturb=False, max_steps=1024, T_thresh=1e-2, **kwargs):
        dtype = torch.float32
        prefix = rays_o.shape[:-1]
        rays_o = rays_o.contiguous().view(-1, 3)
        rays_d = rays_d.contiguous().view(-1, 3)
        N, device = rays_o.shape[0], rays_o.device
        max_iter_num, hgs, bound = kwargs.get("max_iter_num"), kwargs.get("hash_grid_size"), kwargs.get("bound")
        cut = kwargs.get("cut")
        cut_bounds = torch.tensor(kwargs.get("cut_bounds") or [0.0] * 6, dtype=dtype, device=device)
        p_def, p_ori, F_IP, dF_IP = self._ip_state(device)
        bmin, bmax = p_def.min(axis=0).values, p_def.max(axis=0).values
        if cut:
            bmin = -bound * torch.ones(3, dtype=dtype, device=device)
            bmax = bound * torch.ones(3, dtype=dtype, device=device)
        marg = 1e-3
        bbmin = bmin - marg * torch.ones(3, dtype=dtype, device=device)
        bbmax = bmax + marg * torch.ones(3, dtype=dtype, device=device)
        resolution = torch.ceil((bbmax - bbmin) / hgs).to(torch.int32)
        aabb = torch.cat((bbmin, bbmax), dim=0)
        nears, fars = raymarching.near_far_from_aabb(rays_o, rays_d, aabb, self.min_near)
        if self.bg_radius > 0:
            bg_color = self.background(raymarching.sph_from_ray(rays_o, rays_d, self.bg_radius), rays_d)
        elif bg_color is None:
            bg_color = 1
        weights_sum = torch.zeros(N, dtype=dtype, device=device)
        depth = torch.zeros(N, dtype=dtype, device=device)
        image = torch.zeros(N, 3, dtype=dtype, device=device)
        num_seek_IP = kwargs.get("num_seek_IP")
        n_vtx = p_ori.shape[0]
        n_grid = int(resolution[2] * resolution[1] * resolution[0])
        assert p_def.shape == p_ori.shape and n_vtx > 0
        pig_cnt, pig_bgn, pig_idx = get_pnts_in_grids(n_vtx, n_grid, p_def, bbmin, bbmax, hgs, resolution)
        rays_alive = torch.arange(N, dtype=torch.int32, device=device)
        rays_t = nears.clone()
        step, trips, samples = 0, 0, 0
        while step < max_steps:
            n_alive = rays_alive.shape[0]
            if n_alive <= 0:
                break
            n_step = max(min(N // n_alive, 8), 1)
            xyzs, dirs, deltas = raymarching.march_rays_quadratic_bending(
                pig_cnt, pig_bgn, pig_idx, n_vtx, n_grid, p_def, p_ori, F_IP, dF_IP, max_iter_num, bbmin, bbmax, hgs, resolution, num_seek_IP,
                self.IP_dx, cut, cut_bounds, n_alive, n_step, rays_alive, rays_t, rays_o, rays_d, self.bound, self.density_bitfield, self.cascade,
                self.grid_size, nears, fars, 128, perturb if step == 0 else False, dt_gamma, max_steps)
            sigmas, rgbs = self(xyzs, dirs)
            sigmas = self.density_scale * sigmas
            raymarching.composite_rays(n_alive, n_step, rays_alive, rays_t, sigmas, rgbs, deltas, weights_sum, depth, image, T_thresh)
            rays_alive = raymarching.compact_rays(rays_alive)
            samples += int((deltas[:, 0] != 0).sum())
            step += n_step
            trips += 1
        self.last_stats = dict(trips=trips, samples=samples, err=0, alive_at_exit=int(rays_alive.shape[0]))
        depth_0 = depth
        image = image + (1 - weights_sum).unsqueeze(-1) * bg_color
        depth = torch.clamp(depth - nears, min=0) / (fars - nears)
        return {"depth": depth.view(*prefix), "image": image.view(*prefix, 3), "depth_0": depth_0.view(*prefix), "weights_sum": weights_sum}
```

Measured before the change: 1485.

## Build deformation tables ahead on sim stream and generate camera rays in prologue

Adds a separate table-build entry point that constructs the per-frame deformation lookup tables (point-in-grid lists, neighbour ranges, records, grid regions) in its own captured graph on the sim stream. The render prologue then skips that work when the tables are already built. It also fuses camera ray generation into the frame prologue kernel, removing the separate get_rays launch from the render graph. The intent is to move table building off the render lane's critical path and overlap it with rendering. The cost is extra graph state and key checks, and stale tables become possible if the frame slot's inputs change between the build and the render.

```diff
diff --git a/include/pienerf_hip.h b/include/pienerf_hip.h
--- a/include/pienerf_hip.h
+++ b/include/pienerf_hip.h
@@ -161,6 +161,16 @@
 int pn_render_deformed_async(pn_frame* f, const pn_net* net, const pn_render_opts* opts, const float* rays_o, const float* rays_d, uint32_t N,
                              const float* p_def, const float* p_ori, const float* F_IP, const float* dF_IP, int n_vtx, const uint8_t* bitfield,
                              float* image, float* depth, float* depth_0, float* weights_sum, int n_trips, void* stream);
+int pn_frame_build_tables(pn_frame* f, const pn_render_opts* opts, const float* p_def, const float* p_ori, const float* F_IP, const float* dF_IP,
+                          int n_vtx, const uint8_t* bitfield, void* stream);
+int pn_frame_tables_ahead(const pn_frame* f, uint32_t* generation_out);
+int pn_frame_drop_tables(pn_frame* f);
+int pn_frame_set_camera(pn_frame* f, const float* pose, float fx, float fy, float cx, float cy, int H, int W);
+enum { PN_TABLE_PIG_CNT = 0, PN_TABLE_PIG_BGN, PN_TABLE_PIG_IDX, PN_TABLE_NB_RNG , PN_TABLE_NB ,
+       PN_TABLE_REC , PN_TABLE_CELL_BITS , PN_TABLE_GRID_REGIONS,
+       PN_TABLE_FRAME_RECORD , PN_TABLE_NEARS, PN_TABLE_FARS };
+int pn_frame_read_table(pn_frame* f, int which, void* dst_host, uint64_t bytes, uint64_t* bytes_total, void* stream);
+
 int pn_render_status(pn_frame* f, int64_t* stats_host, int synchronize, void* stream);
 int pn_frame_reset_unfinished(pn_frame* f, void* stream);
 
diff --git a/pienerf_amd/_lib.py b/pienerf_amd/_lib.py
--- a/pienerf_amd/_lib.py
+++ b/pienerf_amd/_lib.py
@@ -74,6 +74,11 @@
     "pn_frame_destroy": (None, [P]),
     "pn_render_deformed": (i32, [P, P, C.POINTER(RenderOpts), P, P, u32, P, P, P, P, i32, P, P, P, P, P, P, P]),
     "pn_render_deformed_async": (i32, [P, P, C.POINTER(RenderOpts), P, P, u32, P, P, P, P, i32, P, P, P, P, P, i32, P]),
+    "pn_frame_build_tables": (i32, [P, C.POINTER(RenderOpts), P, P, P, P, i32, P, P]),
+    "pn_frame_tables_ahead": (i32, [P, C.POINTER(u32)]),
+    "pn_frame_drop_tables": (i32, [P]),
+    "pn_frame_set_camera": (i32, [P, P, f32, f32, f32, f32, i32, i32]),
+    "pn_frame_read_table": (i32, [P, i32, P, u64, C.POINTER(u64), P]),
     "pn_render_status": (i32, [P, P, i32, P]),
     "pn_frame_reset_unfinished": (i32, [P, P]),
     "pn_render_continue": (i32, [P, P, C.POINTER(RenderOpts), P, P, u32, P, P, P, P, P, P, i32, i32, P]),
diff --git a/pienerf_amd/csrc/pn_frame_kernels.h b/pienerf_amd/csrc/pn_frame_kernels.h
--- a/pienerf_amd/csrc/pn_frame_kernels.h
+++ b/pienerf_amd/csrc/pn_frame_kernels.h
@@ -5,6 +5,7 @@
 #include "pn_compact.h"
 #include "pn_march_kernels.h"
 #include "pn_near_far.h"
+#include "pn_ray_dir.h"
 #include "pn_side_tables.h"
 
 #define PN_MAX_TRIPS 1100
@@ -14,6 +15,15 @@
 #define PN_TIMED_TRIPS 64
 
 #include "pn_trips_fused.h"
+
+struct PnTablesKey {
+    const uint8_t* bitfield;
+    int n_vtx, cut, swap;
+    float hash_grid_size, bound, cut_bounds[6];
+    uint32_t cascade, grid_size;
+    int pad0;
+};
+static_assert(sizeof(PnTablesKey) == 64, "8 + 14 x 4 bytes");
 
 struct pn_frame {
     uint32_t max_rays, max_vtx, max_cells;
@@ -45,6 +55,12 @@
     uint32_t last_N;
     uint32_t last_group_rays;
     int tables_n_vtx;
+    int tables_ahead;
+    uint32_t tables_gen;
+    PnTablesKey tables_key;
+    int cam_set, cam_H, cam_W;
+    const float* cam_pose;
+    float cam_k[4];
     unsigned long long* march_counters;
     int march_counters_on;
     hipEvent_t ev[PN_TIMED_TRIPS][3];
@@ -263,7 +279,8 @@
     int n_grid_max; const int* n_grid_dev; const int* res; const int* pig_cnt; const int* pig_bgn; const int* pig_idx; const float* p_def; int swap;
     int2* nb_rng; float4* nb; int nb_capacity; int list_blocks; uint32_t* cell_bits; int lds_words;
     int pack_blocks; int n_vtx; const float* p_ori; const float* F_IP; const float* dF_IP; float* rec;
-    const float* rays_o; const float* rays_d; PnFrameDev* dev; uint32_t N; float min_near; float* nears; float* fars; float* rays_t; PnTrip* trips;
+    const float* pose; float fx, fy, cx, cy; int cam_W;
+    float* rays_o; float* rays_d; PnFrameDev* dev; uint32_t N; float min_near; float* nears; float* fars; float* rays_t; PnTrip* trips;
     int* tail_counts; int* seg_counters; int n_trip_records; int* alive; float* weights_sum; float* depth_0; float* image; PnGroup* groups;
     int* group_cnt; uint32_t group_rays; uint32_t n_groups; int* chunk_words;
     uint32_t tile_w, tile_lw;
@@ -372,7 +389,7 @@
             reinterpret_cast<int*>(a.trips + t)[w] = v;
             if (w == 0) a.tail_counts[t] = 0;
         }
-        if (block + 1 == gridDim.x - (uint32_t)(a.list_blocks + a.pack_blocks)) {
+        if (block + 1 == gridDim.x - (uint32_t)(a.list_blocks + a.pack_blocks + a.gr_blocks)) {
             for (int t2 = ((int)block + 1) * 4 + (int)(threadIdx.x >> 6); t2 < a.n_trip_records; t2 += 4) {
                 reinterpret_cast<int*>(a.trips + t2)[w] = 0;
                 if (w == 0) a.tail_counts[t2] = 0;
@@ -388,11 +405,19 @@
         }
     }
     if (threadIdx.x == 0) a.chunk_words[block] = 0;
-    if (threadIdx.x < 2 && block + 1 == gridDim.x - (uint32_t)(a.list_blocks + a.pack_blocks)) a.chunk_words[block + 1 + threadIdx.x] = 0;
+    if (threadIdx.x < 2 && block + 1 == gridDim.x - (uint32_t)(a.list_blocks + a.pack_blocks + a.gr_blocks)) a.chunk_words[block + 1 + threadIdx.x] = 0;
     if (n >= a.N) return;
     const float* aabb = a.dev->aabb;
-    const float ox = a.rays_o[n * 3], oy = a.rays_o[n * 3 + 1], oz = a.rays_o[n * 3 + 2];
-    const float dx = a.rays_d[n * 3], dy = a.rays_d[n * 3 + 1], dz = a.rays_d[n * 3 + 2];
+    float ro[3], rd[3];
+    if (a.pose) {
+        pn_pixel_ray(a.pose, a.fx, a.fy, a.cx, a.cy, (int)n % a.cam_W, (int)n / a.cam_W, ro, rd);
+#pragma unroll
+        for (int c = 0; c < 3; c++) { a.rays_o[n * 3 + c] = ro[c]; a.rays_d[n * 3 + c] = rd[c]; }
+    } else {
+#pragma unroll
+        for (int c = 0; c < 3; c++) { ro[c] = a.rays_o[n * 3 + c]; rd[c] = a.rays_d[n * 3 + c]; }
+    }
+    const float ox = ro[0], oy = ro[1], oz = ro[2], dx = rd[0], dy = rd[1], dz = rd[2];
     float near, far;
     pn_near_far(aabb, ox, oy, oz, dx, dy, dz, a.min_near, near, far);
     a.nears[n] = near;
diff --git a/pienerf_amd/csrc/pn_render_ops.hip b/pienerf_amd/csrc/pn_render_ops.hip
--- a/pienerf_amd/csrc/pn_render_ops.hip
+++ b/pienerf_amd/csrc/pn_render_ops.hip
@@ -303,6 +303,25 @@
     return PN_OK;
 }
 
+static PnTablesKey make_tables_key(const pn_render_opts* o, int n_vtx, const uint8_t* bitfield) {
+    PnTablesKey k;
+    memset(&k, 0, sizeof(k));
+    k.n_vtx = n_vtx; k.cut = o->cut ? 1 : 0; k.swap = (o->num_seek_IP == 1) ? 1 : 0;
+    k.hash_grid_size = o->hash_grid_size; k.bound = o->bound;
+    memcpy(k.cut_bounds, o->cut_bounds, sizeof(k.cut_bounds));
+    k.cascade = o->cascade; k.grid_size = o->grid_size; k.bitfield = bitfield;
+    return k;
+}
+
+static int upload_cut_bounds(pn_frame* f, const pn_render_opts* o, hipStream_t st) {
+    if (!f->cut_bounds_valid || memcmp(f->cut_bounds_host, o->cut_bounds, sizeof(f->cut_bounds_host)) != 0) {
+        memcpy(f->cut_bounds_host, o->cut_bounds, sizeof(f->cut_bounds_host));
+        PN_HIP_CHECK(hipMemcpyAsync(f->cut_bounds, f->cut_bounds_host, 6 * sizeof(float), hipMemcpyHostToDevice, st));
+        f->cut_bounds_valid = 1;
+    }
+    return PN_OK;
+}
+
 static int enqueue_tables(const RenderCall& c, bool is_static, bool keep_tables) {
     pn_frame* f = c.f;
     const pn_render_opts* o = c.o;
@@ -331,16 +350,11 @@
     return PN_OK;
 }
 
-static int enqueue_prologue(const RenderCall& c, const FramePlan& pl) {
+static void fill_table_ranges(FramePrologue& fp, const RenderCall& c, const FramePlan& pl, bool lists_and_records) {
     pn_frame* f = c.f;
     const pn_render_opts* o = c.o;
-    const bool keep_tables = !pl.is_static && o->reuse_tables && f->tables_n_vtx == c.n_vtx;
-    int rc = enqueue_tables(c, pl.is_static, keep_tables);
-    if (rc) return rc;
-    FramePrologue fp;
-    memset(&fp, 0, sizeof(fp));
-    if (!pl.is_static && !keep_tables) {
-        f->tables_n_vtx = c.n_vtx;
+    fp.dev = f->dev;
+    if (lists_and_records) {
         fp.n_grid_max = (int)f->max_cells; fp.n_grid_dev = f->dev->resolution + 3; fp.res = f->dev->resolution; fp.pig_cnt = f->pig_cnt; fp.pig_bgn = f->pig_bgn;
         fp.pig_idx = f->pig_idx; fp.p_def = c.p_def; fp.swap = (o->num_seek_IP == 1) ? 1 : 0; fp.nb_rng = f->side.nb_rng; fp.nb = f->side.nb;
         fp.nb_capacity = f->side.nb_capacity; fp.cell_bits = f->cell_bits;
@@ -348,7 +362,19 @@
         fp.pack_blocks = (int)pn_div_up((uint64_t)c.n_vtx * PN_REC_FLOATS, 256);
         fp.n_vtx = c.n_vtx; fp.p_ori = c.p_ori; fp.F_IP = c.F_IP; fp.dF_IP = c.dF_IP; fp.rec = f->side.rec;
     }
-    fp.rays_o = c.rays_o; fp.rays_d = c.rays_d; fp.dev = f->dev; fp.N = c.N; fp.min_near = o->min_near; fp.nears = f->nears; fp.fars = f->fars; fp.rays_t = f->rays_t;
+    fp.lds_words = (fp.list_blocks > 0 && pl.bit_words * 8 <= 64 * 1024) ? (int)pl.bit_words : 0;
+    if (pl.grid_region_words > 0) {
+        fp.grid = c.bitfield; fp.grid_regions = f->grid_regions; fp.gr_R = (int)pl.reg_R; fp.gr_C = (int)o->cascade; fp.gr_H = o->grid_size;
+        fp.gr_bound = o->bound; fp.cut_bounds = f->cut_bounds; fp.gr_blocks = (int)pn_div_up((uint64_t)pl.grid_region_words_1 * 32, 256);
+    }
+}
+
+static void fill_ray_range(FramePrologue& fp, const RenderCall& c, const FramePlan& pl, bool with_camera) {
+    pn_frame* f = c.f;
+    const pn_render_opts* o = c.o;
+    fp.rays_o = const_cast<float*>(c.rays_o); fp.rays_d = const_cast<float*>(c.rays_d);
+    if (with_camera) { fp.pose = f->cam_pose; fp.fx = f->cam_k[0]; fp.fy = f->cam_k[1]; fp.cx = f->cam_k[2]; fp.cy = f->cam_k[3]; fp.cam_W = f->cam_W; }
+    fp.dev = f->dev; fp.N = c.N; fp.min_near = o->min_near; fp.nears = f->nears; fp.fars = f->fars; fp.rays_t = f->rays_t;
     fp.trips = f->trips; fp.tail_counts = f->tail_counts; fp.seg_counters = f->seg_counters; fp.n_trip_records = PN_MAX_TRIPS + 2; fp.alive = f->alive_a;
     fp.weights_sum = c.weights_sum; fp.depth_0 = c.depth_0; fp.image = f->acc_image; fp.groups = pl.group_rays ? f->groups : nullptr; fp.group_cnt = f->group_cnt;
     fp.group_rays = pl.group_rays; fp.n_groups = pl.n_groups; fp.chunk_words = f->chunk_counts;
@@ -359,13 +385,24 @@
         fp.tile_lw = lw;
         fp.tile_w = (!pl.is_static && !pl.group_rays && tw && tw % (1u << lw) == 0 && c.N % ((64u >> lw) * tw) == 0) ? tw : 0u;
     }
-    fp.lds_words = (fp.list_blocks > 0 && pl.bit_words * 8 <= 64 * 1024) ? (int)pl.bit_words : 0;
-    if (pl.grid_region_words > 0) {
-        fp.grid = c.bitfield; fp.grid_regions = f->grid_regions; fp.gr_R = (int)pl.reg_R; fp.gr_C = (int)o->cascade; fp.gr_H = o->grid_size;
-        fp.gr_bound = o->bound; fp.cut_bounds = f->cut_bounds; fp.gr_blocks = (int)pn_div_up((uint64_t)pl.grid_region_words_1 * 32, 256);
-    }
+}
+
+static int enqueue_prologue(const RenderCall& c, const FramePlan& pl, bool ahead, bool with_camera) {
+    pn_frame* f = c.f;
+    const pn_render_opts* o = c.o;
+    const bool keep_tables = !pl.is_static && (ahead || (o->reuse_tables && f->tables_n_vtx == c.n_vtx));
+    int rc = enqueue_tables(c, pl.is_static, keep_tables);
+    if (rc) return rc;
+    FramePrologue fp;
+    memset(&fp, 0, sizeof(fp));
+    if (!ahead) {
+        if (!pl.is_static && !keep_tables) f->tables_n_vtx = c.n_vtx;
+        fill_table_ranges(fp, c, pl, !pl.is_static && !keep_tables);
+    }
+    fill_ray_range(fp, c, pl, with_camera);
     k_frame_prologue<<<(uint32_t)(fp.list_blocks + fp.pack_blocks + fp.gr_blocks) + pl.nblk, 256, (size_t)fp.lds_words * 8, c.st>>>(fp);
     PN_LAUNCH_CHECK();
+    if (ahead) f->tables_ahead = 0;
     return PN_OK;
 }
 
@@ -547,6 +584,15 @@
     c.image = image; c.depth = depth; c.depth_0 = depth_0; c.weights_sum = weights_sum; c.aabb_static = aabb_static; c.st = (hipStream_t)stream;
     int rc = check_render_call(c, is_static, resume, async_trips);
     if (rc) return rc;
+    const bool ahead = f->tables_ahead != 0;
+    if (ahead) {
+        PN_REQUIRE(!is_static && !resume);
+        const PnTablesKey key = make_tables_key(o, n_vtx, bitfield);
+        PN_REQUIRE(memcmp(&key, &f->tables_key, sizeof(key)) == 0);
+    }
+    const bool with_camera = f->cam_set != 0 && !resume;
+    if (!resume) f->cam_set = 0;
+    PN_REQUIRE(!with_camera || (!is_static && (uint64_t)f->cam_H * (uint64_t)f->cam_W == (uint64_t)N));
     const FramePlan pl = make_frame_plan(f, o, N, is_static, resume, async_trips, bitfield);
     c.mp = make_march_params(f->pig_cnt, f->pig_bgn, f->pig_idx, n_vtx, 0, p_def, p_ori, F_IP, dF_IP, o->max_iter_num, f->dev->aabb, f->dev->aabb + 3,
                              o->hash_grid_size, f->dev->resolution, o->num_seek_IP, o->IP_dx, o->cut, f->cut_bounds, f->rays_t, rays_o, rays_d, o->bound,
@@ -556,13 +602,9 @@
     if (pl.short_rays) c.mq.fars = f->fars_eff;
     c.tb = pnm2::March2Tables{f->side.nb_rng, f->side.nb, (const float4*)f->side.rec};
 
-    if (!f->cut_bounds_valid || memcmp(f->cut_bounds_host, o->cut_bounds, sizeof(f->cut_bounds_host)) != 0) {
-        memcpy(f->cut_bounds_host, o->cut_bounds, sizeof(f->cut_bounds_host));
-        PN_HIP_CHECK(hipMemcpyAsync(f->cut_bounds, f->cut_bounds_host, 6 * sizeof(float), hipMemcpyHostToDevice, c.st));
-        f->cut_bounds_valid = 1;
-    }
+    if ((rc = upload_cut_bounds(f, o, c.st))) return rc;
     if (!resume) {
-        if ((rc = enqueue_prologue(c, pl))) return rc;
+        if ((rc = enqueue_prologue(c, pl, ahead, with_camera))) return rc;
         f->skip_done = 0;
         f->head_marched = 0;
     }
@@ -586,6 +628,79 @@
     return PN_OK;
 }
 
+extern "C" int pn_frame_build_tables(pn_frame* f, const pn_render_opts* o, const float* p_def, const float* p_ori, const float* F_IP, const float* dF_IP,
+                                     int n_vtx, const uint8_t* bitfield, void* stream) {
+    PN_REQUIRE(f && o && p_def && p_ori && F_IP && dF_IP && bitfield && n_vtx > 0 && (uint32_t)n_vtx <= f->max_vtx);
+    PN_REQUIRE(o->num_seek_IP >= 1 && o->num_seek_IP <= 3 && o->cascade >= 1 && o->cascade <= 8);
+    RenderCall c{};
+    c.f = f; c.o = o; c.p_def = p_def; c.p_ori = p_ori; c.F_IP = F_IP; c.dF_IP = dF_IP; c.n_vtx = n_vtx; c.bitfield = bitfield; c.st = (hipStream_t)stream;
+    const FramePlan pl = make_frame_plan(f, o, 1, false, false, 1, bitfield);
+    int rc;
+    f->tables_ahead = 0;
+    if ((rc = upload_cut_bounds(f, o, c.st))) return rc;
+    if ((rc = enqueue_tables(c, false, false))) return rc;
+    FramePrologue fp;
+    memset(&fp, 0, sizeof(fp));
+    fill_table_ranges(fp, c, pl, true);
+    k_frame_prologue<<<(uint32_t)(fp.list_blocks + fp.pack_blocks + fp.gr_blocks), 256, (size_t)fp.lds_words * 8, c.st>>>(fp);
+    PN_LAUNCH_CHECK();
+    f->tables_n_vtx = n_vtx;
+    f->tables_key = make_tables_key(o, n_vtx, bitfield);
+    f->tables_gen++;
+    f->tables_ahead = 1;
+    return PN_OK;
+}
+
+extern "C" int pn_frame_tables_ahead(const pn_frame* f, uint32_t* generation_out) {
+    if (!f) return 0;
+    if (generation_out) *generation_out = f->tables_gen;
+    return f->tables_ahead;
+}
+
+extern "C" int pn_frame_drop_tables(pn_frame* f) {
+    PN_REQUIRE(f);
+    f->tables_ahead = 0;
+    f->tables_n_vtx = 0;
+    return PN_OK;
+}
+
+extern "C" int pn_frame_set_camera(pn_frame* f, const float* pose, float fx, float fy, float cx, float cy, int H, int W) {
+    PN_REQUIRE(f);
+    if (!pose) { f->cam_set = 0; return PN_OK; }
+    PN_REQUIRE(H > 0 && W > 0 && (uint64_t)H * (uint64_t)W <= f->max_rays);
+    f->cam_pose = pose; f->cam_k[0] = fx; f->cam_k[1] = fy; f->cam_k[2] = cx; f->cam_k[3] = cy; f->cam_H = H; f->cam_W = W;
+    f->cam_set = 1;
+    return PN_OK;
+}
+
+extern "C" int pn_frame_read_table(pn_frame* f, int which, void* dst_host, uint64_t bytes, uint64_t* bytes_total, void* stream) {
+    PN_REQUIRE(f);
+    const size_t words = ((size_t)f->max_cells + 31) / 32;
+    const void* src = nullptr;
+    size_t total = 0;
+    switch (which) {
+        case PN_TABLE_PIG_CNT: src = f->pig_cnt; total = (size_t)f->max_cells * 4; break;
+        case PN_TABLE_PIG_BGN: src = f->pig_bgn; total = (size_t)f->max_cells * 4; break;
+        case PN_TABLE_PIG_IDX: src = f->pig_idx; total = (size_t)f->max_vtx * 4; break;
+        case PN_TABLE_NB_RNG: src = f->side.nb_rng; total = (size_t)f->max_cells * sizeof(int2); break;
+        case PN_TABLE_NB: src = f->side.nb; total = (size_t)f->side.nb_capacity * sizeof(float4); break;
+        case PN_TABLE_REC: src = f->side.rec; total = (size_t)f->max_vtx * PN_REC_FLOATS * 4; break;
+        case PN_TABLE_CELL_BITS: src = f->cell_bits; total = 2 * words * 4; break;
+        case PN_TABLE_GRID_REGIONS: src = f->grid_regions; total = (size_t)PN_GRID_REGION_WORDS * 4; break;
+        case PN_TABLE_FRAME_RECORD: src = f->dev; total = 10 * 4; break;
+        case PN_TABLE_NEARS: src = f->nears; total = (size_t)f->max_rays * 4; break;
+        case PN_TABLE_FARS: src = f->fars; total = (size_t)f->max_rays * 4; break;
+        default: PN_REQUIRE(which >= 0 && which <= PN_TABLE_FARS);
+    }
+    if (bytes_total) *bytes_total = total;
+    if (dst_host && bytes > 0) {
+        PN_REQUIRE(bytes <= total);
+        PN_HIP_CHECK(hipStreamSynchronize((hipStream_t)stream));
+        PN_HIP_CHECK(hipMemcpy(dst_host, src, bytes, hipMemcpyDeviceToHost));
+    }
+    return PN_OK;
+}
+
 extern "C" int pn_render_deformed(pn_frame* f, const pn_net* net, const pn_render_opts* o, const float* rays_o, const float* rays_d, uint32_t N,
                                   const float* p_def, const float* p_ori, const float* F_IP, const float* dF_IP, int n_vtx,
                                   const uint8_t* bitfield, float* image, float* depth, float* depth_0, float* weights_sum, int64_t* stats_host,
diff --git a/pienerf_amd/frames.py b/pienerf_amd/frames.py
--- a/pienerf_amd/frames.py
+++ b/pienerf_amd/frames.py
@@ -116,6 +116,8 @@
         n_ws = self.lanes * self.depth
         self.render_done = [b.event() for _ in range(n_ws)]
         self.out_ready = [b.event() for _ in range(n_ws)]
+        self.tables_ready = [b.event() for _ in range(n_ws)]
+        self.ws_used = [False] * n_ws
         self.pending = [None] * n_ws
         self.frame = 0
         self.my_frames = 0
@@ -126,6 +128,7 @@
         self.sim_on_lanes = bool(sim_on_lanes) and self.world == 1
         self.sub_done = [b.event() for _ in range(self.lanes + 2)] if self.sim_on_lanes else []
         self.force_done, self.force_pending = (b.event() if self.sim_on_lanes else None), False
+        self.ahead_tables = bool(getattr(b, "ahead_tables", False)) and hasattr(b, "build_tables") and not self.sim_on_lanes
 
     def before_force(self):
         if self.sim_on_lanes and self.sim_next > 0:
@@ -196,22 +199,45 @@
     def step(self, pose=None):
         b, f, S = self.b, self.frame, self.slots
         self.retired = []
-        if self.rank == self.owner:
-            self._advance_simulator(f + self.ahead)
-        if self.collectives:
-            self._broadcasts(f + self.ahead)
         mine = frame_owner(f, self.world, self.owner, self.dedicated) == self.rank
-        if mine:
+        built = mine and self.ahead_tables
+        if built:
+            if self.rank == self.owner:
+                self._advance_simulator(f)
+            if self.collectives:
+                self._broadcasts(f)
             lane, ws = self._ws(self.my_frames)
             done = self.retire(ws)
             if done is not None:
                 self.retired.append(done)
             slot = f % S
+            sb = self.s_comm if self.collectives else self.s_sim
+            if self.ws_used[ws]:
+                sb.wait(self.render_done[ws])
+            b.build_tables(sb, f, ws, slot)
+            self.tables_ready[ws].record(sb)
+            self.ip_done[slot].record(sb)
+            self.ip_used[slot] = True
+        if self.rank == self.owner:
+            self._advance_simulator(f + self.ahead)
+        if self.collectives:
+            self._broadcasts(f + self.ahead)
+        if mine:
+            lane, ws = self._ws(self.my_frames)
+            slot = f % S
             s = self.s_lane[lane]
-            s.wait(self.bc_done[slot] if self.collectives else self.snap_ready[slot])
+            if built:
+                s.wait(self.tables_ready[ws])
+            else:
+                done = self.retire(ws)
+                if done is not None:
+                    self.retired.append(done)
+                s.wait(self.bc_done[slot] if self.collectives else self.snap_ready[slot])
             b.render(s, f, ws, slot, pose)
-            self.ip_done[slot].record(s)
-            self.ip_used[slot] = True
+            if not built:
+                self.ip_done[slot].record(s)
+                self.ip_used[slot] = True
+            self.ws_used[ws] = True
             self.render_done[ws].record(s)
             if self.copy_out:
                 where = getattr(b, "copy_on", "copy")
@@ -261,8 +287,10 @@
 
 class SimulatedBackend:
 
-    def __init__(self, world, rank, n_dof=64, owner=0, seed=0, needs_more_trips=lambda frame: False, group=None):
+    def __init__(self, world, rank, n_dof=64, owner=0, seed=0, needs_more_trips=lambda frame: False, group=None, ahead_tables=False):
         self.world, self.rank, self.owner, self.group = world, rank, owner, group
+        self.ahead_tables = bool(ahead_tables)
+        self.ws_tables, self.ws_rendering = {}, {}
         self.rng = random.Random(seed * 1000 + rank)
         self.streams = {}
         self.dof = torch.arange(n_dof, dtype=torch.float64) * (1.0 if rank == owner else -7.0)
@@ -347,15 +375,38 @@
             self.snap_tag[slot] = g
         self._enqueue(s, f"broadcast {g}", run)
 
+    def build_tables(self, s, frame, ws, slot):
+        key = (slot, frame)
+        self.readers_left[key] = self.readers_left.get(key, 0) + 1
+        self.ws_build_enqueued = getattr(self, "ws_build_enqueued", {})
+        self.ws_build_enqueued[ws] = frame
+
+        def run():
+            assert self.snap_tag.get(slot) == frame, f"tables of frame {frame} built from slot {slot} holding frame {self.snap_tag.get(slot)}"
+            others = self.ws_rendering.get(ws, set()) - {frame}
+            assert not others, f"tables of workspace {ws} rebuilt for frame {frame} while frame {sorted(others)} still reads them"
+            self.readers_left[key] -= 1
+            self.ws_tables[ws] = (frame, float(self.snap[slot].sum()))
+        self._enqueue(s, f"build_tables {frame}", run)
+
     def render(self, s, frame, ws, slot, pose):
         key = (slot, frame)
-        self.readers_left[key] = self.readers_left.get(key, 0) + 1
-
-        def run():
-            assert self.snap_tag.get(slot) == frame, f"frame {frame} rendered from slot {slot} holding frame {self.snap_tag.get(slot)}"
-            self.readers_left[key] -= 1
+        if not self.ahead_tables:
+            self.readers_left[key] = self.readers_left.get(key, 0) + 1
+        self.ws_rendering.setdefault(ws, set()).add(frame)
+
+        def run():
+            if self.ahead_tables:
+                assert self.ws_tables.get(ws, (None,))[0] == frame, f"frame {frame} rendered from workspace {ws} holding the tables of frame {self.ws_tables.get(ws)}"
+                state = self.ws_tables[ws][1]
+            else:
+                assert self.snap_tag.get(slot) == frame, f"frame {frame} rendered from slot {slot} holding frame {self.snap_tag.get(slot)}"
+                self.readers_left[key] -= 1
+                state = float(self.snap[slot].sum())
             short = bool(self.needs_more_trips(frame))
-            self.ws_out[ws] = (frame, float(self.snap[slot].sum()), None if pose is None else float(pose), "partial" if short else "full")
+            if not short:
+                self.ws_rendering[ws].discard(frame)
+            self.ws_out[ws] = (frame, state, None if pose is None else float(pose), "partial" if short else "full")
             self.ws_trips_short[ws] = short
             self.log.append(frame)
         self._enqueue(s, f"render {frame}", run)
@@ -370,6 +421,10 @@
 
     def finish(self, ws):
         f, v, p, _ = self.ws_out[ws]
+        assert self.ws_tables.get(ws, (f,))[0] == f, f"frame {f} continued on workspace {ws} holding the tables of frame {self.ws_tables[ws][0]}"
+        later = getattr(self, "ws_build_enqueued", {}).get(ws, f)
+        assert later == f, f"frame {f} continued on workspace {ws} with the build of frame {later} already enqueued"
+        self.ws_rendering.get(ws, set()).discard(f)
         self.ws_out[ws] = self.ws_host[ws] = (f, v, p, "full")
         self.ws_trips_short[ws] = False
 
diff --git a/pienerf_amd/harness.py b/pienerf_amd/harness.py
--- a/pienerf_amd/harness.py
+++ b/pienerf_amd/harness.py
@@ -211,7 +211,7 @@
     @torch.no_grad()
     def capture_pipelined(self, lanes=2, n_trips=8, W=None, H=None, sim_ahead=None, depth=2, sim_priority=0, sim_cus=0, copy_out=True, group=None,
                           frame_parallel=False, sim_owner=0, dedicated_sim=None, on_retire=None, copy_on="host", _probe_no_substep=False, _time_trips=False,
-                          render_kw=None, _force_collectives=False, sim_on_lanes=False):
+                          render_kw=None, _force_collectives=False, sim_on_lanes=False, ahead_tables=True):
         import torch.distributed as dist
 
         from .frames import FramePipeline
@@ -229,7 +229,7 @@
             self.sim.enable_persistent()
         be = _HipBackend(self, lanes, depth, int(n_trips), W, H, sim_priority, sim_cus, copy_out, group if on else None,
                          (dist.get_global_rank(group, sim_owner) if (on and group is not None) else sim_owner), _probe_no_substep, _time_trips, copy_on,
-                         render_kw=render_kw, distributed=on)
+                         render_kw=render_kw, distributed=on, ahead_tables=ahead_tables and not sim_on_lanes)
         self._pipe = FramePipeline(be, world=world, rank=rank, lanes=lanes, depth=depth, ahead=(lanes if sim_ahead is None and world == 1 else sim_ahead),
                                    sim_owner=sim_owner, dedicated_sim=dedicated_sim, copy_out=copy_out, on_retire=on_retire,
                                    force_collectives=bool(_force_collectives) and on, sim_on_lanes=sim_on_lanes)
@@ -340,6 +340,7 @@
 
     def capture_staged(self, batch=None, **kw):
         rk = dict(kw.pop("render_kw", None) or {}, ray_batch=int(batch or self.opt.get("max_ray_batch", 4096)))
+        kw.setdefault("ahead_tables", False)
         return self.capture_pipelined(render_kw=rk, **kw)
 
     def step_staged(self, pose=None):
@@ -434,7 +435,7 @@
 class _HipBackend:
 
     def __init__(self, h, lanes, depth, n_trips, W, H, sim_priority, sim_cus, copy_out, group, src, probe_no_substep, time_trips=False, copy_on="host",
-                 render_kw=None, distributed=False):
+                 render_kw=None, distributed=False, ahead_tables=True):
         self.copy_on = copy_on
         self.copier = None
         if copy_on == "host" and copy_out:
@@ -445,6 +446,7 @@
             check(lib().pn_copier_create(ctypes.byref(hc)), "copier_create")
             self.copier = hc
         self.h, self.lanes, self.depth, self.trips, self.W, self.H, self.group, self.src = h, lanes, depth, n_trips, W, H, group, src
+        self.ahead_tables = bool(ahead_tables)
         dev, m, sim = h.device, h.model, h.sim
         self.continued = 0
         if sim_cus > 0:
@@ -523,20 +525,26 @@
                 sim.stepforward()
             else:
                 sim.dof_vel.mul_(1.0)
-        self.graph, self.rays, self.out, self.host, self.packed = [], [], [], [], []
+        self.graph, self.rays, self.out, self.host, self.packed, self.build_graph = [], [], [], [], [], []
         N = W * H
         for ws in range(n_ws):
             s = self._streams[f"lane{ws // depth}"]
             m.p_def, m.IP_F, m.IP_dF = self.ip[ws]
+            if self.ahead_tables:
+                bg = torch.cuda.CUDAGraph()
+                with _capture(bg, stream=self._streams["sim"]):
+                    m.build_tables(N, **dict(kw, frame_slot=ws))
+                self.build_graph.append(bg)
             if time_trips:
                 m.march_counters(2, slot=ws)
             pk = torch.empty(N * 5, dtype=torch.float32, device=dev)
             ob = {"image": pk[:3 * N].view(N, 3), "depth": pk[3 * N:4 * N], "depth_0": pk[4 * N:], "weights_sum": torch.empty(N, dtype=torch.float32, device=dev)}
+            rays = {"rays_o": torch.empty(1, N, 3, dtype=torch.float32, device=dev), "rays_d": torch.empty(1, N, 3, dtype=torch.float32, device=dev)}
             g = torch.cuda.CUDAGraph()
             with _capture(g, stream=s):
-                rays = get_rays(self.pose_dev[ws], h.intrinsics, H, W, -1)
                 with h._amp():
-                    out = m.render_deformed(rays["rays_o"], rays["rays_d"], staged=True, bg_color=None, perturb=False, out_buffers=ob, **dict(kw, frame_slot=ws))
+                    out = m.render_deformed(rays["rays_o"], rays["rays_d"], staged=True, bg_color=None, perturb=False, out_buffers=ob,
+                                            camera=(self.pose_dev[ws], h.intrinsics, H, W), **dict(kw, frame_slot=ws))
             self.graph.append(g)
             self.rays.append(rays)
             self.out.append(out)
@@ -594,6 +602,11 @@
         with torch.cuda.stream(s.s):
             dist.broadcast(self._snap(slot), src=self.src, group=self.group)
 
+    def build_tables(self, s, frame, ws, slot):
+        with torch.cuda.stream(s.s):
+            self.h.sim.get_IP_info(dof=self._snap(slot), out=self.ip[ws])
+            self.build_graph[ws].replay()
+
     def consumer_fence(self, ws):
         ev = torch.cuda.Event()
         ev.record(torch.cuda.current_stream(self.h.device))
@@ -610,7 +623,8 @@
                 self.pose_key[ws] = key
                 self.pose_pin[ws].copy_(torch.from_numpy(p))
                 self.pose_dev[ws].copy_(self.pose_pin[ws], non_blocking=True)
-            self.h.sim.get_IP_info(dof=self._snap(slot), out=self.ip[ws])
+            if not self.ahead_tables:
+                self.h.sim.get_IP_info(dof=self._snap(slot), out=self.ip[ws])
             self.graph[ws].replay()
 
     def copy_out(self, s, ws, same_buffer=False):
diff --git a/pienerf_amd/nerf/renderer.py b/pienerf_amd/nerf/renderer.py
--- a/pienerf_amd/nerf/renderer.py
+++ b/pienerf_amd/nerf/renderer.py
@@ -177,6 +177,13 @@
             weights_sum = torch.empty(N, dtype=torch.float32, device=device)
         async_trips = int(kwargs.get("async_trips") or 0)
         frame, net = self._frame_handle(N, n_vtx, o.hash_grid_size, int(kwargs.get("frame_slot") or 0)), self._net_handle(half=bool(o.fp16))
+        cam = kwargs.get("camera")
+        if cam is not None:
+            pose, intr, cam_H, cam_W = cam
+            require_gpu(pose)
+            assert pose.dtype == torch.float32 and pose.is_contiguous() and pose.numel() == 16 and int(cam_H) * int(cam_W) == N
+            fx, fy, cx, cy = (float(v) for v in intr)
+            check(lib().pn_frame_set_camera(frame, ptr(pose), fx, fy, cx, cy, int(cam_H), int(cam_W)), "frame_set_camera")
         if async_trips > 0:
             check(lib().pn_render_deformed_async(frame, net, C.byref(o), ptr(rays_o), ptr(rays_d), N, ptr(p_def), ptr(p_ori), ptr(F_IP), ptr(dF_IP),
                                                  n_vtx, ptr(self.density_bitfield), ptr(image), ptr(depth), ptr(depth_0), ptr(weights_sum),
@@ -193,6 +200,33 @@
         elif bg_tensor is not None:
             image = image + (1 - weights_sum).unsqueeze(-1) * bg_tensor
         return {"depth": depth.view(*prefix), "image": image.view(*prefix, 3), "depth_0": depth_0.view(*prefix), "weights_sum": weights_sum}
+
+    def build_tables(self, n_rays, dt_gamma=0, max_steps=1024, T_thresh=1e-2, **kwargs):
+        device = self.density_bitfield.device
+        p_def, p_ori, F_IP, dF_IP = self._ip_state(device)
+        require_gpu(p_def)
+        assert p_def.shape == p_ori.shape and p_ori.shape[0] > 0
+        n_vtx = p_ori.shape[0]
+        o = self._deformed_opts(dt_gamma, 1.0, max_steps, T_thresh, kwargs, n_rays=n_rays)
+        frame = self._frame_handle(int(n_rays), n_vtx, o.hash_grid_size, int(kwargs.get("frame_slot") or 0))
+        check(lib().pn_frame_build_tables(frame, C.byref(o), ptr(p_def), ptr(p_ori), ptr(F_IP), ptr(dF_IP), n_vtx, ptr(self.density_bitfield), stream_ptr()),
+              "frame_build_tables")
+
+    def tables_ahead(self, slot=0):
+        gen = C.c_uint32(0)
+        return bool(lib().pn_frame_tables_ahead(self._frames[slot][0], C.byref(gen))), int(gen.value)
+
+    def drop_tables(self, slot=0):
+        check(lib().pn_frame_drop_tables(self._frames[slot][0]), "frame_drop_tables")
+
+    def read_table(self, which, slot=0, dtype=None):
+        import numpy as np
+        total = C.c_uint64(0)
+        h = self._frames[slot][0]
+        check(lib().pn_frame_read_table(h, int(which), None, 0, C.byref(total), stream_ptr()), "frame_read_table")
+        buf = np.empty(int(total.value), dtype=np.uint8)
+        check(lib().pn_frame_read_table(h, int(which), buf.ctypes.data_as(C.c_void_p), int(total.value), None, stream_ptr()), "frame_read_table")
+        return buf.view(np.int32 if dtype is None else dtype)
 
     def render_continue(self, slot, rays_o, rays_d, out, n_trips=0, dt_gamma=0, bg_color=None, max_steps=1024, T_thresh=1e-2, static=False, **kwargs):
         rays_o, rays_d = _flat_rays(rays_o, rays_d)
```

New measurement: 1271. 0.856x the previous value.
